# google-research/swirl-fem

Measured on AMD Instinct MI355X. Metric: GDOF/s per CG iteration, 3D p=7 Laplacian, higher is better.
Workload: dtype f64

## Files before the change

### include/sfem.h

```cpp
#ifndef SFEM_H_
#define SFEM_H_

#include <stdint.h>

#ifdef __cplusplus
extern "C" {
#endif

#define SFEM_ABI_VERSION 9

enum { SFEM_F32 = 0, SFEM_F64 = 1 };
enum {
  SFEM_OK = 0,
  SFEM_EINVAL = -1,
  SFEM_EHIP = -2,
  SFEM_EUNSUPPORTED = -3
};
#define SFEM_SENTINEL (-1)
#define SFEM_MAX_P 16

#define SFEM_IDX_MASK 0x3FFFFFFF
#define SFEM_IDX_PAD 0x3FFFFFFF
#define SFEM_IDX_DIRICHLET 0x80000000u
#define SFEM_IDX_SHARED 0x40000000u

typedef void* sfem_stream_t;

int sfem_abi_version(void);
const char* sfem_last_error(void);

int sfem_gather(const void* u, const int32_t* indices, void* out,
                int64_t count, double fill, int dtype, sfem_stream_t stream);

int sfem_gather_rows(const void* x, const int32_t* indices, void* out,
                     int64_t count, int ncomp, int dtype, sfem_stream_t stream);

int sfem_scatter_add(const void* u_local, const int32_t* indices, void* out,
                     int64_t count, int64_t num_nodes, int ncomp, int dtype,
                     sfem_stream_t stream);

int sfem_scatter_csr(const void* u_local, const int64_t* offsets,
                     const int32_t* slots, void* out, int64_t num_nodes,
                     int ncomp, int dtype, sfem_stream_t stream);

int sfem_exchange_local(const void* u, void* out, const int32_t* gidx,
                        const int32_t* unique, int64_t count,
                        int64_t num_nodes, void* sums, int64_t num_unique,
                        int ncomp, int dtype, sfem_stream_t stream);

int sfem_exchange_classes(void* u, const int32_t* members,
                          const int32_t* offsets, int64_t num_classes,
                          int ncomp, int64_t node_stride, int64_t comp_stride,
                          int dtype, sfem_stream_t stream);

int sfem_zero_strips(void* base, int64_t strip_len, int64_t strip_stride,
                     int nstrips, int dtype, sfem_stream_t stream);

int sfem_pack(const void* u, const int32_t* idx, void* buf, int64_t count,
              int ncomp, int dtype, sfem_stream_t stream);
int sfem_unpack_add(const void* buf, const int32_t* idx, void* u,
                    int64_t count, int ncomp, int dtype, sfem_stream_t stream);

int sfem_pack_strided(const void* u, const int32_t* idx, void* buf,
                      int64_t count, int ncomp, int64_t node_stride,
                      int64_t comp_stride, int dtype, sfem_stream_t stream);
int sfem_unpack_add_atomic(const void* buf, const int32_t* idx, void* u,
                           int64_t count, int ncomp, int64_t node_stride,
                           int64_t comp_stride, int dtype,
                           sfem_stream_t stream);

int sfem_geom_factors(const void* elem_coords, const void* interp1,
                      const void* grad1, int64_t num_elements, int ndim, int P,
                      int q, void* invjac, void* jacdet, void* quad_coords,
                      int dtype, sfem_stream_t stream);

int sfem_basis_eval(const void* u_local, const void* interp1,
                    const void* grad1, const void* invjac, void* val,
                    void* grad, int64_t num_elements, int ndim, int P, int q,
                    int ncomp, int collocated, int dtype, sfem_stream_t stream);

int sfem_basis_eval_t(const void* c0, const void* c1, const void* interp1,
                      const void* grad1, const void* invjac, const void* wdet,
                      void* out, int64_t num_elements, int ndim, int P, int q,
                      int ncomp, int collocated, int dtype,
                      sfem_stream_t stream);

enum { SFEM_COEF_NONE = 0, SFEM_COEF_ELEM = 1, SFEM_COEF_POINT = 2 };
enum { SFEM_GEO_POINT = 0, SFEM_GEO_AFFINE = 1, SFEM_GEO_MULTILINEAR = 3,
       SFEM_GEO_BOX = 5
                         };

int sfem_helmholtz_setup(const void* invjac, const void* jacdet,
                         const void* weights_nd , void* geo,
                         int64_t num_elements, int ndim, int Q, int dtype,
                         sfem_stream_t stream);
int sfem_helmholtz_setup_multilinear(const void* elem_coords, void* geo_elem,
                                     int64_t num_elements, int ndim, int P,
                                     int dtype, sfem_stream_t stream);

int sfem_encode_elements(const int32_t* elements, const uint8_t* dirichlet,
                         const int32_t* multiplicity,
                         const uint8_t* slot_shared, int32_t* enc,
                         int64_t count, sfem_stream_t stream);

typedef struct sfem_helmholtz_args {
  const void* u;
  void* out;
  const int32_t* enc;
  const void* geo;
  const void* geo_elem;
  const int32_t* geo_index;
  const int32_t* elem_list;
  const void* dmat;
  const void* weights;
  const void* nodes;
  int64_t num_elements;
  int64_t num_listed;
  int64_t num_nodes;
  int64_t zero_begin;
  int64_t zero_end;
  int32_t ndim;
  int32_t P;
  int32_t ncomp;
  int32_t dtype;
  int32_t geo_mode;
  int32_t colored;
  double lambda0;
  double lambda1;
  int64_t node_stride;
  int64_t comp_stride;
  double* dot_out;
  const uint16_t* shared_order;
  int32_t shared_stride;
  const int32_t* cluster_elems;
  const int32_t* cluster_offsets;
  const uint32_t* cluster_nodes;
  int64_t num_clusters;
  const int32_t* facet_table;
  const void* geo_const;
  const int32_t* chain_offsets;
  const int32_t* chain_elems;
  int64_t num_chains;
  int64_t layered_extent;
  int64_t dot_slots;
  const void* beta;
  const void* kappa;
  const void* sigma;
  int32_t coef_mode;
} sfem_helmholtz_args;

int sfem_facet_table_build(const int32_t* elements, const uint8_t* dirichlet,
                           const int32_t* multiplicity, int32_t* table,
                           uint8_t* ok, int64_t num_elements,
                           int64_t num_nodes, int P, sfem_stream_t stream);

int sfem_kernarg_selftest(int32_t* bad, sfem_stream_t stream);

int sfem_helmholtz_setup_affine(const void* geo_elem, void* geo_const,
                                int64_t num_elements, double box_tol,
                                int dtype, sfem_stream_t stream);

int sfem_helmholtz_cluster_limits(int P, int dtype, int* cluster_size,
                                  int* max_shared);
#define SFEM_DOT_SLOTS 1024

int sfem_helmholtz_apply(const sfem_helmholtz_args* args, sfem_stream_t stream);

int sfem_helmholtz_local(const sfem_helmholtz_args* args, sfem_stream_t stream);

typedef struct sfem_stokes_args {
  const void* u;
  void* out;
  const void* p_in;
  void* p_out;
  const void* scale;
  const int32_t* enc;
  const int32_t* penc;
  const void* kfac;
  const void* geo_elem;
  const int32_t* geo_index;
  const int32_t* elem_list;
  const void* dmat;
  const void* weights;
  const void* nodes;
  const void* interp;
  int64_t num_elements;
  int64_t num_listed;
  int64_t num_nodes;
  int64_t zero_begin, zero_end;
  int32_t ndim, P, dtype, geo_mode;
  int64_t node_stride, comp_stride;
  int32_t scale_per_node;
  const uint16_t* shared_order;
  int32_t shared_stride;
  double* dot_out;
  const int32_t* facet_table;
  const int32_t* chain_offsets;
  const int32_t* chain_elems;
  int64_t num_chains;
} sfem_stokes_args;

int sfem_stokes_setup(const void* invjac, const void* jacdet,
                      const void* weights_nd, void* kfac, int64_t num_elements,
                      int ndim, int Q, int dtype, sfem_stream_t stream);
int sfem_stokes_div(const sfem_stokes_args* args, sfem_stream_t stream);
int sfem_stokes_convect_local(const sfem_stokes_args* args,
                              sfem_stream_t stream);
int sfem_stokes_grad_t(const sfem_stokes_args* args, sfem_stream_t stream);
int sfem_stokes_e_first(const sfem_stokes_args* args, sfem_stream_t stream);
int sfem_stokes_e_second(const sfem_stokes_args* args, sfem_stream_t stream);

#define SFEM_CG_NSCALARS_NAMED 16
#define SFEM_CG_RR_SLOTS 64
#define SFEM_CG_NSCALARS (SFEM_CG_NSCALARS_NAMED + SFEM_CG_RR_SLOTS)
#define SFEM_CG_MEAN_SUMS (4 * SFEM_CG_RR_SLOTS)
#define SFEM_CG_STATUS_RUNNING 0.0
#define SFEM_CG_STATUS_CONVERGED 1.0
#define SFEM_CG_STATUS_MAXITER 2.0
#define SFEM_CG_STATUS_BAD_PAP 3.0
#define SFEM_CG_STATUS_BAD_GAMMA 4.0
int sfem_dot(const void* a, const void* b, int64_t count, double* result,
             int dtype, sfem_stream_t stream);
int sfem_dot_accumulate(const void* a, const void* b, int64_t count,
                        double* result, int dtype, sfem_stream_t stream);
int sfem_dot_indexed(const void* a, const void* b, const int64_t* idx,
                     const double* w, int64_t count, int ncomp,
                     int64_t node_stride, int64_t comp_stride, double scale,
                     double* result, int dtype, sfem_stream_t stream);
int sfem_subtract_weighted_mean(const void* w, const void* b, double total,
                                void* out, double* partials, int64_t count,
                                double* dot_result, int dtype,
                                sfem_stream_t stream);
int sfem_cg_scalars(double* scalars, int phase, double maxiter, double tol,
                    double atol, double* partials, sfem_stream_t stream);
int sfem_cg_update_xr(void* x, void* r, const void* p, const void* ap,
                      int64_t count, double* scalars, int fuse_rr, int dtype,
                      sfem_stream_t stream);
int sfem_cg_update_p(void* p, const void* z, int64_t count, double* scalars,
                     int dtype, sfem_stream_t stream);
int sfem_cg_update_r(void* r, const void* ap, int64_t count, double* scalars,
                     int fuse_rr, int dtype, sfem_stream_t stream);
int sfem_cg_update_xp(void* x, void* p, const void* z, int64_t count,
                      double* scalars, int dtype, sfem_stream_t stream);
#define SFEM_FOLD_GROUPS 256
int sfem_cg_scalars_n(double* scalars, int phase, double maxiter, double tol,
                      double atol, double* partials, int64_t num_partials,
                      sfem_stream_t stream);
int sfem_cg_update_r_layered_det(void* r, const void* ap_ext, int64_t count,
                                 const int64_t* layer_len,
                                 const int64_t* layer_off, int num_layers,
                                 const uint8_t* layer_masks,
                                 const int64_t* mask_off,
                                 double* scalars, double* rr_partials,
                                 int64_t rr_capacity, int64_t* num_rr,
                                 int dtype, sfem_stream_t stream);
#define SFEM_CG_LAZY_MAX 8
int sfem_cg_update_xp_lazy(void* x, void* pring, int64_t ring_stride,
                           const void* z, int64_t count, double* scalars,
                           double* lazy, int m, int dtype,
                           sfem_stream_t stream);
int sfem_cg_flush_x(void* x, const void* pring, int64_t ring_stride,
                    int64_t count, const double* scalars, double* lazy, int m,
                    int dtype, sfem_stream_t stream);
#define SFEM_MAX_LAYERS 15
#define SFEM_LAYER_CHUNK 512
int sfem_cg_update_r_layered(void* r, const void* ap_ext, int64_t count,
                             const int64_t* layer_len,
                             const int64_t* layer_off, int num_layers,
                             const uint8_t* layer_masks,
                             const int64_t* mask_off, double* scalars,
                             int fuse_rr, int dtype, sfem_stream_t stream);
int sfem_fold_layers(void* out_ext, int64_t count, const int64_t* layer_len,
                     const int64_t* layer_off, int num_layers, int dtype,
                     sfem_stream_t stream);
int sfem_fold_layers_at(void* out_ext, const int64_t* idx, int64_t num_idx,
                        int64_t count, const int64_t* layer_len,
                        const int64_t* layer_off, int num_layers, int dtype,
                        sfem_stream_t stream);
int sfem_cg_update_r_mean(void* r, const void* ap, const void* w,
                          int64_t count, double* scalars, double* sums,
                          int dtype, sfem_stream_t stream);
int sfem_cg_update_xp_mean(void* x, void* p, const void* r, int64_t count,
                           double* scalars, double* sums, double total,
                           int dtype, sfem_stream_t stream);
int sfem_fdm_solve(const void* r, void* z, const int64_t* pel, const void* S,
                   const int32_t* cases, const void* inv_eigenvalues,
                   int64_t num_elements, int ndim, int Pp, int dtype,
                   sfem_stream_t stream);
int sfem_fdm_solve_sums(const void* r, void* z, const int64_t* pel,
                        const void* S, const int32_t* cases,
                        const void* inv_eigenvalues, const void* weights,
                        void* elem_sum, void* weighted_sum,
                        int64_t num_elements, int ndim, int Pp, int dtype,
                        sfem_stream_t stream);
int sfem_add_element_constants(void* z, const void* yc, const void* shift,
                               int64_t num_elements, int n,
                               int64_t elems_per_member, int dtype,
                               sfem_stream_t stream);
int sfem_ell_chebyshev(const int32_t* cols, const void* vals, const void* dinv,
                       const void* b, void* x, void* work, int64_t n,
                       int width, int steps, double lmin, double lmax,
                       int dtype, sfem_stream_t stream);
#define SFEM_ENS_NSCALARS 16
#define SFEM_ENS_GROUPS 32
#define SFEM_ENS_MAX_MEMBERS 4096
int sfem_ens_dot(const void* a, const void* b, int64_t len, int members,
                 double* partials, int which, int dtype, sfem_stream_t stream);
int sfem_ens_init(double* scalars, const double* partials, int members,
                  double maxiter, double tol, double atol,
                  sfem_stream_t stream);
int sfem_ens_update_r(void* r, const void* ap, int64_t len, int members,
                      const double* scalars, const double* partials,
                      int dtype, sfem_stream_t stream);
int sfem_ens_close(double* scalars, const double* partials, int members,
                   double maxiter, sfem_stream_t stream);
int sfem_ens_update_xp(void* x, void* p, const void* z, int64_t len,
                       int members, const double* scalars, int dtype,
                       sfem_stream_t stream);
int sfem_ens_update_r_mean(void* r, const void* ap, const void* w, int64_t len,
                           int members, const double* scalars,
                           const double* partials, double* sums, int dtype,
                           sfem_stream_t stream);
int sfem_ens_close_mean(double* scalars, const double* partials,
                        const double* sums, double total, int members,
                        double maxiter, sfem_stream_t stream);
int sfem_ens_update_xp_mean(void* x, void* p, const void* r, int64_t len,
                            int members, const double* scalars, int dtype,
                            sfem_stream_t stream);
int sfem_ens_subtract_weighted_mean(const void* w, const void* b, double total,
                                    void* out, double* partials, int64_t len,
                                    int members, int dtype,
                                    sfem_stream_t stream);
typedef struct sfem_diag_args {
  void* mass_out;
  void* stiff_out;
  const void* geo;
  const void* geo_elem;
  const int32_t* geo_index;
  const int32_t* elem_list;
  const void* bmat;
  const void* dtil;
  const void* weights;
  const void* nodes;
  int64_t num_elements;
  int64_t num_listed;
  int ndim;
// ... 94 lines not shown
```

### swirl_fem_amd/_lib.py

```python

from __future__ import annotations

import ctypes
import os

from swirl_fem_amd import switches

_HERE = os.path.dirname(os.path.abspath(__file__))
LIB_PATH = switches.get('SFEM_LIB') or os.path.join(_HERE, 'libsfem_hip.so')
ABI_VERSION = 9

SFEM_F32, SFEM_F64 = 0, 1
SFEM_CG_NSCALARS_NAMED = 16
SFEM_CG_NSCALARS = 80
SFEM_BICGSTAB_NSCALARS = 32
BICGSTAB_STATUS = {0: 'running', 1: 'converged', 2: 'maxiter',
                   3: 'breakdown_rho', 4: 'breakdown_omega',
                   5: 'breakdown_alpha'}
CG_STATUS = {0: 'running', 1: 'converged', 2: 'maxiter', 3: 'breakdown_pAp',
             4: 'breakdown_gamma'}
SFEM_DOT_SLOTS = 1024
SFEM_CG_MEAN_SUMS = 256
SFEM_MAX_LAYERS = 15
SFEM_FOLD_GROUPS = 256
SFEM_LAYER_CHUNK = 512
SFEM_CG_LAZY_MAX = 8
SFEM_IDX_MASK = 0x3FFFFFFF
SFEM_ENS_NSCALARS = 16
SFEM_ENS_GROUPS = 32
SFEM_ENS_MAX_MEMBERS = 4096

c_i32, c_i64, c_dbl, c_ptr = (ctypes.c_int32, ctypes.c_int64, ctypes.c_double,
                              ctypes.c_void_p)


class HelmholtzArgs(ctypes.Structure):
  _fields_ = [
      ('u', c_ptr), ('out', c_ptr), ('enc', c_ptr), ('geo', c_ptr),
      ('geo_elem', c_ptr), ('geo_index', c_ptr), ('elem_list', c_ptr),
      ('dmat', c_ptr), ('weights', c_ptr), ('nodes', c_ptr),
      ('num_elements', c_i64), ('num_listed', c_i64), ('num_nodes', c_i64),
      ('zero_begin', c_i64), ('zero_end', c_i64), ('ndim', c_i32),
      ('P', c_i32), ('ncomp', c_i32), ('dtype', c_i32), ('geo_mode', c_i32),
      ('colored', c_i32), ('lambda0', c_dbl), ('lambda1', c_dbl),
      ('node_stride', c_i64), ('comp_stride', c_i64), ('dot_out', c_ptr),
      ('shared_order', c_ptr), ('shared_stride', c_i32),
      ('cluster_elems', c_ptr), ('cluster_offsets', c_ptr),
      ('cluster_nodes', c_ptr), ('num_clusters', c_i64),
      ('facet_table', c_ptr), ('geo_const', c_ptr),
      ('chain_offsets', c_ptr), ('chain_elems', c_ptr), ('num_chains', c_i64),
      ('layered_extent', c_i64), ('dot_slots', c_i64),
      ('beta', c_ptr),
      ('kappa', c_ptr), ('sigma', c_ptr), ('coef_mode', c_i32),
  ]


class StokesArgs(ctypes.Structure):
  _fields_ = [
      ('u', c_ptr), ('out', c_ptr), ('p_in', c_ptr), ('p_out', c_ptr),
      ('scale', c_ptr), ('enc', c_ptr), ('penc', c_ptr), ('kfac', c_ptr),
      ('geo_elem', c_ptr), ('geo_index', c_ptr), ('elem_list', c_ptr),
      ('dmat', c_ptr), ('weights', c_ptr), ('nodes', c_ptr), ('interp', c_ptr),
      ('num_elements', c_i64), ('num_listed', c_i64), ('num_nodes', c_i64),
      ('zero_begin', c_i64), ('zero_end', c_i64), ('ndim', c_i32),
      ('P', c_i32), ('dtype', c_i32), ('geo_mode', c_i32),
      ('node_stride', c_i64), ('comp_stride', c_i64),
      ('scale_per_node', c_i32), ('shared_order', c_ptr),
      ('shared_stride', c_i32), ('dot_out', c_ptr),
      ('facet_table', c_ptr), ('chain_offsets', c_ptr), ('chain_elems', c_ptr),
      ('num_chains', c_i64),
  ]


class DiagArgs(ctypes.Structure):
  _fields_ = [
      ('mass_out', c_ptr), ('stiff_out', c_ptr), ('geo', c_ptr),
      ('geo_elem', c_ptr), ('geo_index', c_ptr), ('elem_list', c_ptr),
      ('bmat', c_ptr), ('dtil', c_ptr), ('weights', c_ptr), ('nodes', c_ptr),
      ('num_elements', c_i64), ('num_listed', c_i64), ('ndim', c_i32),
      ('P', c_i32), ('Q', c_i32), ('dtype', c_i32), ('geo_mode', c_i32),
      ('kappa', c_ptr), ('sigma', c_ptr), ('coef_mode', c_i32),
  ]


GEO_POINT, GEO_AFFINE, GEO_MULTILINEAR, GEO_BOX = 0, 1, 3, 5
COEF_NONE, COEF_ELEM, COEF_POINT = 0, 1, 2

SIGNATURES = {
    'sfem_gather': [c_ptr, c_ptr, c_ptr, c_i64, c_dbl, c_i32, c_ptr],
    'sfem_gather_rows': [c_ptr, c_ptr, c_ptr, c_i64, c_i32, c_i32, c_ptr],
    'sfem_scatter_add': [c_ptr, c_ptr, c_ptr, c_i64, c_i64, c_i32, c_i32,
                         c_ptr],
    'sfem_scatter_csr': [c_ptr, c_ptr, c_ptr, c_ptr, c_i64, c_i32, c_i32,
                         c_ptr],
    'sfem_exchange_local': [c_ptr, c_ptr, c_ptr, c_ptr, c_i64, c_i64, c_ptr,
                            c_i64, c_i32, c_i32, c_ptr],
    'sfem_exchange_classes': [c_ptr, c_ptr, c_ptr, c_i64, c_i32, c_i64, c_i64,
                              c_i32, c_ptr],
    'sfem_zero_strips': [c_ptr, c_i64, c_i64, c_i32, c_i32, c_ptr],
    'sfem_subtract_weighted_mean': [c_ptr, c_ptr, c_dbl, c_ptr, c_ptr, c_i64,
                                    c_ptr, c_i32, c_ptr],
    'sfem_pack': [c_ptr, c_ptr, c_ptr, c_i64, c_i32, c_i32, c_ptr],
    'sfem_unpack_add': [c_ptr, c_ptr, c_ptr, c_i64, c_i32, c_i32, c_ptr],
    'sfem_pack_strided': [c_ptr, c_ptr, c_ptr, c_i64, c_i32, c_i64, c_i64,
                          c_i32, c_ptr],
    'sfem_unpack_add_atomic': [c_ptr, c_ptr, c_ptr, c_i64, c_i32, c_i64,
                               c_i64, c_i32, c_ptr],
    'sfem_geom_factors': [c_ptr, c_ptr, c_ptr, c_i64, c_i32, c_i32, c_i32,
                          c_ptr, c_ptr, c_ptr, c_i32, c_ptr],
    'sfem_basis_eval': [c_ptr, c_ptr, c_ptr, c_ptr, c_ptr, c_ptr, c_i64, c_i32,
                        c_i32, c_i32, c_i32, c_i32, c_i32, c_ptr],
    'sfem_basis_eval_t': [c_ptr, c_ptr, c_ptr, c_ptr, c_ptr, c_ptr, c_ptr,
                          c_i64, c_i32, c_i32, c_i32, c_i32, c_i32, c_i32,
                          c_ptr],
    'sfem_helmholtz_setup': [c_ptr, c_ptr, c_ptr, c_ptr, c_i64, c_i32, c_i32,
                             c_i32, c_ptr],
    'sfem_encode_elements': [c_ptr, c_ptr, c_ptr, c_ptr, c_ptr, c_i64, c_ptr],
    'sfem_helmholtz_apply': [ctypes.POINTER(HelmholtzArgs), c_ptr],
    'sfem_helmholtz_setup_multilinear': [c_ptr, c_ptr, c_i64, c_i32, c_i32,
                                         c_i32, c_ptr],
    'sfem_helmholtz_local': [ctypes.POINTER(HelmholtzArgs), c_ptr],
    'sfem_facet_table_build': [c_ptr, c_ptr, c_ptr, c_ptr, c_ptr, c_i64, c_i64,
                               c_i32, c_ptr],
    'sfem_helmholtz_setup_affine': [c_ptr, c_ptr, c_i64, c_dbl, c_i32, c_ptr],
    'sfem_helmholtz_cluster_limits': [c_i32, c_i32, ctypes.POINTER(c_i32),
                                      ctypes.POINTER(c_i32)],
    'sfem_dot': [c_ptr, c_ptr, c_i64, c_ptr, c_i32, c_ptr],
    'sfem_dot_accumulate': [c_ptr, c_ptr, c_i64, c_ptr, c_i32, c_ptr],
    'sfem_dot_indexed': [c_ptr, c_ptr, c_ptr, c_ptr, c_i64, c_i32, c_i64,
                         c_i64, c_dbl, c_ptr, c_i32, c_ptr],
    'sfem_cg_scalars': [c_ptr, c_i32, c_dbl, c_dbl, c_dbl, c_ptr, c_ptr],
    'sfem_cg_update_xr': [c_ptr, c_ptr, c_ptr, c_ptr, c_i64, c_ptr, c_i32,
                          c_i32, c_ptr],
    'sfem_cg_update_p': [c_ptr, c_ptr, c_i64, c_ptr, c_i32, c_ptr],
    'sfem_cg_update_r': [c_ptr, c_ptr, c_i64, c_ptr, c_i32, c_i32, c_ptr],
    'sfem_cg_update_xp': [c_ptr, c_ptr, c_ptr, c_i64, c_ptr, c_i32, c_ptr],
    'sfem_cg_update_r_layered': [c_ptr, c_ptr, c_i64, c_ptr, c_ptr, c_i32,
                                 c_ptr, c_ptr, c_ptr, c_i32, c_i32, c_ptr],
    'sfem_kernarg_selftest': [c_ptr, c_ptr],
    'sfem_fdm_solve': [c_ptr, c_ptr, c_ptr, c_ptr, c_ptr, c_ptr, c_i64, c_i32,
                       c_i32, c_i32, c_ptr],
    'sfem_fdm_solve_sums': [c_ptr, c_ptr, c_ptr, c_ptr, c_ptr, c_ptr, c_ptr,
                            c_ptr, c_ptr, c_i64, c_i32, c_i32, c_i32, c_ptr],
    'sfem_add_element_constants': [c_ptr, c_ptr, c_ptr, c_i64, c_i32, c_i64,
                                   c_i32, c_ptr],
    'sfem_ell_chebyshev': [c_ptr, c_ptr, c_ptr, c_ptr, c_ptr, c_ptr, c_i64,
                           c_i32, c_i32, c_dbl, c_dbl, c_i32, c_ptr],
    'sfem_ens_dot': [c_ptr, c_ptr, c_i64, c_i32, c_ptr, c_i32, c_i32, c_ptr],
    'sfem_ens_init': [c_ptr, c_ptr, c_i32, c_dbl, c_dbl, c_dbl, c_ptr],
    'sfem_ens_update_r': [c_ptr, c_ptr, c_i64, c_i32, c_ptr, c_ptr, c_i32,
                          c_ptr],
    'sfem_ens_close': [c_ptr, c_ptr, c_i32, c_dbl, c_ptr],
    'sfem_ens_update_xp': [c_ptr, c_ptr, c_ptr, c_i64, c_i32, c_ptr, c_i32,
                           c_ptr],
    'sfem_ens_update_r_mean': [c_ptr, c_ptr, c_ptr, c_i64, c_i32, c_ptr, c_ptr,
                               c_ptr, c_i32, c_ptr],
    'sfem_ens_close_mean': [c_ptr, c_ptr, c_ptr, c_dbl, c_i32, c_dbl, c_ptr],
    'sfem_ens_update_xp_mean': [c_ptr, c_ptr, c_ptr, c_i64, c_i32, c_ptr,
                                c_i32, c_ptr],
    'sfem_ens_subtract_weighted_mean': [c_ptr, c_ptr, c_dbl, c_ptr, c_ptr,
                                        c_i64, c_i32, c_i32, c_ptr],
    'sfem_fold_layers': [c_ptr, c_i64, c_ptr, c_ptr, c_i32, c_i32, c_ptr],
    'sfem_fold_layers_at': [c_ptr, c_ptr, c_i64, c_i64, c_ptr, c_ptr, c_i32,
                            c_i32, c_ptr],
    'sfem_cg_scalars_n': [c_ptr, c_i32, c_dbl, c_dbl, c_dbl, c_ptr, c_i64,
                          c_ptr],
    'sfem_cg_update_r_layered_det': [c_ptr, c_ptr, c_i64, c_ptr, c_ptr, c_i32,
                                     c_ptr, c_ptr, c_ptr, c_ptr, c_i64, c_ptr,
                                     c_i32, c_ptr],
    'sfem_cg_update_xp_lazy': [c_ptr, c_ptr, c_i64, c_ptr, c_i64, c_ptr, c_ptr,
                               c_i32, c_i32, c_ptr],
    'sfem_cg_flush_x': [c_ptr, c_ptr, c_i64, c_i64, c_ptr, c_ptr, c_i32, c_i32,
                        c_ptr],
    'sfem_cg_update_r_mean': [c_ptr, c_ptr, c_ptr, c_i64, c_ptr, c_ptr, c_i32,
                              c_ptr],
    'sfem_cg_update_xp_mean': [c_ptr, c_ptr, c_ptr, c_i64, c_ptr, c_ptr, c_dbl,
                               c_i32, c_ptr],
    'sfem_axpby': [c_dbl, c_ptr, c_dbl, c_ptr, c_i64, c_i32, c_ptr],
    'sfem_helmholtz_diag': [ctypes.POINTER(DiagArgs), c_ptr],
    'sfem_cg_update_r_jacobi': [c_ptr, c_ptr, c_ptr, c_i64, c_i32, c_ptr,
                                c_ptr, c_i32, c_ptr, c_ptr, c_ptr, c_ptr,
                                c_i64, c_ptr, c_i32, c_ptr],
    'sfem_cg_update_xp_jacobi': [c_ptr, c_ptr, c_ptr, c_ptr, c_i64, c_i32,
                                 c_ptr, c_i32, c_ptr],
    'sfem_stokes_setup': [c_ptr, c_ptr, c_ptr, c_ptr, c_i64, c_i32, c_i32,
                          c_i32, c_ptr],
    'sfem_stokes_div': [c_ptr, c_ptr],
    'sfem_stokes_grad_t': [c_ptr, c_ptr],
    'sfem_stokes_e_first': [c_ptr, c_ptr],
    'sfem_stokes_e_second': [c_ptr, c_ptr],
    'sfem_stokes_convect_local': [c_ptr, c_ptr],
    'sfem_pmg_prolong': [c_ptr, c_ptr, c_ptr, c_ptr, c_ptr, c_ptr, c_i64,
                         c_i32, c_i32, c_i32, c_i32, c_i32, c_ptr],
    'sfem_pmg_restrict': [c_ptr, c_ptr, c_ptr, c_ptr, c_ptr, c_ptr, c_i64,
                          c_i32, c_i32, c_i32, c_i32, c_ptr],
    'sfem_cheb_step': [c_ptr, c_ptr, c_ptr, c_ptr, c_ptr, c_ptr, c_dbl, c_dbl,
                       c_i64, c_i32, c_i32, c_ptr],
    'sfem_pmg_dot2': [c_ptr, c_ptr, c_ptr, c_i64, c_ptr, c_i32, c_i32, c_ptr],
    'sfem_pmg_cg_scalars': [c_ptr, c_i32, c_ptr, c_i64, c_dbl, c_dbl, c_dbl,
                            c_ptr],
    'sfem_boundary_geom': [c_ptr, c_ptr, c_i64, c_ptr, c_ptr, c_ptr, c_i32,
                           c_i32, c_i32, c_ptr, c_ptr, c_i32, c_ptr],
    'sfem_boundary_covector': [c_ptr, c_i32, c_ptr, c_i64, c_ptr, c_ptr,
                               c_i32, c_i32, c_i32, c_ptr, c_i32, c_ptr],
    'sfem_boundary_mass_apply': [c_ptr, c_ptr, c_i64, c_ptr, c_ptr, c_i32,
                                 c_i32, c_i32, c_dbl, c_ptr, c_i32, c_ptr],
    'sfem_boundary_mass_diag': [c_ptr, c_i64, c_ptr, c_ptr, c_i32, c_i32,
                                c_i32, c_dbl, c_ptr, c_i32, c_ptr],
    'sfem_boundary_add_rows': [c_ptr, c_ptr, c_ptr, c_ptr, c_i64, c_ptr, c_i32,
                               c_ptr],
    'sfem_ell_spmv': [c_ptr, c_ptr, c_ptr, c_ptr, c_i64, c_i32, c_i64, c_i64,
                      c_ptr, c_i64, c_i32, c_ptr],
    'sfem_bicgstab_scalars': [c_ptr, c_i32, c_dbl, c_dbl, c_dbl, c_ptr],
    'sfem_bicgstab_dot': [c_ptr, c_ptr, c_i64, c_ptr, c_i32, c_i32, c_i32,
                          c_ptr],
    'sfem_bicgstab_update_p': [c_ptr, c_ptr, c_ptr, c_ptr, c_ptr, c_i64, c_ptr,
                               c_i32, c_ptr],
    'sfem_bicgstab_update_s': [c_ptr, c_ptr, c_ptr, c_ptr, c_ptr, c_i64, c_ptr,
                               c_i32, c_ptr],
    'sfem_bicgstab_update_xr': [c_ptr, c_ptr, c_ptr, c_ptr, c_ptr, c_ptr,
                                c_ptr, c_i64, c_ptr, c_i32, c_ptr],
    'sfem_abi_version': [],
}

_lib = None


class SfemError(RuntimeError):
  """A C-ABI call returned a non-zero status."""


def load() -> ctypes.CDLL:
  global _lib
  if _lib is not None:
    return _lib
  if not os.path.exists(LIB_PATH):
    raise SfemError(
        f'{LIB_PATH} is missing: the HIP extension has not been built. '
        'Run `make -C swirl_fem_amd/csrc -j8` (needs hipcc, gfx950). There is '
        'no CPU fallback.')
  lib = ctypes.CDLL(LIB_PATH)
  for name, argtypes in SIGNATURES.items():
    fn = getattr(lib, name)
    fn.argtypes = argtypes
    fn.restype = ctypes.c_int
  lib.sfem_last_error.argtypes = []
  lib.sfem_last_error.restype = ctypes.c_char_p
  if lib.sfem_abi_version() != ABI_VERSION:
    raise SfemError(f'ABI version mismatch: library '
                    f'{lib.sfem_abi_version()} != binding {ABI_VERSION}')
  _lib = lib
  return lib


def check(status: int, who: str):
  if status != 0:
# ... 3 lines not shown
```

### swirl_fem_amd/_ops.py

```python

from __future__ import annotations

import ctypes
import os

import numpy as np
import torch

from swirl_fem_amd import switches
from swirl_fem_amd import _lib

_DT = {torch.float32: _lib.SFEM_F32, torch.float64: _lib.SFEM_F64}


def _dtype_code(t: torch.Tensor) -> int:
  try:
    return _DT[t.dtype]
  except KeyError:
    raise TypeError(f'unsupported dtype {t.dtype}; use float32 or float64')


def _dev(*tensors):
  dev = None
  for t in tensors:
# ... 320 lines not shown
  dev = _dev(elements, dirichlet_u8, multiplicity, slot_shared)
  enc = torch.empty_like(elements)
  with torch.cuda.device(dev):
    _lib.check(_lib.load().sfem_encode_elements(
        _ptr(elements), _ptr(dirichlet_u8), _ptr(multiplicity),
        _ptr(slot_shared), _ptr(enc), elements.numel(), _stream(dev)),
        'sfem_encode_elements')
  return enc


def helmholtz_setup_multilinear(elem_coords, ndim, P):
  elem_coords = elem_coords.contiguous()
  dev = _dev(elem_coords)
  E = elem_coords.shape[0]
  geo_elem = torch.empty((E, 24), dtype=elem_coords.dtype, device=dev)
  with torch.cuda.device(dev):
    _lib.check(_lib.load().sfem_helmholtz_setup_multilinear(
        _ptr(elem_coords), _ptr(geo_elem), E, ndim, P,
        _dtype_code(elem_coords), _stream(dev)),
        'sfem_helmholtz_setup_multilinear')
  return geo_elem


_KERNARG_CHECKED = set()


def kernarg_selftest(dev):
  if dev in _KERNARG_CHECKED:
    return
  bad = torch.zeros(1, dtype=torch.int32, device=dev)
  with torch.cuda.device(dev):
    _lib.check(_lib.load().sfem_kernarg_selftest(_ptr(bad), _stream(dev)),
               'sfem_kernarg_selftest')
  if int(bad.item()) != 0:
    raise _lib.SfemError(
        'the kernel-argument layout differs from what the facet kernels '
        f'assume (probe flags {int(bad.item())}): rebuild libsfem_hip.so with '
        'the toolchain it was written for (FacetKernarg::MAT_OFF)')
  _KERNARG_CHECKED.add(dev)


def facet_table(elements, dirichlet_u8, multiplicity, P):
  elements = _idx(elements)
  dev = _dev(elements, dirichlet_u8, multiplicity)
  kernarg_selftest(dev)
  E = elements.shape[0]
  tab = torch.empty((E, 27, 4), dtype=torch.int32, device=dev)
  ok = torch.empty((E,), dtype=torch.uint8, device=dev)
  with torch.cuda.device(dev):
    _lib.check(_lib.load().sfem_facet_table_build(
        _ptr(elements), _ptr(dirichlet_u8), _ptr(multiplicity), _ptr(tab),
        _ptr(ok), E, multiplicity.shape[0], P, _stream(dev)),
        'sfem_facet_table_build')
  return tab, ok != 0


def helmholtz_setup_affine(geo_elem, box_tol):
  geo_elem = geo_elem.contiguous()
  dev = _dev(geo_elem)
  E = geo_elem.shape[0]
  out = torch.empty((E, 8), dtype=geo_elem.dtype, device=dev)
  with torch.cuda.device(dev):
    _lib.check(_lib.load().sfem_helmholtz_setup_affine(
        _ptr(geo_elem), _ptr(out), E, float(box_tol), _dtype_code(geo_elem),
        _stream(dev)), 'sfem_helmholtz_setup_affine')
  return out


def _host(a, dtype):
  np_dt = np.float64 if dtype == torch.float64 else np.float32
  return None if a is None else np.ascontiguousarray(a, dtype=np_dt)


def _hptr(a):
  return None if a is None else a.ctypes.data


def _dptr(t):
  return None if t is None else t.data_ptr()


def _helmholtz_args(u, out, enc, part, host, ndim, P, num_elements, num_nodes,
                    lambda0, lambda1, zero_range, dot_out=None,
                    layered_extent=0, dot_slots=0):
  vec = u.dim() != (1 if enc is not None else 2)
  ncomp = u.shape[-1] if vec else 1
  node_stride = comp_stride = 0
  if vec and not u.is_contiguous():
    node_stride, comp_stride = 1, u.stride(-1)
  lst = part.get('elem_list')
  so = part.get('shared_order')
  cl = part.get('cluster') if enc is not None else None
  if cl is not None:
    enc, so = cl.enc, None
  ft = part.get('facet_table') if enc is not None else None
  ch = None
  if layered_extent:
    ft, so = part['layered_table'], None
    ch = part.get('chains') if part.get('layered_chains') else None
  elif ft is not None:
    so = None
    if ((not vec or node_stride == 1) and
        switches.get('SFEM_CHAIN') != '0' and
        (not vec or switches.get('SFEM_CHAIN_VECTOR') != '0')):
      ch = part.get('chains')
  return _lib.HelmholtzArgs(
      u=u.data_ptr(), out=out.data_ptr(), enc=_dptr(enc),
      geo=_dptr(part.get('geo')), geo_elem=_dptr(part.get('geo_elem')),
      geo_index=_dptr(part.get('geo_index')), elem_list=_dptr(lst),
      dmat=_hptr(host['dmat']), weights=_hptr(host.get('weights')),
      nodes=_hptr(host.get('nodes')), num_elements=num_elements,
      num_listed=0 if lst is None else lst.numel(), num_nodes=num_nodes,
      zero_begin=int(zero_range[0]), zero_end=int(zero_range[1]), ndim=ndim,
      P=P, ncomp=ncomp, dtype=_dtype_code(u), geo_mode=part['geo_mode'],
      colored=int(bool(part.get('colored', False))), lambda0=float(lambda0),
      lambda1=float(lambda1), node_stride=node_stride,
      comp_stride=comp_stride,
      dot_out=_dptr(dot_out),
      shared_order=_dptr(so if enc is not None else None),
      shared_stride=0 if so is None or enc is None else so.shape[1],
      cluster_elems=_dptr(cl.elems if cl is not None else None),
      cluster_offsets=_dptr(cl.offsets if cl is not None else None),
      cluster_nodes=_dptr(cl.nodes if cl is not None else None),
      num_clusters=0 if cl is None else cl.num_clusters,
      facet_table=_dptr(ft),
      geo_const=_dptr(part.get('geo_const') if ft is not None else None),
      chain_offsets=_dptr(ch[0] if ch is not None else None),
      chain_elems=_dptr(ch[1] if ch is not None else None),
      num_chains=0 if ch is None else ch[0].numel() - 1,
      layered_extent=int(layered_extent), dot_slots=int(dot_slots),
      kappa=_dptr(part.get('kappa')), sigma=_dptr(part.get('sigma')),
      coef_mode=int(part.get('coef_mode', _lib.COEF_NONE)),
      beta=_dptr(part.get('beta')))


_CLUSTER_LIMITS = {}


def helmholtz_cluster_limits(P, dtype):
  key = (P, dtype)
  if key not in _CLUSTER_LIMITS:
    size, kmax = ctypes.c_int32(0), ctypes.c_int32(0)
    code = _lib.SFEM_F64 if dtype == torch.float64 else _lib.SFEM_F32
    rc = _lib.load().sfem_helmholtz_cluster_limits(
        P, code, ctypes.byref(size), ctypes.byref(kmax))
    _CLUSTER_LIMITS[key] = None if rc else (size.value, kmax.value)
  return _CLUSTER_LIMITS[key]


def helmholtz_kernel_name(real, P, ndim, scalar, geo_mode, part, mass,
                          layered=False):
  b = lambda v: 'true' if v else 'false'
  if part.get('facet_table') is not None:
    elem = ('sfem::BoxElem<%s, %d, %s>' % (real, P, b(mass)) if geo_mode == 5
            else 'sfem::FacetElem<%s, %d, %d, %s>' % (real, P, geo_mode,
                                                     b(mass)))
    if layered:
      if part.get('chains') is not None and part.get('layered_chains'):
        return 'sfem::helmholtz_chain_kernel<%s, %d, %s, *, true>' % (
            real, P, elem)
      return 'sfem::helmholtz_facet_kernel<%s, %d, %s, true, *, true>' % (
          real, P, elem)
    if (scalar and part.get('chains') is not None and
        switches.get('SFEM_CHAIN') != '0'):
      return 'sfem::helmholtz_chain_kernel<%s, %d, %s, ' % (real, P, elem)
    return 'sfem::helmholtz_facet_kernel<%s, %d, %s, %s, ' % (
        real, P, elem, b(scalar))
  if (real == 'float' and P == 12 and ndim == 3 and scalar and
      geo_mode in (1, 3) and part.get('cluster') is None and
      not part.get('colored') and switches.get('SFEM_MFMA') == '1'):
    return 'sfem::helmholtz_mfma_p12_kernel<%d, %s>' % (geo_mode, b(mass))
  if part.get('cluster') is not None:
    return 'sfem::helmholtz_cluster_kernel<%s, %d, %s, %d, %s>' % (
        real, P, b(scalar), geo_mode, b(mass))
  if part.get('beta') is not None:
    return 'sfem::helmholtz_adv_kernel<%s, %d, %d, true, %d>' % (
        real, P, ndim, geo_mode)
  if part.get('coef_mode'):
    return ('sfem::helmholtz_kernel<%s, %d, %d, true, true, %d, false, %s, '
            '%d>' % (real, P, ndim, geo_mode, b(mass), part['coef_mode']))
  tpe = P * P if ndim == 3 else P
  can_sort = ndim == 3 and tpe <= 64
  sort = (can_sort and part.get('shared_order') is not None and
          not part.get('colored') and not (geo_mode == 3 and mass))
  b = lambda v: 'true' if v else 'false'
  return 'sfem::helmholtz_kernel<%s, %d, %d, true, %s, %d, %s, %s>' % (
      real, P, ndim, b(scalar), geo_mode, b(sort), b(mass))


def helmholtz_apply(u, out, enc, parts, host, ndim, P, lambda0, lambda1,
                    zero_range, dot_out=None):
  dev = _dev(enc)
  _check_vector_layout(u, out)
  host = {k: _host(v, u.dtype) for k, v in host.items()}
  if not parts and zero_range[1] > zero_range[0]:
    out[zero_range[0]:zero_range[1]].zero_()
  with torch.cuda.device(dev):
    for n, part in enumerate(parts):
      args = _helmholtz_args(u, out, part.get('enc', enc), part, host, ndim,
                             P, enc.shape[0], u.shape[0], lambda0, lambda1,
                             zero_range if n == 0 else (0, 0), dot_out)
      _lib.check(_lib.load().sfem_helmholtz_apply(ctypes.byref(args),
                                                  _stream(dev)),
                 'sfem_helmholtz_apply')
  return out


def layered_dot_waves(parts, P, num_elements):
  waves = (P * P + 63) // 64
  out = []
  for part in parts:
    if part.get('layered_chains'):
      groups = part['chains'][0].numel() - 1
    elif 'elem_list' in part:
      groups = part['elem_list'].numel()
    else:
      groups = num_elements
    out.append(groups * waves)
  return out


def helmholtz_apply_layered(u, ext, enc, parts, host, ndim, P, lambda0,
                            lambda1, dot_out=None, per_wave=False):
  dev = _dev(enc)
  if u.dim() != 1 or not u.is_contiguous() or not ext.is_contiguous():
    raise ValueError('layered assembly takes contiguous scalar fields')
  if ext.dtype != u.dtype:
    raise ValueError('u and the extended output differ in dtype')
  host = {k: _host(v, u.dtype) for k, v in host.items()}
  waves = (layered_dot_waves(parts, P, enc.shape[0])
           if per_wave and dot_out is not None else None)
  if waves is not None and sum(waves) > dot_out.numel():
    raise ValueError(f'{sum(waves)} waves but {dot_out.numel()} dot slots')
  at = 0
  with torch.cuda.device(dev):
    for n, part in enumerate(parts):
      dots = dot_out if waves is None else dot_out[at:at + waves[n]]
      args = _helmholtz_args(u, ext, enc, part, host, ndim, P, enc.shape[0],
                             u.shape[0], lambda0, lambda1, (0, 0), dots,
                             layered_extent=ext.numel(),
                             dot_slots=0 if waves is None else waves[n])
      if waves is not None:
        at += waves[n]
      _lib.check(_lib.load().sfem_helmholtz_apply(ctypes.byref(args),
                                                  _stream(dev)),
                 'sfem_helmholtz_apply')
  return ext


def _layer_arrays(layers):
  n = len(layers)
  arr = ctypes.c_int64 * max(n, 1)
  return (arr(*[int(l[0]) for l in layers]) if n else arr(0),
          arr(*[int(l[1]) for l in layers]) if n else arr(0), n)


def _mask_args(masks, n):
  if masks is None:
    return None, None
  data, offs = masks
  arr = ctypes.c_int64 * max(n, 1)
  return _ptr(data), arr(*[int(o) for o in offs])


def cg_update_r_layered(r, ap_ext, layers, scalars, fuse_rr, masks=None):
  dev = _dev(r, ap_ext, scalars)
  ln, off, n = _layer_arrays(layers)
  mptr, moff = _mask_args(masks, n)
  with torch.cuda.device(dev):
    _lib.check(_lib.load().sfem_cg_update_r_layered(
        _ptr(r), _ptr(ap_ext), r.numel(), ln, off, n, mptr, moff,
        _ptr(scalars), int(fuse_rr), _dtype_code(r), _stream(dev)),
        'sfem_cg_update_r_layered')


def cg_update_r_layered_det(r, ap_ext, layers, scalars, rr_partials,
                            masks=None):
  dev = _dev(r, ap_ext, scalars, rr_partials)
  ln, off, n = _layer_arrays(layers)
  mptr, moff = _mask_args(masks, n)
  count = ctypes.c_int64(0)
  with torch.cuda.device(dev):
    _lib.check(_lib.load().sfem_cg_update_r_layered_det(
        _ptr(r), _ptr(ap_ext), r.numel(), ln, off, n, mptr, moff,
        _ptr(scalars),
        _ptr(rr_partials), rr_partials.numel(), ctypes.byref(count),
        _dtype_code(r), _stream(dev)), 'sfem_cg_update_r_layered_det')
  return count.value


def cg_scalars_n(scalars, phase, maxiter, tol, atol, partials, num_partials):
  dev = _dev(scalars, partials)
  with torch.cuda.device(dev):
    _lib.check(_lib.load().sfem_cg_scalars_n(
        _ptr(scalars), phase, float(maxiter), float(tol), float(atol),
        _ptr(partials), int(num_partials), _stream(dev)), 'sfem_cg_scalars_n')


def fold_layers_at(ext, idx, count, layers):
  dev = _dev(ext, idx)
  if idx.dtype != torch.int64:
    raise ValueError('fold_layers_at: int64 node positions')
  ln, off, n = _layer_arrays(layers)
  with torch.cuda.device(dev):
    _lib.check(_lib.load().sfem_fold_layers_at(
        _ptr(ext), _ptr(idx), idx.numel(), int(count), ln, off, n,
        _dtype_code(ext), _stream(dev)), 'sfem_fold_layers_at')
  return ext


def fdm_solve(r, pel, S, cases, inv_ev, ndim, Pp):
  dev = _dev(r, pel, S, cases, inv_ev)
  z = torch.empty_like(r)
  with torch.cuda.device(dev):
    _lib.check(_lib.load().sfem_fdm_solve(
        _ptr(r), _ptr(z), _ptr(pel), _ptr(S), _ptr(cases), _ptr(inv_ev),
        cases.shape[1], int(ndim), int(Pp), _dtype_code(r), _stream(dev)),
        'sfem_fdm_solve')
  return z


def fdm_solve_sums(r, pel, S, cases, inv_ev, weights, ndim, Pp):
  dev = _dev(r, pel, S, cases, inv_ev, weights)
  E = cases.shape[1]
# ... 339 lines not shown
  for t in (u, out):
    if not t.is_cuda:
      raise RuntimeError(
          'swirl_fem_amd kernels run on MI355X device tensors only; got a '
          f'{t.device} tensor (there is no CPU fallback)')
    if not (t.is_contiguous() or is_component_major(t)):
      raise ValueError('expected a contiguous or component-major tensor')
  if u.stride() != out.stride() or u.shape != out.shape:
    raise ValueError('u and out must share shape and memory layout')


def helmholtz_local(u_local, parts, host, ndim, P, lambda0, lambda1):
  if not (u_local.is_contiguous() or is_component_major(u_local)):
    u_local = u_local.contiguous()
  dev = u_local.device
  host = {k: _host(v, u_local.dtype) for k, v in host.items()}
  out = torch.empty_like(u_local)
  _check_vector_layout(u_local, out)
  with torch.cuda.device(dev):
    for part in parts:
      args = _helmholtz_args(u_local, out, None, part, host, ndim, P,
                             u_local.shape[0], 0, lambda0, lambda1, (0, 0))
      _lib.check(_lib.load().sfem_helmholtz_local(ctypes.byref(args),
                                                  _stream(dev)),
                 'sfem_helmholtz_local')
  return out


def dot(a, b, result, slot, accumulate=False):
  dev = _dev(a, b, result)
  fn = (_lib.load().sfem_dot_accumulate if accumulate
        else _lib.load().sfem_dot)
  with torch.cuda.device(dev):
    _lib.check(fn(_ptr(a), _ptr(b), a.numel(),
                  ctypes.c_void_p(result.data_ptr() + 8 * slot),
                  _dtype_code(a), _stream(dev)), 'sfem_dot')


def dot_indexed(a, b, idx, w, result, slot, scale):
  ncomp, ns, cs = _node_view(a)
  if _node_view(b) != (ncomp, ns, cs) or a.dtype != b.dtype:
    raise ValueError('dot_indexed: operands must share layout and dtype')
  flat = lambda t: t.movedim(-1, 0) if is_component_major(t) else t
  dev = _dev(flat(a), flat(b), idx, w, result)
  with torch.cuda.device(dev):
    _lib.check(_lib.load().sfem_dot_indexed(
        _ptr(a), _ptr(b), _ptr(idx), _ptr(w), idx.numel(), ncomp, ns, cs,
        float(scale), result.data_ptr() + 8 * slot, _dtype_code(a),
        _stream(dev)), 'sfem_dot_indexed')


def cg_scalars(scalars, phase, maxiter, tol, atol, partials=None):
  dev = _dev(scalars, partials)
  with torch.cuda.device(dev):
    _lib.check(_lib.load().sfem_cg_scalars(
        _ptr(scalars), phase, float(maxiter), float(tol), float(atol),
        _ptr(partials), _stream(dev)), 'sfem_cg_scalars')


def cg_update_xr(x, r, p, ap, scalars, fuse_rr):
  dev = _dev(x, r, p, ap, scalars)
  with torch.cuda.device(dev):
    _lib.check(_lib.load().sfem_cg_update_xr(
        _ptr(x), _ptr(r), _ptr(p), _ptr(ap), x.numel(), _ptr(scalars),
        int(fuse_rr), _dtype_code(x), _stream(dev)), 'sfem_cg_update_xr')


def cg_update_p(p, z, scalars):
  dev = _dev(p, z, scalars)
  with torch.cuda.device(dev):
    _lib.check(_lib.load().sfem_cg_update_p(
        _ptr(p), _ptr(z), p.numel(), _ptr(scalars), _dtype_code(p),
        _stream(dev)), 'sfem_cg_update_p')


def cg_update_r(r, ap, scalars, fuse_rr):
  dev = _dev(r, ap, scalars)
  with torch.cuda.device(dev):
    _lib.check(_lib.load().sfem_cg_update_r(
        _ptr(r), _ptr(ap), r.numel(), _ptr(scalars), int(fuse_rr),
        _dtype_code(r), _stream(dev)), 'sfem_cg_update_r')


def cg_update_xp_lazy(x, pring, z, scalars, lazy):
  dev = _dev(x, pring, z, scalars, lazy)
  with torch.cuda.device(dev):
    _lib.check(_lib.load().sfem_cg_update_xp_lazy(
        _ptr(x), _ptr(pring), pring.stride(0), _ptr(z), x.numel(),
        _ptr(scalars), _ptr(lazy), pring.shape[0], _dtype_code(x),
        _stream(dev)), 'sfem_cg_update_xp_lazy')


def cg_flush_x(x, pring, scalars, lazy):
  dev = _dev(x, pring, scalars, lazy)
  with torch.cuda.device(dev):
    _lib.check(_lib.load().sfem_cg_flush_x(
        _ptr(x), _ptr(pring), pring.stride(0), x.numel(), _ptr(scalars),
        _ptr(lazy), pring.shape[0], _dtype_code(x), _stream(dev)),
        'sfem_cg_flush_x')


def cg_update_xp(x, p, z, scalars):
  dev = _dev(x, p, z, scalars)
  with torch.cuda.device(dev):
    _lib.check(_lib.load().sfem_cg_update_xp(
        _ptr(x), _ptr(p), _ptr(z), x.numel(), _ptr(scalars), _dtype_code(x),
        _stream(dev)), 'sfem_cg_update_xp')


def cg_update_r_mean(r, ap, w, scalars, sums):
  dev = _dev(r, ap, w, scalars, sums)
  with torch.cuda.device(dev):
    _lib.check(_lib.load().sfem_cg_update_r_mean(
        _ptr(r), _ptr(ap), _ptr(w), r.numel(), _ptr(scalars), _ptr(sums),
        _dtype_code(r), _stream(dev)), 'sfem_cg_update_r_mean')


def cg_update_xp_mean(x, p, r, scalars, sums, total):
  dev = _dev(x, p, r, scalars, sums)
  with torch.cuda.device(dev):
    _lib.check(_lib.load().sfem_cg_update_xp_mean(
        _ptr(x), _ptr(p), _ptr(r), x.numel(), _ptr(scalars), _ptr(sums),
        float(total), _dtype_code(x), _stream(dev)), 'sfem_cg_update_xp_mean')


def axpby(a, x, b, y):
  dev = _dev(x, y)
  with torch.cuda.device(dev):
    _lib.check(_lib.load().sfem_axpby(
        float(a), _ptr(x), float(b), _ptr(y), x.numel(), _dtype_code(x),
        _stream(dev)), 'sfem_axpby')
  return y


def bicgstab_scalars(scalars, phase, maxiter, tol, atol):
  dev = _dev(scalars)
  with torch.cuda.device(dev):
    _lib.check(_lib.load().sfem_bicgstab_scalars(
        _ptr(scalars), int(phase), float(maxiter), float(tol), float(atol),
        _stream(dev)), 'sfem_bicgstab_scalars')


def bicgstab_dot(a, b, scalars, slot, two=False):
  dev = _dev(a, b, scalars)
  if a.dtype != b.dtype or a.numel() != b.numel():
    raise ValueError('bicgstab_dot: operands must share size and dtype')
  with torch.cuda.device(dev):
    _lib.check(_lib.load().sfem_bicgstab_dot(
        _ptr(a), _ptr(b), a.numel(), _ptr(scalars), int(slot), int(two),
        _dtype_code(a), _stream(dev)), 'sfem_bicgstab_dot')


def _same(name, *ts):
  first = ts[0]
  for t in ts:
    if t is not None and (t.dtype != first.dtype or
                          t.numel() != first.numel()):
      raise ValueError(f'{name}: vectors must share size and dtype')


def bicgstab_update_p(p, phat, r, v, dinv, scalars):
  dev = _dev(p, phat, r, v, dinv, scalars)
  _same('bicgstab_update_p', p, phat, r, v, dinv)
  with torch.cuda.device(dev):
    _lib.check(_lib.load().sfem_bicgstab_update_p(
        _ptr(p), _ptr(phat), _ptr(r), _ptr(v), _ptr(dinv), p.numel(),
        _ptr(scalars), _dtype_code(p), _stream(dev)),
        'sfem_bicgstab_update_p')


def bicgstab_update_s(s, shat, r, v, dinv, scalars):
  dev = _dev(s, shat, r, v, dinv, scalars)
  _same('bicgstab_update_s', s, shat, r, v, dinv)
  with torch.cuda.device(dev):
    _lib.check(_lib.load().sfem_bicgstab_update_s(
        _ptr(s), _ptr(shat), _ptr(r), _ptr(v), _ptr(dinv), s.numel(),
        _ptr(scalars), _dtype_code(s), _stream(dev)),
        'sfem_bicgstab_update_s')


def bicgstab_update_xr(x, r, phat, shat, s, t, r0, scalars):
  dev = _dev(x, r, phat, shat, s, t, r0, scalars)
# ... 222 lines not shown
```

### swirl_fem_amd/core/operators.py

```python

from __future__ import annotations

import dataclasses
import os

import numpy as np
import torch

from swirl_fem_amd import switches
from swirl_fem_amd import _ops

MAX_FUSED_P = 12


def supports_fused(fespace) -> str | None:
  P = fespace.mesh.gridpoints_1d.num_points
  if not fespace.is_collocated:
    return 'quadrature points differ from the nodes'
  if fespace.mesh.ndim not in (2, 3):
    return f'ndim={fespace.mesh.ndim}'
  if not 2 <= P <= MAX_FUSED_P:
    return f'P={P} outside 2..{MAX_FUSED_P}'
  d = fespace.interpolator._differentiation_matrix_1d()
  if not np.allclose(d[::-1, ::-1], -d, rtol=0,
# ... 717 lines not shown
  def split(self, element_mask):
    if any(p.get('colored') for p in self.parts):
      raise NotImplementedError('split() of a coloured operator')
    if self.coefs is not None:
      raise NotImplementedError('split() of an operator with coefficients')
    mask = torch.as_tensor(element_mask, device=self.enc.device).to(torch.bool)
    E = self.enc.shape[0]
    if mask.shape != (E,):
      raise ValueError(f'expected an ({E},) element mask')
    clustered = any(p.get('cluster') is not None for p in self.parts)

    def restrict(part_list, keep):
      parts = []
      for part in part_list:
        part = {k: v for k, v in part.items() if k != 'cluster'}
        if 'elem_list' in part:
          lst = part['elem_list']
          lst = lst[keep[lst.to(torch.int64)]]
        else:
          lst = torch.nonzero(keep).reshape(-1).to(torch.int32)
        if lst.numel():
          new = dict(part, elem_list=lst.contiguous())
          if 'chains' in new:
            new['chains'] = facet_chains(
                self.fespace.mesh.elements, lst.to(torch.int64),
                self.fespace.mesh.gridpoints_1d.num_points, new['chain_len'])
          parts.append(new)
      return parts

    halves = []
    for keep in (mask, ~mask):
      parts = restrict(self.parts, keep)
      if clustered:
        parts = _attach_clusters(
            self.fespace, self.enc,
            self.fespace.mesh.assembly_plan().multiplicity, parts)
      facet = (None if self.facet_parts is None
               else restrict(self.facet_parts, keep))
      halves.append(dataclasses.replace(self, parts=parts, facet_parts=facet,
                                        _vector_parts=None, _layer_plan=False,
                                        _diag=None, _diag_adv=None))
    return tuple(halves)

  def apply(self, u, lambda0=0.0, lambda1=1.0, out=None, *, zero=True,
            dot_out=None):
    mesh = self.fespace.mesh
    if u.shape[0] != mesh.num_nodes:
      raise ValueError(f'expected {mesh.num_nodes} nodal values, got '
                       f'{tuple(u.shape)}')
    if self.coefs is not None:
      _check_scalar_field(u)
      lambda0, lambda1 = _scaled(self.coefs, lambda0, lambda1)
    if self.beta is not None:
      _check_scalar_field(u, 'a velocity takes')
      if dot_out is not None:
        raise NotImplementedError('dot_out of an operator with a velocity')
    u = u.to(self.fespace.dtype)
    if not (u.is_contiguous() or _ops.is_component_major(u)):
      u = u.contiguous()
    if out is None:
      out = torch.empty_like(u)
    return _ops.helmholtz_apply(
        u, out, self.enc, self._parts_for(u), self.host, mesh.ndim,
        mesh.gridpoints_1d.num_points, lambda0, lambda1,
        self.zero_range if zero else (0, 0), dot_out)

  def layer_plan(self):
    if self._layer_plan is None:
      plan = None
      if (self.facet_parts is not None and
          switches.get('SFEM_LAYERED') != '0'):
        mesh = self.fespace.mesh
        plan = build_layer_plan(self.facet_parts, mesh.num_elements,
                                mesh.num_nodes, mesh.gridpoints_1d.num_points)
      self._layer_plan = plan if plan is not None else False
    return self._layer_plan or None

  def new_extended(self):
    plan = self.layer_plan()
    return torch.zeros(plan.extent, dtype=self.fespace.dtype,
                       device=self.enc.device)

  def apply_layered(self, u, ext, lambda0=0.0, lambda1=1.0, *, dot_out=None,
                    per_wave=False):
    plan = self.layer_plan()
    if plan is None:
      raise NotImplementedError('this operator has no layer plan')
    mesh = self.fespace.mesh
    if tuple(u.shape) != (mesh.num_nodes,):
      raise ValueError(f'expected ({mesh.num_nodes},) nodal values, got '
                       f'{tuple(u.shape)}')
    if tuple(ext.shape) != (plan.extent,):
      raise ValueError(f'expected an extended output of {plan.extent} values')
    return _ops.helmholtz_apply_layered(
        u.to(self.fespace.dtype).contiguous(), ext, self.enc, plan.parts,
        self.host, mesh.ndim, mesh.gridpoints_1d.num_points, lambda0, lambda1,
        dot_out, per_wave)

  def layered_dot_slots(self):
    mesh = self.fespace.mesh
    return sum(_ops.layered_dot_waves(self.layer_plan().parts,
                                      mesh.gridpoints_1d.num_points,
                                      mesh.num_elements))

  def _parts_for(self, u):
    if self.facet_parts is None or not (
        u.dim() == 1 or u.shape[-1] == 1 or _ops.is_component_major(u)):
      return self.parts
    if u.dim() == 1 or u.shape[-1] == 1:
      return self.facet_parts
    if self._vector_parts is None:
      if not any(q['geo_mode'] == _GEO_POINT and 'facet_table' in q
                 for q in self.facet_parts):
        self._vector_parts = self.facet_parts
      elif self.fespace.dtype == torch.float64:
        self._vector_parts = (
            [q for q in self.facet_parts if q['geo_mode'] != _GEO_POINT] +
            [q for q in self.parts if q['geo_mode'] == _GEO_POINT])
      else:
        self._vector_parts = [
            {k: v for k, v in q.items() if k != 'chains'}
            if q['geo_mode'] == _GEO_POINT else q for q in self.facet_parts]
    return self._vector_parts

  def diagonal(self, lambda0=0.0, lambda1=1.0, assembled=True):
    if self._diag is None:
      self._diag = _assembled_diagonal(self.fespace, self.parts, self.host,
                                       self.keep, None)
    lambda0, lambda1 = _scaled(self.coefs, lambda0, lambda1)
    d = _combine_diagonal(self._diag, lambda0, lambda1, assembled,
                          self.fespace.mesh)
    if self.beta is not None:
      if self._diag_adv is None:
        self._diag_adv = _advection_diagonal(
            self.fespace, self.parts, self.beta, self.host['dmat'], self.keep,
            None)
      d = d + self._diag_adv
    return d

  def point_weights(self):
    mesh = self.fespace.mesh
    P = mesh.gridpoints_1d.num_points
    mass, _ = _ops.helmholtz_diag(
        self._geo_parts or self.parts, mesh.num_elements, mesh.ndim, P,
        self.host['dmat'], self.host['weights'], self.host['nodes'], None,
        want_stiff=False, dtype=self.fespace.dtype, device=self.fespace.device)
    return mass

  def apply_local(self, u_local, lambda0=0.0, lambda1=1.0):
    mesh = self.fespace.mesh
    if self.coefs is not None:
      if u_local.dim() == 3 and u_local.shape[-1] != 1:
        raise NotImplementedError('coefficients take scalar fields')
      lambda0, lambda1 = _scaled(self.coefs, lambda0, lambda1)
    if self.beta is not None and u_local.dim() == 3 and u_local.shape[-1] != 1:
      raise NotImplementedError('a velocity takes scalar fields')
    return _ops.helmholtz_local(
        u_local.to(self.fespace.dtype), self.parts, self.host, mesh.ndim,
        mesh.gridpoints_1d.num_points, lambda0, lambda1)

  def linear_operator(self, lambda0=0.0, lambda1=1.0):
    if self.beta is not None:
      return _PlainLinearOperator(self, lambda0, lambda1)
    return FusedLinearOperator(self, lambda0, lambda1)

  def bytes_per_apply(self, lambda0=0.0, ncomp=1, layered=False):
    mesh = self.fespace.mesh
    E, n = mesh.elements.shape
    s = 8 if self.fespace.dtype == torch.float64 else 4
    total = 2 * s * mesh.num_nodes * ncomp
    parts = self.facet_parts if self.facet_parts is not None else self.parts
    if layered:
      plan = self.layer_plan()
      total = s * (mesh.num_nodes + plan.written)
      parts = plan.parts
    for part in parts:
      count = part['elem_list'].numel() if 'elem_list' in part else E
      mode = part['geo_mode']
      if 'facet_table' in part:
        conn = 27 * 16 + (4 if 'chains' in part and ncomp == 1 else 0)
      else:
        conn = 4 * n + (4 if 'elem_list' in part else 0)
        if part.get('shared_order') is not None:
          conn += 2 * part['shared_order'].shape[1]
      if mode == _GEO_POINT:
        geo = (7 if lambda0 else 6) * s * n
      elif 'facet_table' in part and mode in (_GEO_AFFINE, _GEO_BOX):
        geo = 8 * s
      else:
        geo = 24 * s
      geo += _coefficient_bytes(part, s, n, lambda0)
      if part.get('beta') is not None:
        geo += s * n * mesh.ndim
      total += count * (conn + geo)
    return total

  def kernel_name(self, lambda0=0.0, lambda1=1.0, ncomp=1, layered=False):
    mesh = self.fespace.mesh
    real = 'double' if self.fespace.dtype == torch.float64 else 'float'
    P = mesh.gridpoints_1d.num_points
    names = []
    parts = (self.layer_plan().parts if layered else
             self.parts if self.facet_parts is None else self.facet_parts)
    for part in parts:
      gm = part['geo_mode']
      names.append(_ops.helmholtz_kernel_name(
          real, P, mesh.ndim, ncomp == 1, gm, part,
          _scaled(self.coefs, lambda0, lambda1)[0] != 0, layered))
    return ' + '.join(sorted(set(names)))


class FusedLinearOperator:

  def __init__(self, op, lambda0, lambda1):
    self.op, self.lambda0, self.lambda1 = op, lambda0, lambda1
    self._ext = None

  def __call__(self, u):
    return self.op.apply(u, self.lambda0, self.lambda1)

  def apply_with_dot(self, u, partials):
    return self.op.apply(u, self.lambda0, self.lambda1, dot_out=partials)

  def layer_plan(self):
    plan = self.op.layer_plan()
    if plan is not None and switches.get('SFEM_LAYERED') != 'force' and any(
        q['geo_mode'] == _GEO_POINT for q in plan.parts):
      return None
    return plan

  def apply_layered_with_dot(self, u, partials, per_wave=False):
    if self._ext is None:
      self._ext = self.op.new_extended()
    return self.op.apply_layered(u, self._ext, self.lambda0, self.lambda1,
                                 dot_out=partials, per_wave=per_wave)

  def layered_dot_slots(self):
    return self.op.layered_dot_slots()


def supports_fused_stokes(vspace, pspace) -> str | None:
  why = supports_fused(vspace)
  if why is not None:
    return why
  P = vspace.mesh.gridpoints_1d.num_points
  if P < 4:
    return f'P={P} < 4'
  if pspace.mesh.gridpoints_1d.num_points != P - 2:
    return 'pressure space is not P - 2 points per direction'
  if pspace.interpolator.evalpoints_1d != vspace.mesh.gridpoints_1d:
    return 'pressure quadrature differs from the velocity nodes'
  if pspace.mesh.num_elements != vspace.mesh.num_elements:
    return 'velocity and pressure meshes have different elements'
  E = vspace.mesh.num_elements
  sample = torch.unique(torch.linspace(
      0, max(E - 1, 0), steps=min(E, 512), device=vspace.device).round().long())
  jv, jp = _sample_jacdets(vspace, sample), _sample_jacdets(pspace, sample)
  ndim = vspace.mesh.ndim
  if jv.numel():
    h = 2.0 * float(jv.abs().amax()) ** (1.0 / ndim)
    xmax = float(vspace.mesh.node_coords.abs().amax())
    P = vspace.mesh.gridpoints_1d.num_points
    rounding = 32 * torch.finfo(jv.dtype).eps * P * P * max(xmax / h, 1.0)
  else:
    rounding = 0.0
  tight = 1e-10 if jv.dtype == torch.float64 else 1e-4
  kind = _cached_geometry_kind(vspace)[sample]
  tol = torch.where(kind != _GEO_POINT, max(tight, rounding),
                    max(tight, rounding / 4)).to(jv.dtype)
  if jv.shape != jp.shape or not bool(
      ((jv - jp).abs() <= tol[:, None] * jv.abs().amax()).all()):
    return 'velocity and pressure spaces carry different geometry'
  return None


def _cached_geometry_kind(fespace):
  cache = fespace._cache
  if 'geometry_kind' not in cache:
    cache['geometry_kind'] = classify_geometry(fespace)[0]
  return cache['geometry_kind']


def _sample_jacdets(space, elements):
  mesh = space.mesh
  i1, g1 = space._matrices()
  xe = _ops.gather_rows(mesh.node_coords,
                        mesh.elements[elements].contiguous())
  _, jacdets, _ = _ops.geom_factors(
      xe, i1, g1, mesh.ndim, mesh.gridpoints_1d.num_points,
      space.quadrature.num_points, want_quad_coords=False)
  return jacdets


def shared_slot_order(enc):
  E, n = enc.shape
  chunks, smax = [], 0
  step = max(1, (1 << 25) // n)
  for lo in range(0, E, step):
    e64 = enc[lo:lo + step].to(torch.int64)
    ids = e64 & 0x3FFFFFFF
    take = ((e64 & (1 << 30)) != 0) & (e64 >= 0) & (ids != 0x3FFFFFFF)
    key = torch.where(take, ids, torch.full_like(ids, 1 << 40))
    order = torch.argsort(key, dim=1, stable=True)
    count = take.sum(dim=1)
    smax = max(smax, int(count.max()) if count.numel() else 0)
    chunks.append((order, count))
  if smax == 0:
    return None
  out = torch.empty((E, smax), dtype=torch.int16, device=enc.device)
  col = torch.arange(smax, device=enc.device)[None, :]
  at = 0
  for order, count in chunks:
    tab = order[:, :smax].to(torch.int32)
    tab = torch.where(col < count[:, None], tab, torch.full_like(tab, 0xFFFF))
    out[at:at + len(tab)] = tab.to(torch.int16)
    at += len(tab)
  return out.contiguous()

# ... 643 lines not shown
```

### swirl_fem_amd/csrc/sfem_core.hip

```cpp
#include <stdarg.h>
#include <string.h>

#include "sfem_common.h"

namespace sfem {

static thread_local char g_error[512] = "";

void set_error(const char* fmt, ...) {
  va_list ap;
  va_start(ap, fmt);
  vsnprintf(g_error, sizeof(g_error), fmt, ap);
  va_end(ap);
}

template <typename T>
__global__ void __launch_bounds__(256)
gather_kernel(const T* __restrict__ u, const int32_t* __restrict__ idx,
              T* __restrict__ out, int64_t count, T fill) {
  const int64_t stride = (int64_t)gridDim.x * blockDim.x;
  for (int64_t i = (int64_t)blockIdx.x * blockDim.x + threadIdx.x; i < count;
       i += stride) {
    const int32_t k = idx[i];
    out[i] = k < 0 ? fill : u[k];
// ... 440 lines not shown
    const int64_t i = nvec * VN + threadIdx.x;
    p[i] = z[i] + beta * p[i];
  }
}

template <typename T, bool FUSE_RR, bool NT, bool STRIPED = false>
__global__ void __launch_bounds__(512)
cg_update_r_kernel(T* __restrict__ r, const T* __restrict__ ap, int64_t count,
                   double* __restrict__ scalars) {
  if (scalars[7] != 0.0) return;
  using V = typename Vec16<T>::type;
  constexpr int VN = Vec16<T>::N;
  const T alpha = (T)(scalars[0] / scalars[1]);
  const int64_t nvec = count / VN;
  V* rv = reinterpret_cast<V*>(r);
  const V* apv = reinterpret_cast<const V*>(ap);
  const int64_t stride = (int64_t)gridDim.x * blockDim.x;
  double acc = 0.0;
  for (int64_t i = (int64_t)blockIdx.x * blockDim.x + threadIdx.x; i < nvec;
       i += stride) {
    V rr = ld16<T, NT>(&rv[i]);
    const V aa = ld16<T, NT>(&apv[i]);
#pragma unroll
    for (int c = 0; c < VN; ++c) {
      T* re = reinterpret_cast<T*>(&rr) + c;
      *re -= alpha * vget<T>(aa, c);
      if (FUSE_RR) acc += (double)*re * (double)*re;
    }
    st16<T, NT>(rr, &rv[i]);
  }
  if (blockIdx.x == 0 && threadIdx.x < count - nvec * VN) {
    const int64_t i = nvec * VN + threadIdx.x;
    const T rn = r[i] - alpha * ap[i];
    r[i] = rn;
    if (FUSE_RR) acc += (double)rn * (double)rn;
  }
  if (FUSE_RR) {
    const double total = block_sum(acc);
    if (threadIdx.x == 0)
      unsafeAtomicAdd(STRIPED ? &scalars[SFEM_CG_NSCALARS_NAMED +
                                         (blockIdx.x & (SFEM_CG_RR_SLOTS - 1))]
                              : &scalars[2], total);
  }
}

template <typename T, bool NT>
__global__ void __launch_bounds__(512)
cg_update_xp_kernel(T* __restrict__ x, T* __restrict__ p,
                    const T* __restrict__ z, int64_t count,
                    const double* __restrict__ scalars) {
  if (scalars[7] != 0.0) return;
  using V = typename Vec16<T>::type;
  constexpr int VN = Vec16<T>::N;
  const T alpha = (T)(scalars[0] / scalars[1]);
  const T beta = (T)(cg_gamma_new(scalars) / scalars[0]);
  const int64_t nvec = count / VN;
  V* xv = reinterpret_cast<V*>(x);
  V* pv = reinterpret_cast<V*>(p);
  const V* zv = reinterpret_cast<const V*>(z);
  const int64_t stride = (int64_t)gridDim.x * blockDim.x;
  for (int64_t i = (int64_t)blockIdx.x * blockDim.x + threadIdx.x; i < nvec;
       i += stride) {
    V xx = ld16<T, NT>(&xv[i]);
    V pp = ld16<T, NT>(&pv[i]);
    const V zz = ld16<T, NT>(&zv[i]);
#pragma unroll
    for (int c = 0; c < VN; ++c) {
      T* xe = reinterpret_cast<T*>(&xx) + c;
      T* pe = reinterpret_cast<T*>(&pp) + c;
      *xe += alpha * *pe;
      *pe = vget<T>(zz, c) + beta * *pe;
    }
    st16<T, NT>(xx, &xv[i]);
    st16<T, NT>(pp, &pv[i]);
  }
  if (blockIdx.x == 0 && threadIdx.x < count - nvec * VN) {
    const int64_t i = nvec * VN + threadIdx.x;
    const T pi = p[i];
    x[i] += alpha * pi;
    p[i] = z[i] + beta * pi;
  }
}

template <typename T, bool NT>
__global__ void __launch_bounds__(512)
cg_update_xp_lazy_kernel(T* __restrict__ x, T* __restrict__ pring,
                         int64_t ring_stride, const T* __restrict__ z,
                         int64_t count, const double* __restrict__ scalars,
                         double* __restrict__ lazy, int m) {
  if (scalars[7] != 0.0) return;
  using V = typename Vec16<T>::type;
  constexpr int VN = Vec16<T>::N;
  const int64_t k = (int64_t)scalars[8];
  const int slot = (int)(k % m), next = (int)((k + 1) % m);
  const T alpha = (T)(scalars[0] / scalars[1]);
  const T beta = (T)(cg_gamma_new(scalars) / scalars[0]);
  const bool flush = next == 0;
  int64_t lo = (int64_t)lazy[0];
  if (lo < k + 1 - m) lo = k + 1 - m;
  T a_old[SFEM_CG_LAZY_MAX];
  int s_old[SFEM_CG_LAZY_MAX];
  int n_old = 0;
  if (flush) {
    for (int64_t j = lo; j < k; ++j) {
      s_old[n_old] = (int)(j % m);
      a_old[n_old++] = (T)lazy[1 + (j % m)];
    }
  }
  if (blockIdx.x == 0 && threadIdx.x == 0) lazy[1 + slot] = (double)alpha;
  const int64_t nvec = count / VN;
  V* xv = reinterpret_cast<V*>(x);
  const V* pk = reinterpret_cast<const V*>(pring + slot * ring_stride);
  V* pn = reinterpret_cast<V*>(pring + next * ring_stride);
  const V* zv = reinterpret_cast<const V*>(z);
  const int64_t stride = (int64_t)gridDim.x * blockDim.x;
  for (int64_t i = (int64_t)blockIdx.x * blockDim.x + threadIdx.x; i < nvec;
       i += stride) {
    const V pp = ld16<T, NT>(&pk[i]);
    const V zz = ld16<T, NT>(&zv[i]);
    if (flush) {
      V xx = ld16<T, NT>(&xv[i]);
      for (int q = 0; q < n_old; ++q) {
        const V po = ld16<T, NT>(
            reinterpret_cast<const V*>(pring + s_old[q] * ring_stride) + i);
#pragma unroll
        for (int c = 0; c < VN; ++c)
          reinterpret_cast<T*>(&xx)[c] += a_old[q] * vget<T>(po, c);
      }
#pragma unroll
      for (int c = 0; c < VN; ++c)
        reinterpret_cast<T*>(&xx)[c] += alpha * vget<T>(pp, c);
      st16<T, NT>(xx, &xv[i]);
    }
    V np;
#pragma unroll
    for (int c = 0; c < VN; ++c)
      reinterpret_cast<T*>(&np)[c] = vget<T>(zz, c) + beta * vget<T>(pp, c);
    st16<T, NT>(np, &pn[i]);
  }
  if (blockIdx.x == 0 && threadIdx.x < count - nvec * VN) {
    const int64_t i = nvec * VN + threadIdx.x;
    const T pi = pring[slot * ring_stride + i];
    if (flush) {
      T xx = x[i];
      for (int q = 0; q < n_old; ++q)
        xx += a_old[q] * pring[s_old[q] * ring_stride + i];
      xx += alpha * pi;
      x[i] = xx;
    }
    pring[next * ring_stride + i] = z[i] + beta * pi;
  }
}

template <typename T>
__global__ void __launch_bounds__(512)
cg_flush_x_kernel(T* __restrict__ x, const T* __restrict__ pring,
                  int64_t ring_stride, int64_t count,
                  const double* __restrict__ scalars,
                  const double* __restrict__ lazy, int m) {
  const int64_t iters = (int64_t)scalars[8];
  int64_t lo = (int64_t)lazy[0];
  if (lo < iters - iters % m) lo = iters - iters % m;
  if (lo >= iters) return;
  const int64_t stride = (int64_t)gridDim.x * blockDim.x;
  for (int64_t i = (int64_t)blockIdx.x * blockDim.x + threadIdx.x; i < count;
       i += stride) {
    T xx = x[i];
    for (int64_t j = lo; j < iters; ++j)
      xx += (T)lazy[1 + (j % m)] * pring[(j % m) * ring_stride + i];
    x[i] = xx;
  }
}

__global__ void cg_lazy_mark_kernel(const double* __restrict__ scalars,
                                    double* __restrict__ lazy) {
  if (threadIdx.x == 0 && blockIdx.x == 0) lazy[0] = scalars[8];
}

template <typename T, bool NT>
__global__ void __launch_bounds__(512)
cg_update_r_mean_kernel(T* __restrict__ r, const T* __restrict__ ap,
                        const T* __restrict__ w, int64_t count,
                        double* __restrict__ scalars,
                        double* __restrict__ sums) {
  if (scalars[7] != 0.0) return;
  using V = typename Vec16<T>::type;
  constexpr int VN = Vec16<T>::N;
  const T alpha = (T)(scalars[0] / scalars[1]);
  double* set = sums + (((int64_t)scalars[8]) & 1) * (2 * SFEM_CG_RR_SLOTS);
  const int64_t nvec = count / VN;
  V* rv = reinterpret_cast<V*>(r);
  const V* apv = reinterpret_cast<const V*>(ap);
  const V* wv = reinterpret_cast<const V*>(w);
  const int64_t stride = (int64_t)gridDim.x * blockDim.x;
  double rr_acc = 0.0, one_acc = 0.0, w_acc = 0.0;
  for (int64_t i = (int64_t)blockIdx.x * blockDim.x + threadIdx.x; i < nvec;
       i += stride) {
    V rr = ld16<T, NT>(&rv[i]);
    const V aa = ld16<T, NT>(&apv[i]);
    const V ww = ld16<T, NT>(&wv[i]);
#pragma unroll
    for (int c = 0; c < VN; ++c) {
      T* re = reinterpret_cast<T*>(&rr) + c;
      *re -= alpha * vget<T>(aa, c);
      const double v = (double)*re;
      rr_acc += v * v;
      one_acc += v;
      w_acc += v * (double)vget<T>(ww, c);
    }
    st16<T, NT>(rr, &rv[i]);
  }
  if (blockIdx.x == 0 && threadIdx.x < count - nvec * VN) {
    const int64_t i = nvec * VN + threadIdx.x;
    const T rn = r[i] - alpha * ap[i];
    r[i] = rn;
    rr_acc += (double)rn * (double)rn;
    one_acc += (double)rn;
    w_acc += (double)rn * (double)w[i];
  }
  double t[3] = {rr_acc, one_acc, w_acc};
  block_sum3(t);
  if (threadIdx.x == 0) {
    const int q = blockIdx.x & (SFEM_CG_RR_SLOTS - 1);
    unsafeAtomicAdd(&scalars[SFEM_CG_NSCALARS_NAMED + q], t[0]);
    unsafeAtomicAdd(&set[q], t[1]);
    unsafeAtomicAdd(&set[SFEM_CG_RR_SLOTS + q], t[2]);
  }
}

template <typename T, bool NT>
__global__ void __launch_bounds__(512)
cg_update_xp_mean_kernel(T* __restrict__ x, T* __restrict__ p,
                         const T* __restrict__ r, int64_t count,
                         double* __restrict__ scalars,
                         double* __restrict__ sums, double total) {
  if (scalars[7] != 0.0) return;
  using V = typename Vec16<T>::type;
  constexpr int VN = Vec16<T>::N;
  const int par = (int)(((int64_t)scalars[8]) & 1);
  const double* set = sums + par * (2 * SFEM_CG_RR_SLOTS);
  double one_r = set[threadIdx.x & 63];
  double w_r = set[SFEM_CG_RR_SLOTS + (threadIdx.x & 63)];
#pragma unroll
  for (int off = 32; off > 0; off >>= 1) {
    one_r += __shfl_xor(one_r, off, 64);
    w_r += __shfl_xor(w_r, off, 64);
  }
  const double mean = w_r / total;
  const double corr = -mean * one_r;
// ... 972 lines not shown
  SFEM_REQUIRE(x && p && z, "sfem_cg_update_xp: null pointer");
  DISPATCH_DTYPE(dtype, {
    if (streams_past_caches(count, sizeof(T)))
      hipLaunchKernelGGL((cg_update_xp_kernel<T, true>),
                         dim3(stream_grid(count, 512 * 2)), dim3(512), 0,
                         as_stream(stream), (T*)x, (T*)p, (const T*)z, count,
                         scalars);
    else
      hipLaunchKernelGGL((cg_update_xp_kernel<T, false>),
                         dim3(stream_grid(count, 512 * 2)), dim3(512), 0,
                         as_stream(stream), (T*)x, (T*)p, (const T*)z, count,
                         scalars);
  });
  SFEM_LAUNCH_CHECK();
  return SFEM_OK;
}

int sfem_cg_update_r_jacobi(void* r, const void* ap_ext, const void* dinv,
                            int64_t period, int ncomp,
                            const int64_t* layer_len,
                            const int64_t* layer_off, int num_layers,
                            const uint8_t* layer_masks,
                            const int64_t* mask_off, double* scalars,
                            double* rz_partials, int64_t rz_capacity,
                            int64_t* num_rz, int dtype, sfem_stream_t stream) {
  SFEM_REQUIRE(period >= 0 && ncomp >= 1 && scalars &&
                   (!rz_partials || (num_rz && rz_capacity >= 1)),
               "sfem_cg_update_r_jacobi: bad arguments");
  SFEM_REQUIRE(dtype == SFEM_F32 || dtype == SFEM_F64,
               "sfem_cg_update_r_jacobi: unknown dtype %d", dtype);
  const int vn = dtype == SFEM_F64 ? 2 : 4;
  SFEM_REQUIRE(ncomp == 1 || (period % vn == 0 && num_layers == 0),
               "sfem_cg_update_r_jacobi: %d components need a period that is "
               "a multiple of %d and no layers", ncomp, vn);
  if (num_rz) *num_rz = 0;
  if (period == 0) return SFEM_OK;
  SFEM_REQUIRE(r && ap_ext && dinv, "sfem_cg_update_r_jacobi: null pointer");
  LayerDesc ld;
  const int rc = make_layer_desc("sfem_cg_update_r_jacobi", layer_len,
                                 layer_off, num_layers, period, vn, &ld,
                                 layer_masks, mask_off);
  if (rc != SFEM_OK) return rc;
  int grid = stream_grid(period, 512 * 2);
  if (rz_partials && grid > rz_capacity) grid = (int)rz_capacity;
  if (num_rz) *num_rz = rz_partials ? grid : 0;
  DISPATCH_DTYPE(dtype, launch_update_r_jacobi<T>(
      streams_past_caches(period * ncomp, sizeof(T)), rz_partials != nullptr,
      grid, as_stream(stream), (T*)r, (const T*)ap_ext, (const T*)dinv,
      period, ncomp, ld, scalars, rz_partials));
  SFEM_LAUNCH_CHECK();
  return SFEM_OK;
}

int sfem_cg_update_xp_jacobi(void* x, void* p, const void* r,
                             const void* dinv, int64_t period, int ncomp,
                             double* scalars, int dtype,
                             sfem_stream_t stream) {
  SFEM_REQUIRE(period >= 0 && ncomp >= 1 && scalars,
               "sfem_cg_update_xp_jacobi: bad arguments");
  SFEM_REQUIRE(dtype == SFEM_F32 || dtype == SFEM_F64,
               "sfem_cg_update_xp_jacobi: unknown dtype %d", dtype);
  SFEM_REQUIRE(ncomp == 1 || period % (dtype == SFEM_F64 ? 2 : 4) == 0,
               "sfem_cg_update_xp_jacobi: %d components need a period that "
               "is a multiple of the vector width", ncomp);
  if (period == 0) return SFEM_OK;
  SFEM_REQUIRE(x && p && r && dinv, "sfem_cg_update_xp_jacobi: null pointer");
  DISPATCH_DTYPE(dtype, {
    const unsigned grid = stream_grid(period, 512 * 2);
    if (streams_past_caches(period * ncomp, sizeof(T)))
      hipLaunchKernelGGL((cg_update_xp_jacobi_kernel<T, true>), dim3(grid),
                         dim3(512), 0, as_stream(stream), (T*)x, (T*)p,
                         (const T*)r, (const T*)dinv, period, ncomp, scalars);
    else
      hipLaunchKernelGGL((cg_update_xp_jacobi_kernel<T, false>), dim3(grid),
                         dim3(512), 0, as_stream(stream), (T*)x, (T*)p,
                         (const T*)r, (const T*)dinv, period, ncomp, scalars);
  });
  SFEM_LAUNCH_CHECK();
  return SFEM_OK;
}

int sfem_cg_update_xp_lazy(void* x, void* pring, int64_t ring_stride,
                           const void* z, int64_t count, double* scalars,
                           double* lazy, int m, int dtype,
                           sfem_stream_t stream) {
  SFEM_REQUIRE(count >= 0 && scalars && lazy,
               "sfem_cg_update_xp_lazy: bad arguments");
  SFEM_REQUIRE(m >= 2 && m <= SFEM_CG_LAZY_MAX,
               "sfem_cg_update_xp_lazy: ring of %d directions (2..%d)", m,
               SFEM_CG_LAZY_MAX);
  if (count == 0) return SFEM_OK;
  SFEM_REQUIRE(x && pring && z && ring_stride >= count,
               "sfem_cg_update_xp_lazy: null pointer or ring stride < count");
  SFEM_REQUIRE(dtype == SFEM_F32 || dtype == SFEM_F64,
               "sfem_cg_update_xp_lazy: unknown dtype %d", dtype);
  SFEM_REQUIRE(ring_stride % (dtype == SFEM_F64 ? 2 : 4) == 0,
               "sfem_cg_update_xp_lazy: ring stride must keep 16-byte "
               "alignment");
  DISPATCH_DTYPE(dtype, {
    const int grid = stream_grid(count, 512 * 2);
    if (streams_past_caches(count, sizeof(T)))
      hipLaunchKernelGGL((cg_update_xp_lazy_kernel<T, true>), dim3(grid),
                         dim3(512), 0, as_stream(stream), (T*)x, (T*)pring,
                         ring_stride, (const T*)z, count, scalars, lazy, m);
    else
      hipLaunchKernelGGL((cg_update_xp_lazy_kernel<T, false>), dim3(grid),
                         dim3(512), 0, as_stream(stream), (T*)x, (T*)pring,
                         ring_stride, (const T*)z, count, scalars, lazy, m);
  });
  SFEM_LAUNCH_CHECK();
  return SFEM_OK;
}

int sfem_cg_flush_x(void* x, const void* pring, int64_t ring_stride,
                    int64_t count, const double* scalars, double* lazy, int m,
                    int dtype, sfem_stream_t stream) {
  SFEM_REQUIRE(count >= 0 && scalars && lazy && m >= 2 &&
                   m <= SFEM_CG_LAZY_MAX,
               "sfem_cg_flush_x: bad arguments");
  SFEM_REQUIRE(dtype == SFEM_F32 || dtype == SFEM_F64,
               "sfem_cg_flush_x: unknown dtype %d", dtype);
  if (count > 0) {
    SFEM_REQUIRE(x && pring && ring_stride >= count,
                 "sfem_cg_flush_x: null pointer or ring stride < count");
    DISPATCH_DTYPE(dtype, {
      hipLaunchKernelGGL((cg_flush_x_kernel<T>),
                         dim3(stream_grid(count, 512)), dim3(512), 0,
                         as_stream(stream), (T*)x, (const T*)pring,
                         ring_stride, count, scalars, lazy, m);
    });
  }
  hipLaunchKernelGGL(cg_lazy_mark_kernel, dim3(1), dim3(1), 0,
                     as_stream(stream), scalars, lazy);
  SFEM_LAUNCH_CHECK();
  return SFEM_OK;
}

int sfem_cg_update_r_mean(void* r, const void* ap, const void* w,
                          int64_t count, double* scalars, double* sums,
                          int dtype, sfem_stream_t stream) {
  SFEM_REQUIRE(count >= 0 && scalars && sums,
               "sfem_cg_update_r_mean: bad arguments");
  if (count == 0) return SFEM_OK;
  SFEM_REQUIRE(r && ap && w, "sfem_cg_update_r_mean: null pointer");
  DISPATCH_DTYPE(dtype, {
    const int grid = stream_grid(count, 512 * 2);
    if (streams_past_caches(count, sizeof(T)))
      hipLaunchKernelGGL((cg_update_r_mean_kernel<T, true>), dim3(grid),
                         dim3(512), 0, as_stream(stream), (T*)r, (const T*)ap,
                         (const T*)w, count, scalars, sums);
    else
      hipLaunchKernelGGL((cg_update_r_mean_kernel<T, false>), dim3(grid),
                         dim3(512), 0, as_stream(stream), (T*)r, (const T*)ap,
                         (const T*)w, count, scalars, sums);
  });
  SFEM_LAUNCH_CHECK();
  return SFEM_OK;
}

int sfem_cg_update_xp_mean(void* x, void* p, const void* r, int64_t count,
                           double* scalars, double* sums, double total,
                           int dtype, sfem_stream_t stream) {
  SFEM_REQUIRE(count >= 0 && scalars && sums && total != 0.0,
               "sfem_cg_update_xp_mean: bad arguments");
  if (count == 0) return SFEM_OK;
  SFEM_REQUIRE(x && p && r, "sfem_cg_update_xp_mean: null pointer");
  DISPATCH_DTYPE(dtype, {
    const int grid = stream_grid(count, 512 * 2);
    if (streams_past_caches(count, sizeof(T)))
      hipLaunchKernelGGL((cg_update_xp_mean_kernel<T, true>), dim3(grid),
                         dim3(512), 0, as_stream(stream), (T*)x, (T*)p,
                         (const T*)r, count, scalars, sums, total);
    else
      hipLaunchKernelGGL((cg_update_xp_mean_kernel<T, false>), dim3(grid),
                         dim3(512), 0, as_stream(stream), (T*)x, (T*)p,
                         (const T*)r, count, scalars, sums, total);
  });
  SFEM_LAUNCH_CHECK();
  return SFEM_OK;
}

int sfem_cg_scalars(double* scalars, int phase, double maxiter, double tol,
                    double atol, double* partials, sfem_stream_t stream) {
  SFEM_REQUIRE(scalars && phase >= 0 && phase <= 7 &&
                   (phase < 3 || phase >= 6 || partials),
               "sfem_cg_scalars: bad arguments");
  hipLaunchKernelGGL(cg_scalar_kernel, dim3(1), dim3(256), 0,
                     as_stream(stream), scalars, phase, maxiter, tol, atol,
                     partials, (int64_t)SFEM_DOT_SLOTS, false);
  SFEM_LAUNCH_CHECK();
  return SFEM_OK;
}

int sfem_cg_scalars_n(double* scalars, int phase, double maxiter, double tol,
                      double atol, double* partials, int64_t num_partials,
                      sfem_stream_t stream) {
  SFEM_REQUIRE(scalars && partials && num_partials >= 1 &&
                   (phase == 3 || phase == 4 || phase == 5 || phase == 8),
               "sfem_cg_scalars_n: phases 3, 4, 5, 8 over stored partial sums");
  if (num_partials > 4096) {
    const int64_t chunk = (num_partials + SFEM_FOLD_GROUPS - 1) /
                          SFEM_FOLD_GROUPS;
    hipLaunchKernelGGL(fold_partials_kernel, dim3(SFEM_FOLD_GROUPS), dim3(256),
                       0, as_stream(stream), partials, num_partials, chunk,
                       partials + num_partials);
    partials += num_partials;
    num_partials = SFEM_FOLD_GROUPS;
  }
  hipLaunchKernelGGL(cg_scalar_kernel, dim3(1), dim3(256), 0,
                     as_stream(stream), scalars, phase, maxiter, tol, atol,
                     partials, num_partials, true);
  SFEM_LAUNCH_CHECK();
// ... 17 lines not shown
```

### swirl_fem_amd/csrc/sfem_helmholtz.hip

```cpp
#include <stdlib.h>

#include "sfem_helmholtz_cluster.h"
#include "sfem_helmholtz_mfma.h"
#include "sfem_helmholtz_facet.h"
#include "sfem_helmholtz_adv.h"

namespace sfem {

template <typename T>
__global__ void __launch_bounds__(256)
helmholtz_setup_kernel(const T* __restrict__ invjac,
                       const T* __restrict__ jacdet,
                       const T* __restrict__ weights, T* __restrict__ geo,
                       int64_t num_elements, int d, int Q) {
  const int ng = d * (d + 1) / 2;
  const int64_t total = num_elements * Q;
  const int64_t stride = (int64_t)gridDim.x * blockDim.x;
  for (int64_t t = (int64_t)blockIdx.x * blockDim.x + threadIdx.x; t < total;
       t += stride) {
    const int64_t e = t / Q;
    const int q = (int)(t - e * Q);
    const T* ij = invjac + t * d * d;
    const T wd = weights[q] * jacdet[t];
    T vals[7];
// ... 127 lines not shown
  __syncthreads();
  auto cls = [P](int a) { return a == 0 ? 0 : (a == P - 1 ? 2 : 1); };
  if (lane < 27) {
    const int c[3] = {lane / 9, (lane / 3) % 3, lane % 3};
    int o[3], inner[3];
    bool exists = true;
    for (int d = 0; d < 3; ++d) {
      inner[d] = c[d] == 1;
      o[d] = c[d] == 0 ? 0 : (c[d] == 1 ? 1 : P - 1);
      if (inner[d] && P < 3) exists = false;
    }
    int32_t code = 0, sd[3] = {0, 0, 0};
    if (exists) {
      const int os = (o[0] * P + o[1]) * P + o[2];
      const int32_t id0 = ids[os];
      const int stride[3] = {P * P, P, 1};
      for (int d = 0; d < 3; ++d)
        if (inner[d] && P >= 4) sd[d] = ids[os + stride[d]] - id0;
      if (id0 < 0 || id0 >= num_nodes) {
        atomicOr(&bad, 1);
      } else {
        uint32_t v = (uint32_t)id0;
        if (dirichlet && dirichlet[id0]) v |= SFEM_IDX_DIRICHLET;
        if (multiplicity[id0] > 1) v |= SFEM_IDX_SHARED;
        code = (int32_t)v;
      }
      for (int d = 0; d < 3; ++d)
        if (sd[d] > 0x7FFFFF || sd[d] < -0x7FFFFF) atomicOr(&bad, 1);
    }
    ent[lane][0] = code; ent[lane][1] = sd[0]; ent[lane][2] = sd[1];
    ent[lane][3] = sd[2];
  }
  __syncthreads();
  for (int s = lane; s < n; s += 64) {
    const int a = s / (P * P), i = (s / P) % P, j = s % P;
    const int f = cls(a) * 9 + cls(i) * 3 + cls(j);
    const uint32_t code = (uint32_t)ent[f][0];
    const int32_t pred = (int32_t)(code & SFEM_IDX_MASK) + ent[f][1] * (a - 1) +
                         ent[f][2] * (i - 1) + ent[f][3] * (j - 1);
    const int32_t id = ids[s];
    bool good = id == pred && id >= 0 && id < num_nodes;
    if (good) {
      const bool dir = dirichlet && dirichlet[id];
      const bool sh = multiplicity[id] > 1;
      good = dir == ((code & SFEM_IDX_DIRICHLET) != 0) &&
             sh == ((code & SFEM_IDX_SHARED) != 0);
    }
    if (!good) atomicOr(&bad, 1);
  }
  __syncthreads();
  if (lane < 27) {
    int32_t* dst = tab + e * FACET_ROW + lane * 4;
    for (int q = 0; q < 4; ++q) dst[q] = ent[lane][q];
  }
  if (lane == 0) ok[e] = bad ? 0 : 1;
}

struct HelmholtzCall {
  const void* u; void* out; const int32_t* enc; const void* geo;
  const void* geo_elem; const int32_t* geo_index; const int32_t* elem_list;
  const void* dmat; const void* weights; const void* nodes;
  int64_t num_elements; int ndim, P, ncomp, geo_mode; double l0, l1; bool gs;
  double* dot_out;
  int colored;
  int64_t node_stride, comp_stride;
  const uint16_t* shared_order = nullptr;
  int shared_stride = 0;
  const int32_t* cluster_elems = nullptr;
  const int32_t* cluster_offsets = nullptr;
  const uint32_t* cluster_nodes = nullptr;
  int64_t num_clusters = 0;
  const int32_t* facet_table = nullptr;
  const void* geo_const = nullptr;
  int64_t num_nodes = 0;
  const int32_t* chain_offsets = nullptr;
  const int32_t* chain_elems = nullptr;
  int64_t num_chains = 0;
  int64_t layered_extent = 0;
  int64_t dot_slots = 0;
  const void* kappa = nullptr;
  const void* sigma = nullptr;
  int coef_mode = 0;
  const void* beta = nullptr;
};

template <typename T>
static int run_helmholtz(const HelmholtzCall& c, hipStream_t stream) {
  HelmholtzParams<T> prm{};
  prm.u = (const T*)c.u; prm.out = (T*)c.out; prm.enc = c.enc;
  prm.geo = (const T*)c.geo; prm.geo_elem = (const T*)c.geo_elem;
  prm.geo_index = c.geo_index; prm.geo_mode = c.geo_mode;
  prm.dmat_host = (const T*)c.dmat; prm.weights_host = (const T*)c.weights;
  prm.nodes_host = (const T*)c.nodes; prm.num_elements = c.num_elements;
  prm.elem_list = c.elem_list; prm.ncomp = c.ncomp;
  prm.node_stride = c.node_stride > 0 ? c.node_stride : c.ncomp;
  prm.comp_stride = c.node_stride > 0 ? c.comp_stride : 1;
  prm.comp = 0; prm.lambda0 = (T)c.l0; prm.lambda1 = (T)c.l1;
  prm.dot_out = c.dot_out;
  prm.colored = c.colored;
  prm.shared_order = c.shared_order;
  prm.shared_stride = c.shared_stride;
  if (c.beta) {
    HelmholtzAdvParams<T> ap{};
    static_cast<HelmholtzParams<T>&>(ap) = prm;
    ap.dot_out = nullptr;
    ap.shared_order = nullptr;
    ap.kappa = (const T*)c.kappa;
    ap.sigma = (const T*)c.sigma;
    ap.beta = (const T*)c.beta;
    if (c.ndim == 3) return dispatch_helmholtz_adv<T, 3>(ap, c.P, c.gs, stream);
    return dispatch_helmholtz_adv<T, 2>(ap, c.P, c.gs, stream);
  }
  if (c.coef_mode != COEF_NONE) {
    HelmholtzCoefParams<T> cp{};
    static_cast<HelmholtzParams<T>&>(cp) = prm;
    cp.kappa = (const T*)c.kappa;
    cp.sigma = (const T*)c.sigma;
    cp.coef_mode = c.coef_mode;
    if (c.ndim == 3) return dispatch_helmholtz_coef<T, 3>(cp, c.P, c.gs, stream);
    return dispatch_helmholtz_coef<T, 2>(cp, c.P, c.gs, stream);
  }
  if (c.cluster_elems) {
    ClusterParams<T> cl{c.cluster_elems, c.cluster_offsets, c.cluster_nodes,
                        c.num_clusters};
    return dispatch_helmholtz_cluster<T>(prm, cl, c.P, stream);
  }
  if (c.facet_table) {
    FacetParams<T> fp{};
    fp.u = prm.u; fp.out = prm.out; fp.tab = c.facet_table;
    fp.geo_const = (const T*)c.geo_const; fp.geo_elem = prm.geo_elem;
    fp.geo = prm.geo; fp.geo_index = prm.geo_index;
    fp.elem_list = prm.elem_list; fp.comp_stride = prm.comp_stride;
    fp.ncomp = prm.ncomp; fp.lambda0 = prm.lambda0; fp.lambda1 = prm.lambda1;
    fp.dot_out = prm.dot_out;
    fp.chain_off = c.chain_offsets;
    fp.chain_elems = c.chain_elems;
    fp.layered = c.layered_extent > 0;
    fp.dot_slots = c.dot_slots;
    if (fp.layered)
      return dispatch_helmholtz_facet<T>(
          fp, c.P, c.geo_mode,
          c.chain_offsets ? c.num_chains : c.num_elements, c.layered_extent,
          prm.dmat_host, prm.weights_host, prm.nodes_host, stream);
    if (c.chain_offsets && c.ncomp > 1) {
      for (int k = 0; k < c.ncomp; ++k) {
        FacetParams<T> fk = fp;
        fk.u = prm.u + (int64_t)k * prm.comp_stride;
        fk.out = prm.out + (int64_t)k * prm.comp_stride;
        fk.ncomp = 1;
        const int rc = dispatch_helmholtz_facet<T>(
            fk, c.P, c.geo_mode, c.num_chains, c.num_nodes, prm.dmat_host,
            prm.weights_host, prm.nodes_host, stream);
        if (rc != SFEM_OK) return rc;
      }
      return SFEM_OK;
    }
    return dispatch_helmholtz_facet<T>(fp, c.P, c.geo_mode,
                                       c.chain_offsets ? c.num_chains
                                                       : c.num_elements,
                                       c.num_nodes, prm.dmat_host,
                                       prm.weights_host, prm.nodes_host,
                                       stream);
  }
  if constexpr (sizeof(T) == 4) {
    const char* v = getenv("SFEM_MFMA");
    const bool mfma_on = v && v[0] == '1';
    if (mfma_on && helmholtz_mfma_applies(prm, c.P, c.ndim, c.gs))
      return launch_helmholtz_mfma_p12(prm, stream);
  }
  if (c.ndim == 3) return dispatch_helmholtz<T, 3>(prm, c.P, c.gs, stream);
  if (c.ndim == 2) return dispatch_helmholtz<T, 2>(prm, c.P, c.gs, stream);
  set_error("helmholtz: ndim=%d (fused kernel supports 2 and 3)", c.ndim);
  return SFEM_EUNSUPPORTED;
}

static int check_coefficients(const char* who, const sfem_helmholtz_args* a) {
  if (a->coef_mode == SFEM_COEF_NONE) return SFEM_OK;
  SFEM_REQUIRE(a->coef_mode == SFEM_COEF_ELEM || a->coef_mode == SFEM_COEF_POINT,
               "%s: unknown coef_mode %d", who, a->coef_mode);
  SFEM_REQUIRE(a->kappa || a->sigma,
               "%s: coef_mode %d needs kappa or sigma", who, a->coef_mode);
  SFEM_REQUIRE(a->ncomp == 1, "%s: coefficients take scalar fields", who);
  SFEM_REQUIRE(a->ndim == 2 || a->ndim == 3, "%s: coefficients need ndim 2 or 3",
               who);
  SFEM_REQUIRE(a->geo_mode == SFEM_GEO_AFFINE ||
                   a->geo_mode == SFEM_GEO_MULTILINEAR,
               "%s: coefficients need affine or multilinear elements (fold "
               "them into the stored factors of curved ones)", who);
  SFEM_REQUIRE(!a->cluster_elems && !a->facet_table && !a->shared_order &&
                   !a->layered_extent,
               "%s: coefficients run on index rows (no cluster, facet, "
               "layered or sorted assembly)", who);
  return SFEM_OK;
}

static int check_advection(const char* who, const sfem_helmholtz_args* a) {
  if (!a->beta) return SFEM_OK;
  const char* why = nullptr;
  if (a->ncomp != 1) why = "a vector field";
  else if (a->ndim != 2 && a->ndim != 3) why = "ndim other than 2 or 3";
  else if (a->geo_mode == SFEM_GEO_BOX) why = "SFEM_GEO_BOX";
  else if (a->cluster_elems || a->facet_table || a->shared_order ||
           a->layered_extent || a->chain_offsets)
    why = "cluster, facet, chain, layered or sorted assembly";
  else if (a->dot_out) why = "dot_out";
  else if (a->coef_mode == SFEM_COEF_ELEM)
    why = "per-element coefficients (expand them per point)";
  else if (a->coef_mode != SFEM_COEF_NONE && a->geo_mode == SFEM_GEO_POINT)
    why = "coefficient arrays on stored factors (fold them in)";
  else if (a->node_stride > 1) why = "a strided field";
  if (why) {
    set_error("%s: the advective term (beta) does not take %s", who, why);
    return SFEM_EUNSUPPORTED;
  }
  return SFEM_OK;
}

static int check_geometry(const char* who, int geo_mode, const void* geo,
                          const void* geo_elem, const void* weights,
                          const void* nodes) {
  if (geo_mode == SFEM_GEO_POINT) {
// ... 112 lines not shown
  }
  if (a->num_elements == 0) return SFEM_OK;
  SFEM_REQUIRE(a->u && (a->enc || a->facet_table) && a->dmat,
               "sfem_helmholtz_apply: null pointer");
  SFEM_REQUIRE(a->geo_mode != SFEM_GEO_BOX || a->facet_table,
               "sfem_helmholtz_apply: SFEM_GEO_BOX needs a facet table");
  int rc = check_geometry("sfem_helmholtz_apply", a->geo_mode, a->geo,
                          a->geo_elem, a->weights, a->nodes);
  if (rc) return rc;
  rc = check_advection("sfem_helmholtz_apply", a);
  if (rc) return rc;
  rc = check_coefficients("sfem_helmholtz_apply", a);
  if (rc) return rc;
  const int64_t work = a->elem_list ? a->num_listed : a->num_elements;
  SFEM_REQUIRE(work >= 0 && work <= a->num_elements,
               "sfem_helmholtz_apply: bad element list length");
  if (work == 0) return SFEM_OK;
  HelmholtzCall c{a->u, a->out, a->enc, a->geo, a->geo_elem, a->geo_index,
                  a->elem_list, a->dmat, a->weights, a->nodes, work, a->ndim,
                  a->P, a->ncomp, a->geo_mode, a->lambda0, a->lambda1, true,
                  a->dot_out, a->colored, a->node_stride, a->comp_stride,
                  a->shared_order, a->shared_stride};
  c.kappa = a->kappa;
  c.sigma = a->sigma;
  c.coef_mode = a->coef_mode;
  c.beta = a->beta;
  SFEM_REQUIRE(!a->shared_order || (a->shared_stride > 0 &&
                                    a->shared_stride <= 0xFFFF),
               "sfem_helmholtz_apply: bad shared_stride");
  if (a->cluster_elems) {
    SFEM_REQUIRE(a->ndim == 3 && a->P >= 4 && a->P <= 8,
                 "sfem_helmholtz_apply: cluster assembly is 3D, P = 4..8");
    SFEM_REQUIRE(a->cluster_offsets && a->cluster_nodes && a->num_clusters > 0,
                 "sfem_helmholtz_apply: incomplete cluster description");
    SFEM_REQUIRE(!a->colored && !a->shared_order,
                 "sfem_helmholtz_apply: clusters exclude colored / "
                 "shared_order");
    c.cluster_elems = a->cluster_elems;
    c.cluster_offsets = a->cluster_offsets;
    c.cluster_nodes = a->cluster_nodes;
    c.num_clusters = a->num_clusters;
  }
  if (a->facet_table) {
    SFEM_REQUIRE(a->ndim == 3 && facet_supported_p(a->P),
                 "sfem_helmholtz_apply: facet tables are 3D, P = 6..12");
    SFEM_REQUIRE(!a->colored && !a->cluster_elems,
                 "sfem_helmholtz_apply: facet tables exclude colored / "
                 "cluster assembly");
    SFEM_REQUIRE(a->ncomp == 1 || a->node_stride == 1,
                 "sfem_helmholtz_apply: facet tables need node_stride = 1");
    SFEM_REQUIRE(a->geo_const || (a->geo_mode != SFEM_GEO_AFFINE &&
                                  a->geo_mode != SFEM_GEO_BOX),
                 "sfem_helmholtz_apply: affine / box facet applies need "
                 "geo_const");
    c.facet_table = a->facet_table;
    c.geo_const = a->geo_const;
    c.num_nodes = a->num_nodes;
    if (a->layered_extent) {
      SFEM_REQUIRE(a->layered_extent >= a->num_nodes &&
                       a->layered_extent <= SFEM_IDX_MASK,
                   "sfem_helmholtz_apply: layered_extent must cover the "
                   "nodal values and stay below 2^30");
      SFEM_REQUIRE(a->ncomp == 1 && a->zero_end == a->zero_begin,
                   "sfem_helmholtz_apply: layered assembly takes scalar "
                   "fields and clears nothing");
      c.layered_extent = a->layered_extent;
      SFEM_REQUIRE(a->dot_slots >= 0, "sfem_helmholtz_apply: negative dot_slots");
      c.dot_slots = a->dot_slots;
    } else {
      SFEM_REQUIRE(a->dot_slots == 0,
                   "sfem_helmholtz_apply: dot_slots goes with layered "
                   "assembly");
    }
    if (a->chain_offsets) {
      SFEM_REQUIRE(a->chain_elems && a->num_chains > 0 &&
                       (a->ncomp == 1 || a->node_stride == 1),
                   "sfem_helmholtz_apply: chains need chain_elems, "
                   "num_chains > 0 and a scalar or component-major field");
      c.chain_offsets = a->chain_offsets;
      c.chain_elems = a->chain_elems;
      c.num_chains = a->num_chains;
    }
  }
  SFEM_REQUIRE(!a->layered_extent || a->facet_table,
               "sfem_helmholtz_apply: layered assembly needs a facet table");
  if (a->dtype == SFEM_F64) return run_helmholtz<double>(c, as_stream(stream));
  return run_helmholtz<float>(c, as_stream(stream));
}

int sfem_kernarg_selftest(int32_t* bad, sfem_stream_t stream) {
  SFEM_REQUIRE(bad, "sfem_kernarg_selftest: null pointer");
  hipStream_t st = as_stream(stream);
  launch_kernarg_probe<FacetParams<double>, SMat<double, 8>>(bad, st);
  launch_kernarg_probe<FacetParams<double>, DMat<double, 8>>(bad, st);
  launch_kernarg_probe<FacetParams<float>, DMat<float, 12>>(bad, st);
  launch_kernarg_probe<FacetParams<float>, SMat<float, 12>>(bad, st);
  SFEM_LAUNCH_CHECK();
  return SFEM_OK;
}

int sfem_facet_table_build(const int32_t* elements, const uint8_t* dirichlet,
                           const int32_t* multiplicity, int32_t* table,
                           uint8_t* ok, int64_t num_elements,
                           int64_t num_nodes, int P, sfem_stream_t stream) {
  SFEM_REQUIRE(num_elements >= 0 && num_nodes >= 0 && P >= 2 && P <= 12,
               "sfem_facet_table_build: bad sizes");
  if (num_elements == 0) return SFEM_OK;
  SFEM_REQUIRE(elements && multiplicity && table && ok,
               "sfem_facet_table_build: null pointer");
  SFEM_REQUIRE(num_elements <= 0x7fffffff,
               "sfem_facet_table_build: too many elements");
  hipLaunchKernelGGL(facet_table_kernel, dim3((unsigned)num_elements), dim3(64),
                     0, as_stream(stream), elements, dirichlet, multiplicity,
                     table, ok, num_elements, num_nodes, P);
  SFEM_LAUNCH_CHECK();
  return SFEM_OK;
}

int sfem_helmholtz_setup_affine(const void* geo_elem, void* geo_const,
                                int64_t num_elements, double box_tol,
                                int dtype, sfem_stream_t stream) {
  SFEM_REQUIRE(num_elements >= 0, "sfem_helmholtz_setup_affine: bad sizes");
  if (num_elements == 0) return SFEM_OK;
  SFEM_REQUIRE(geo_elem && geo_const,
               "sfem_helmholtz_setup_affine: null pointer");
  const unsigned grid = (unsigned)((num_elements + 255) / 256);
  if (dtype == SFEM_F64)
    hipLaunchKernelGGL(helmholtz_setup_affine_kernel<double>, dim3(grid),
                       dim3(256), 0, as_stream(stream),
                       (const double*)geo_elem, (double*)geo_const,
                       num_elements, box_tol);
  else if (dtype == SFEM_F32)
    hipLaunchKernelGGL(helmholtz_setup_affine_kernel<float>, dim3(grid),
                       dim3(256), 0, as_stream(stream), (const float*)geo_elem,
                       (float*)geo_const, num_elements, (float)box_tol);
  else {
    set_error("sfem_helmholtz_setup_affine: unknown dtype %d", dtype);
    return SFEM_EINVAL;
  }
  SFEM_LAUNCH_CHECK();
  return SFEM_OK;
}

int sfem_helmholtz_cluster_limits(int P, int dtype, int* cluster_size,
                                  int* max_shared) {
  SFEM_REQUIRE(cluster_size && max_shared,
               "sfem_helmholtz_cluster_limits: null pointer");
  int rc;
  if (dtype == SFEM_F64) rc = cluster_limits<double>(P, cluster_size, max_shared);
  else if (dtype == SFEM_F32) rc = cluster_limits<float>(P, cluster_size, max_shared);
  else {
    set_error("sfem_helmholtz_cluster_limits: unknown dtype %d", dtype);
    return SFEM_EINVAL;
  }
  if (rc) set_error("sfem_helmholtz_cluster_limits: P=%d outside 4..8", P);
  return rc;
}

int sfem_helmholtz_setup_multilinear(const void* elem_coords, void* geo_elem,
                                     int64_t num_elements, int ndim, int P,
                                     int dtype, sfem_stream_t stream) {
  SFEM_REQUIRE(num_elements >= 0 && (ndim == 2 || ndim == 3) && P >= 2 &&
                   P <= SFEM_MAX_P,
               "sfem_helmholtz_setup_multilinear: bad sizes");
  if (num_elements == 0) return SFEM_OK;
  SFEM_REQUIRE(elem_coords && geo_elem,
// ... 53 lines not shown
```

### swirl_fem_amd/csrc/sfem_helmholtz_facet.h

```cpp
#pragma once
#include <stdlib.h>

#include "sfem_helmholtz.h"

namespace sfem {

constexpr int GEO_BOX = 5;
constexpr int FACET_ROW = 27 * 4;

template <typename T>
struct FacetParams {
  const T* u;
  T* out;
  const int32_t* tab;
  const T* geo_const;
  const T* geo_elem;
  const T* geo;
  const int32_t* geo_index;
  const int32_t* elem_list;
  const int32_t* chain_off;
  const int32_t* chain_elems;
  int64_t comp_stride;
  int ncomp;
  T lambda0, lambda1;
  double* dot_out;
  int layered;
  int64_t dot_slots;
};

constexpr uint32_t FACET_SKIP = 0x40000000u;

template <int P>
struct FacetLayout {
  static constexpr int B = P >= 9 ? (P | 1) : P;
  static constexpr int A = P == 8 ? 67 : (P == 7 ? 52 : P * B);
  static constexpr bool SWAP = P == 8;
  static constexpr int WORDS = (P - 1) * (A + B + 1) + 1;
  static constexpr int COPY = (WORDS + 3) & ~3;
  static constexpr int TPE = P * P;
  static constexpr int WAVES = (TPE + 63) / 64;
  static constexpr int BLOCK = 64 * WAVES;
  __host__ __device__ static constexpr int word(int x, int y, int z) {
    return A * x + B * y + z;
  }
};

template <int P>
__device__ __forceinline__ void facet_sync() {
  if (FacetLayout<P>::WAVES == 1) wave_sync();
  else lds_barrier();
}

template <int P>
struct FacetSlots {
  uint16_t s[FacetLayout<P>::BLOCK][6];
};

template <int P>
constexpr FacetSlots<P> make_facet_slots() {
  using L = FacetLayout<P>;
  FacetSlots<P> t{};
  for (int l = 0; l < L::BLOCK; ++l)
    for (int q = 0; q < 6; ++q) t.s[l][q] = 0xFFFF;
  constexpr int M = P - 2, NF = M * M;
  static_assert(NF + 2 * M + 8 <= L::TPE, "rounds must fit the element's lanes");
  int edges[12][3] = {};
  int ne = 0;
  for (int d = 2; d >= 0; --d)
    for (int pp = 0; pp < 2; ++pp)
      for (int r = 0; r < 2; ++r) {
        int c[3] = {0, 0, 0};
        c[d] = -1;
        c[(d + 1) % 3] = pp ? P - 1 : 0;
        c[(d + 2) % 3] = r ? P - 1 : 0;
        for (int k = 0; k < 3; ++k) edges[ne][k] = c[k];
        ++ne;
      }
  for (int q = 0; q < 6; ++q) {
    const int d = q / 2, fixed = (q & 1) ? P - 1 : 0;
    for (int l = 0; l < NF; ++l) {
      const int x = l / M + 1, y = l % M + 1;
      int c[3] = {0, 0, 0};
      c[d] = fixed;
      c[(d + 1) % 3] = d == 1 ? y : x;
      c[(d + 2) % 3] = d == 1 ? x : y;
      t.s[l][q] = (uint16_t)L::word(c[0], c[1], c[2]);
    }
    for (int h = 0; h < 2; ++h)
      for (int z = 0; z < M; ++z) {
        int c[3] = {0, 0, 0};
        for (int k = 0; k < 3; ++k)
          c[k] = edges[2 * q + h][k] < 0 ? z + 1 : edges[2 * q + h][k];
        t.s[NF + h * M + z][q] = (uint16_t)L::word(c[0], c[1], c[2]);
      }
  }
  for (int v = 0; v < 8; ++v)
    t.s[NF + 2 * M + v][0] = (uint16_t)L::word(
        (v & 4) ? P - 1 : 0, (v & 2) ? P - 1 : 0, (v & 1) ? P - 1 : 0);
  return t;
}

template <int P>
__device__ const FacetSlots<P> g_facet_slots = make_facet_slots<P>();

template <typename T, int P>
struct SMat {
  static constexpr int PH = P / 2, PC = P - P / 2;
  T e[PC * PC];
  T o[PH * PH > 0 ? PH * PH : 1];
  T w[P];
// ... 612 lines not shown
    } else {
#pragma unroll
      for (int a = 0; a < P; ++a)
        acc[a] = MASS ? (Wm * sym_w<T, P>(sm, a)) * ua[a] : T(0);
    }
  }
};

template <typename T, int P, typename ELEM, bool SCALAR, bool OFF32,
          bool LAY = false>
__global__ void __launch_bounds__(FacetLayout<P>::BLOCK, ELEM::MINW)
helmholtz_facet_kernel(FacetParams<T> prm, typename ELEM::Mat dm) {
  using L = FacetLayout<P>;
  using Mat = typename ELEM::Mat;
  using KA = FacetKernarg<FacetParams<T>, Mat>;
  static_assert(!LAY || SCALAR, "layered assembly takes scalar fields");
  __shared__ T lds[ELEM::LDS_WORDS];
  T* s0 = lds;
  uint32_t* codes = reinterpret_cast<uint32_t*>(lds + L::COPY);

  FacetWave<P> w;
  w.init();
  const uint32_t work = blockIdx.x;
  const int64_t e = prm.elem_list ? (int64_t)prm.elem_list[work]
                                  : (int64_t)work;
  const Mat* kdm = reinterpret_cast<const Mat*>(kernarg_bytes() + KA::MAT_OFF);

  FacetLane<P, LAY> fl;
  fl.load(prm.tab, e, w.i, w.j);
  ELEM el;
  {
    typename ELEM::Raw raw;
    ELEM::fetch(raw, prm, e);
    el.finish(raw, prm, dm, kdm, w, w.template wij<T>(kdm));
  }

  const int nc = SCALAR ? 1 : prm.ncomp;
  double udot = 0.0;
  for (int k = 0; k < nc; ++k) {
    const T* ug = prm.u + (SCALAR ? 0 : k * prm.comp_stride);
    T* og = prm.out + (SCALAR ? 0 : k * prm.comp_stride);
    T ua[P], acc[P];
    if (w.ok) {
#pragma unroll
      for (int a = 0; a < P; ++a) {
        ua[a] = *facet_node<const T, OFF32>(ug, fl.code(a));
      }
    } else {
#pragma unroll
      for (int a = 0; a < P; ++a) ua[a] = T(0);
    }
    el.apply(prm, dm, w, lds, ua, acc);
    if (w.ok)
      facet_scatter_head<T, P, LAY>(fl, acc, ua, prm.dot_out != nullptr, udot);
    if constexpr (LAY && !ELEM::LAYERED_SLOTS) {
      facet_store_layered<T, P, OFF32>(fl, acc, og, w.ok);
    } else {
      uint16_t slots[6];
#pragma unroll
      for (int q = 0; q < 6; ++q) slots[q] = g_facet_slots<P>.s[w.lane][q];
      if constexpr (LAY)
        facet_store_layered_slots<T, P, OFF32>(
            fl, slots, acc, og, s0, codes, w.own_w, w.ok,
            FacetLane<P>::cls(w.i) == 1 && FacetLane<P>::cls(w.j) == 1);
      else
        facet_scatter_tail<T, P, OFF32>(fl, slots, acc, og, s0, codes, w.own_w,
                                        w.ok);
      facet_sync<P>();
    }
  }
  if (prm.dot_out) {
#pragma unroll
    for (int off = 32; off > 0; off >>= 1) udot += __shfl_down(udot, off, 64);
    if ((w.lane & 63) == 0) {
      const int64_t wave = (int64_t)blockIdx.x * L::WAVES + (w.lane >> 6);
      if (LAY && prm.dot_slots > 0)
        prm.dot_out[wave] = udot;
      else
        unsafeAtomicAdd(&prm.dot_out[wave & (SFEM_DOT_SLOTS - 1)], udot);
    }
  }
}

template <typename T, int P, typename ELEM, bool OFF32, bool LAY = false>
__global__ void __launch_bounds__(FacetLayout<P>::BLOCK, ELEM::CHAIN_MINW)
helmholtz_chain_kernel(FacetParams<T> prm, typename ELEM::Mat dm) {
  using L = FacetLayout<P>;
  using Mat = typename ELEM::Mat;
  using KA = FacetKernarg<FacetParams<T>, Mat>;
  using FL = FacetLane<P, LAY>;
  __shared__ T lds[ELEM::LDS_WORDS];
  T* s0 = lds;
  uint32_t* codes = reinterpret_cast<uint32_t*>(lds + L::COPY);

  FacetWave<P> w;
  w.init();
  const uint32_t seg = blockIdx.x;
  const int32_t k0 = prm.chain_off[seg];
  const int32_t k1 = prm.chain_off[seg + 1];
  const Mat* kdm = reinterpret_cast<const Mat*>(kernarg_bytes() + KA::MAT_OFF);
  constexpr bool OWN_ORDER = LAY && !ELEM::LAYERED_SLOTS;
  uint16_t slots[OWN_ORDER ? 1 : 6];
  if constexpr (!OWN_ORDER) {
#pragma unroll
    for (int q = 0; q < 6; ++q) slots[q] = g_facet_slots<P>.s[w.lane][q];
  }
  const bool face_inner = FL::cls(w.i) == 1 && FL::cls(w.j) == 1;
  const T* ug = prm.u;
  T* og = prm.out;

  const T wij = w.template wij<T>(kdm);
  double udot = 0.0;
  T carry = T(0);
  {
  FL fl, fn;
  typename FL::Raw traw;
  typename ELEM::Raw graw;
  fl.load(prm.tab, (int64_t)prm.chain_elems[k0], w.i, w.j);
  fn = fl;
  ELEM::fetch(graw, prm, (int64_t)prm.chain_elems[k0]);
  T ua[P];
#pragma unroll
  for (int a = 0; a < P; ++a)
    ua[a] = w.ok ? *facet_node<const T, OFF32>(ug, fl.code(a)) : T(0);
  if (k0 + 1 < k1)
    FL::issue(traw, prm.tab, (int64_t)prm.chain_elems[k0 + 1], w.i, w.j);
  for (int32_t k = k0; k < k1; ++k) {
    const bool has_pred = k > k0, has_succ = k + 1 < k1;
    ELEM el;
    el.finish(graw, prm, dm, kdm, w, wij);
    if (has_succ) {
      fn.finish(traw, w.i, w.j);
      ELEM::fetch(graw, prm, (int64_t)prm.chain_elems[k + 1]);
    }
    T acc[P];
    el.apply(prm, dm, w, lds, ua, acc);
    if (has_pred) acc[0] += carry;
    carry = acc[P - 1];
    FL fe = fl;
    if constexpr (LAY) {
      if (has_succ) fe.to[2] |= FACET_SKIP | SFEM_IDX_DIRICHLET;
    } else {
      if (has_pred && face_inner) fe.t[0] &= ~(uint32_t)SFEM_IDX_SHARED;
      if (has_succ) fe.t[2] |= SFEM_IDX_SHARED | SFEM_IDX_DIRICHLET;
    }
    const T u_last = ua[P - 1];
    if (w.ok)
      facet_scatter_head<T, P, LAY>(fe, acc, ua, prm.dot_out != nullptr, udot);
    fl = fn;
    if (has_succ) {
      ua[0] = u_last;
#pragma unroll
      for (int a = 1; a < P; ++a)
        ua[a] = w.ok ? *facet_node<const T, OFF32>(ug, fl.code(a)) : T(0);
      if (k + 2 < k1)
        FL::issue(traw, prm.tab, (int64_t)prm.chain_elems[k + 2], w.i, w.j);
    }
    if constexpr (OWN_ORDER) {
      facet_store_layered<T, P, OFF32>(fe, acc, og, w.ok);
    } else {
      if constexpr (LAY)
        facet_store_layered_slots<T, P, OFF32>(fe, slots, acc, og, s0, codes,
                                               w.own_w, w.ok, face_inner);
      else
        facet_scatter_tail<T, P, OFF32>(fe, slots, acc, og, s0, codes, w.own_w,
                                        w.ok);
      facet_sync<P>();
    }
  }
  }
  if (prm.dot_out) {
#pragma unroll
    for (int off = 32; off > 0; off >>= 1) udot += __shfl_down(udot, off, 64);
    if ((w.lane & 63) == 0) {
      const int64_t wave = (int64_t)blockIdx.x * L::WAVES + (w.lane >> 6);
      if (LAY && prm.dot_slots > 0)
        prm.dot_out[wave] = udot;
      else
        unsafeAtomicAdd(&prm.dot_out[wave & (SFEM_DOT_SLOTS - 1)], udot);
    }
  }
}

template <typename T, int P, typename ELEM>
int launch_facet_elem(const FacetParams<T>& prm, const typename ELEM::Mat& mat,
                      unsigned groups, bool off32, hipStream_t stream) {
  const dim3 grid(groups), block(FacetLayout<P>::BLOCK);
  if (prm.layered) {
    if (prm.ncomp != 1) {
      set_error("helmholtz (facet): layered assembly takes scalar fields");
      return SFEM_EINVAL;
    }
    if (prm.chain_off) {
      if constexpr (ELEM::CHAINS) {
        if (off32)
          hipLaunchKernelGGL((helmholtz_chain_kernel<T, P, ELEM, true, true>),
                             grid, block, 0, stream, prm, mat);
        else
          hipLaunchKernelGGL((helmholtz_chain_kernel<T, P, ELEM, false, true>),
                             grid, block, 0, stream, prm, mat);
      } else {
        set_error("helmholtz (facet): no chain kernel for this geometry at "
                  "P=%d", P);
        return SFEM_EUNSUPPORTED;
      }
    } else if (off32) {
      hipLaunchKernelGGL(
          (helmholtz_facet_kernel<T, P, ELEM, true, true, true>), grid, block,
          0, stream, prm, mat);
    } else {
      hipLaunchKernelGGL(
          (helmholtz_facet_kernel<T, P, ELEM, true, false, true>), grid, block,
          0, stream, prm, mat);
    }
    return SFEM_OK;
  }
  if (prm.chain_off) {
    if constexpr (ELEM::CHAINS) {
      if (off32)
        hipLaunchKernelGGL((helmholtz_chain_kernel<T, P, ELEM, true>), grid,
                           block, 0, stream, prm, mat);
      else
        hipLaunchKernelGGL((helmholtz_chain_kernel<T, P, ELEM, false>), grid,
                           block, 0, stream, prm, mat);
    } else {
      set_error("helmholtz (facet): no chain kernel for this geometry at P=%d",
                P);
      return SFEM_EUNSUPPORTED;
    }
  } else if (prm.ncomp == 1) {
    if (off32)
      hipLaunchKernelGGL((helmholtz_facet_kernel<T, P, ELEM, true, true>),
                         grid, block, 0, stream, prm, mat);
    else
      hipLaunchKernelGGL((helmholtz_facet_kernel<T, P, ELEM, true, false>),
                         grid, block, 0, stream, prm, mat);
  } else {
    if (off32)
      hipLaunchKernelGGL((helmholtz_facet_kernel<T, P, ELEM, false, true>),
                         grid, block, 0, stream, prm, mat);
    else
      hipLaunchKernelGGL((helmholtz_facet_kernel<T, P, ELEM, false, false>),
                         grid, block, 0, stream, prm, mat);
  }
  return SFEM_OK;
}

template <typename T, int P>
int launch_helmholtz_facet(const FacetParams<T>& prm, int geo_mode,
                           int64_t groups, int64_t field_reals,
                           const T* dmat, const T* weights, const T* nodes,
                           hipStream_t stream) {
  if (groups > 0x7fffffff) {
    set_error("helmholtz (facet): too many workgroups (%lld)",
              (long long)groups);
    return SFEM_EINVAL;
  }
  if (prm.chain_off && prm.ncomp != 1) {
    set_error("helmholtz (facet): chain launches take scalar fields");
    return SFEM_EINVAL;
  }
  const unsigned g = (unsigned)groups;
  if (prm.dot_out && prm.layered && prm.dot_slots > 0 &&
      groups * FacetLayout<P>::WAVES > prm.dot_slots) {
    set_error("helmholtz (facet): %lld waves but %lld dot slots",
              (long long)(groups * FacetLayout<P>::WAVES),
              (long long)prm.dot_slots);
    return SFEM_EINVAL;
  }
  const bool mass = prm.lambda0 != T(0);
  const char* force64 = getenv("SFEM_FACET_OFF64");
  const bool off32 = (uint64_t)field_reals * sizeof(T) < ((uint64_t)1 << 32) &&
                     !(force64 && force64[0] == '1');
  int rc = SFEM_OK;
  if (geo_mode == GEO_BOX) {
    const SMat<T, P> sm = make_smat<T, P>(dmat, weights);
    if (mass) rc = launch_facet_elem<T, P, BoxElem<T, P, true>>(prm, sm, g,
                                                                off32, stream);
    else rc = launch_facet_elem<T, P, BoxElem<T, P, false>>(prm, sm, g, off32,
                                                            stream);
  } else {
    const DMat<T, P> dm = make_dmat<T, P>(dmat, weights, nodes);
#define SFEM_FACET_GM(GMV)                                                    \
// ... 83 lines not shown
```

### swirl_fem_amd/linalg/cg.py

```python

from __future__ import annotations

import os

import torch

from swirl_fem_amd import switches
from swirl_fem_amd import _lib
from swirl_fem_amd import _ops
from swirl_fem_amd.core import layout


def _leaves(t):
  if isinstance(t, dict):
    return [l for k in sorted(t) for l in _leaves(t[k])]
  if isinstance(t, (list, tuple)):
    return [l for x in t for l in _leaves(x)]
  return [t]


def _map(f, *ts):
  t0 = ts[0]
  if isinstance(t0, dict):
    return {k: _map(f, *[t[k] for t in ts]) for k in t0}
# ... 1 lines not shown
    return type(t0)(_map(f, *xs) for xs in zip(*ts))
  return f(*ts)


def _as_vec(t):
  if not isinstance(t, torch.Tensor):
    raise TypeError(f'cg operates on device tensors, got {type(t)}')
  return t


MAX_KEPT_RUNNERS = 6
LAZY_X_MIN_BYTES = 1 << 28
RR_PARTIALS = 1 << 16
RESIDUAL_STOP_GROUPS = 512


def _lazy_min_bytes():
  mb = switches.get('SFEM_LAZY_X_MIN_MB')
  return LAZY_X_MIN_BYTES if mb is None else int(float(mb) * (1 << 20))


class _Scalars:
  GAMMA, PAP, GAMMA_NEW, ALPHA, BETA, BB, ATOL2, DONE, ITERS = range(9)
  STATUS = 10

  def __init__(self, device):
    self.t = torch.zeros(_lib.SFEM_CG_NSCALARS, dtype=torch.float64,
                         device=device)
    self.partials = torch.zeros(_lib.SFEM_DOT_SLOTS, dtype=torch.float64,
                                device=device)

  def interface_correction(self, slot, a, b, interface):
    idx, w = interface
    if idx.numel() == 0:
      return
    for x, y in zip(_leaves(a), _leaves(b)):
      _ops.dot_indexed(x, layout.like(y, x), idx, w, self.t, slot, -1.0)

  def dot_into(self, slot, a, b, dot_fn, reduce_fn, interface=None):
    la, lb = _leaves(a), _leaves(b)
    if dot_fn is None:
      first = True
      for x, y in zip(la, lb):
        _ops.dot(layout.flat(x), layout.flat(layout.like(y, x)), self.t, slot,
                 accumulate=not first)
        first = False
    else:
      total = sum(dot_fn(x, y) for x, y in zip(la, lb))
      self.t[slot] = torch.as_tensor(total, dtype=torch.float64,
                                     device=self.t.device)
    if interface is not None:
      self.interface_correction(slot, a, b, interface)
    if reduce_fn is not None:
      reduce_fn(self.t[slot:slot + 1])


class CGRunner:

  def __init__(self, A, b, x0=None, *, tol=1e-5, atol=0.0, maxiter=None,
               M=None, dot_fn=None, reduce_fn=None, interface=None):
    if interface is not None and (
        dot_fn is not None or
        (M is not None and not getattr(M, 'consistent', False))):
      raise ValueError('interface weights apply to the plain dot of consistent '
                       'vectors (M = None or a preconditioner that maps '
                       'consistent vectors to consistent ones, dot_fn = None)')
    b_leaves = [_as_vec(l) for l in _leaves(b)]
    if not all(l.is_cuda for l in b_leaves):
      raise RuntimeError('swirl_fem_amd.linalg.cg runs on MI355X device '
                         'tensors (there is no CPU fallback)')
    self.A, self.M, self.dot_fn, self.reduce_fn = A, M, dot_fn, reduce_fn
    self.interface = interface
    self.tol, self.atol = tol, atol
    if maxiter is None:
      maxiter = 10 * sum(l.numel() for l in b_leaves)
    self.maxiter = maxiter
    device = b_leaves[0].device
    dense = lambda t: t if (t.is_contiguous() or
                            layout.is_component_major(t)) else t.contiguous()
    b = _map(dense, b)
    self._x = (_map(torch.zeros_like, b) if x0 is None
               else _map(lambda t, bb: layout.like(t, bb).clone(), x0, b))
    self.lazy = None
    self.s = s = _Scalars(device)
    S = _Scalars
    self.identity_m = M is None
    s.dot_into(S.BB, b, b, dot_fn, reduce_fn, interface)
    self.r = _map(lambda bb, ax: bb - layout.like(ax, bb), b, A(self._x))
    z = self.r if self.identity_m else M(self.r)
    self._p = _map(lambda t, rr: layout.like(t, rr).clone(), z, self.r)
    s.dot_into(S.GAMMA, self.r, z, dot_fn, reduce_fn, interface)
    self.fused_dot = (dot_fn is None and hasattr(A, 'apply_with_dot') and
                      isinstance(self._p, torch.Tensor))
    self.parts = s.partials if self.fused_dot else None
    _ops.cg_scalars(s.t, 2, maxiter, tol, atol, self.parts)
    self.fuse_rr = self.identity_m and dot_fn is None
    self.rr_stop = None
    if (getattr(M, 'stops_on_residual', False) and dot_fn is None and
        isinstance(self.r, torch.Tensor) and self.r.dim() == 1):
      self._residual_stop_setup(A, b, z)
    if self.fuse_rr:
      self.fuse_rr = 2
    self.fold_rr = self.fuse_rr == 2 and (reduce_fn is not None or
                                          interface is not None)
    self.mean = None
    probe = getattr(M, 'mean_projection', None)
    if (probe is not None and self.rr_stop is None and dot_fn is None and reduce_fn is None and
        interface is None and isinstance(self.r, torch.Tensor) and
        switches.get('SFEM_FUSED_MEAN') != '0'):
      found = probe()
      if found is not None:
        w, total = found
        self.mean = (layout.flat(layout.like(w.to(self.r.dtype), self.r)),
                     float(total),
                     torch.zeros(_lib.SFEM_CG_MEAN_SUMS, dtype=torch.float64,
                                 device=device))
    self.jacobi = None
    probe = getattr(M, 'jacobi_diagonal', None)
    if (probe is not None and self.mean is None and self.rr_stop is None and
        dot_fn is None and
        (interface is not None or reduce_fn is None) and
        isinstance(self.r, torch.Tensor) and
        switches.get('SFEM_FUSED_JACOBI') != '0'):
      dinv = probe()
      dinv = None if dinv is None else dinv.to(self.r.dtype).contiguous()
      n = -1 if dinv is None else dinv.numel()
      vn = 16 // self.r.element_size()
      if self.r.dim() == 1 or (self.r.dim() == 2 and self.r.shape[1] == 1 and
                               self.r.is_contiguous()):
        ncomp = 1
      elif (self.r.dim() == 2 and layout.is_component_major(self.r) and
            self._p.stride() == self.r.stride() and n % vn == 0):
        ncomp = self.r.shape[1]
      else:
        ncomp = None
      if ncomp is not None and self.r.shape[0] == n:
        self.jacobi = (dinv, ncomp)
    self.jacobi_interface = None
    if self.jacobi is not None and interface is not None:
      idx, w = interface
      self.jacobi_interface = (
          idx, (w * self.jacobi[0][idx].double()).contiguous())
    self.layered = None
    if (self.fused_dot and self.mean is None and self.rr_stop is None and
        self._p.dim() == 1 and
        hasattr(A, 'apply_layered_with_dot')):
      self.layered = A.layer_plan()
    self.det = None
    if (self.layered is not None and reduce_fn is None and interface is None
        and switches.get('SFEM_DETERMINISTIC') != '0'):
      pad = _lib.SFEM_FOLD_GROUPS
      self.det = (torch.zeros(A.layered_dot_slots() + pad, dtype=torch.float64,
                              device=device),
                  torch.zeros(RR_PARTIALS + pad, dtype=torch.float64,
                              device=device))
      self._reproducible_start(b, z)
    m = int(switches.get('SFEM_LAZY_X'))
    if (m >= 2 and self.mean is None and self.jacobi is None and
        self.rr_stop is None and
        isinstance(self._p, torch.Tensor) and
        self._p.is_contiguous() and
        self._p.numel() * self._p.element_size() >= _lazy_min_bytes()):
      m = min(m, _lib.SFEM_CG_LAZY_MAX)
      n = self._p.numel()
      ring = torch.empty((m, (n + 3) // 4 * 4), dtype=self._p.dtype,
                         device=device)
      ring[0, :n] = self._p.reshape(-1)
      self._p = None
      self.lazy = (ring, n, torch.zeros(1 + _lib.SFEM_CG_LAZY_MAX,
                                        dtype=torch.float64, device=device))
      self._shape = tuple(self.r.shape)
    self.issued = 0
    self._graph = None
    self._capture_failed = False

  def _residual_stop_setup(self, A, b, z):
    dev = self.r.device
    G = RESIDUAL_STOP_GROUPS
    layered = None
    if (hasattr(A, 'apply_layered_with_dot') and hasattr(A, 'layer_plan') and
        self.reduce_fn is None and self.interface is None):
      layered = A.layer_plan()
    waves = A.layered_dot_slots() if layered is not None else 0
    self.rr_stop = dict(
        groups=G, layered=layered,
        parts=torch.zeros(2 * G, dtype=torch.float64, device=dev),
        waves=torch.zeros(waves + _lib.SFEM_FOLD_GROUPS, dtype=torch.float64,
                          device=dev), num_waves=waves)
    self.fused_dot = False
    self.parts = None
    self._residual_stop_start(b, z)

  def _residual_stop_start(self, b, z):
    st = self.rr_stop
    G, parts = st['groups'], st['parts']
    args = (self.maxiter, self.tol, self.atol)
    self._dot2(b, b, None)
    _ops.pmg_cg_scalars(self.s.t, 3, parts, G, *args)
    self._dot2(self.r, self.r, layout.like(z, self.r).contiguous())
    _ops.pmg_cg_scalars(self.s.t, 2, parts, G, *args)

  def _dot2(self, a, b, c):
    st = self.rr_stop
    G, parts = st['groups'], st['parts']
    _ops.pmg_dot2(a, b, c, parts, G)
    if self.interface is not None:
      idx, w = self.interface
      if idx.numel():
        _ops.dot_indexed(a, b, idx, w, parts, 0, -1.0)
        if c is not None:
          _ops.dot_indexed(a, c, idx, w, parts, G, -1.0)
    if self.reduce_fn is not None:
      self.reduce_fn(parts[:G if c is None else 2 * G])

  def _step_residual_stop(self):
    s, st = self.s, self.rr_stop
    G, parts = st['groups'], st['parts']
    args = (self.maxiter, self.tol, self.atol)
    if st['layered'] is not None:
      Ap = self.A.apply_layered_with_dot(self.p, st['waves'], per_wave=True)
      _ops.pmg_cg_scalars(s.t, 0, st['waves'], st['num_waves'], *args)
      _ops.cg_update_r_layered(self.r, Ap, st['layered'].layers, s.t, 0,
                               masks=st['layered'].masks)
    else:
      Ap = layout.like(self.A(self.p), self.r).contiguous()
      self._dot2(self.p, Ap, None)
      _ops.pmg_cg_scalars(s.t, 0, parts, G, *args)
      _ops.cg_update_r(self.r, Ap, s.t, 0)
    z = layout.like(self.M(self.r), self.r).contiguous()
    self._dot2(self.r, self.r, z)
    _ops.pmg_cg_scalars(s.t, 4, parts, G, *args)
    _ops.cg_update_xp(self._x, self.p, z, s.t)
    _ops.pmg_cg_scalars(s.t, 1, parts, G, *args)
    self.issued += 1

  def _reproducible_start(self, b, z):
    s, S = self.s, _Scalars
    tree = lambda u, v: (u.double() * v.double()).sum()
    s.t[S.BB] = tree(b, b)
    s.t[S.GAMMA] = tree(self.r, z)
    _ops.cg_scalars(s.t, 2, self.maxiter, self.tol, self.atol, self.parts)

  @property
  def vector_passes(self):
    if self.jacobi is not None:
      return 10
    if self.lazy is None:
      return 8
    m = self.lazy[0].shape[0]
    return 3 + (4 * m + 1) / m

  @property
  def p(self):
    if self.lazy is None:
      return self._p
    ring, n, _ = self.lazy
    return ring[self.issued % ring.shape[0], :n].view(self._shape)

  @property
  def x(self):
    if self.lazy is not None:
      self._flush()
      ring, n, state = self.lazy
      _ops.cg_flush_x(layout.flat(self._x), ring, self.s.t, state)
    return self._x

  def matches(self, b, tol, atol, maxiter) -> bool:
    mine, theirs = _leaves(self.r), _leaves(b)
    if len(mine) != len(theirs) or (tol, atol) != (self.tol, self.atol):
      return False
    if maxiter is None:
      maxiter = 10 * sum(l.numel() for l in theirs)
    if maxiter != self.maxiter:
      return False
    return all(isinstance(t, torch.Tensor) and t.shape == m.shape and
               t.dtype == m.dtype and t.device == m.device and
               (t.stride() == m.stride() or t.is_contiguous())
               for m, t in zip(mine, theirs))

  def restart(self, b, x0=None):
    s, S = self.s, _Scalars
    if x0 is None:
      _map(lambda xx: xx.zero_(), self._x)
    else:
      _map(lambda xx, t: xx.copy_(layout.like(t, xx)), self._x, x0)
    self.issued = 0
    if self.lazy is not None:
      self.lazy[2].zero_()
    s.dot_into(S.BB, b, b, self.dot_fn, self.reduce_fn, self.interface)
    _map(lambda rr, bb, ax: rr.copy_(layout.like(bb, rr) - layout.like(ax, rr)),
         self.r, b, self.A(self._x))
    z = self.r if self.identity_m else self.M(self.r)
    if z is not self.r:
      _map(lambda pp, zz: pp.copy_(layout.like(zz, pp)), self.p, z)
    else:
      _map(lambda pp, rr: pp.copy_(rr), self.p, self.r)
    s.dot_into(S.GAMMA, self.r, z, self.dot_fn, self.reduce_fn, self.interface)
    _ops.cg_scalars(s.t, 2, self.maxiter, self.tol, self.atol, self.parts)
    if self.det is not None:
      self._reproducible_start(b, z)
    if self.rr_stop is not None:
      self._residual_stop_start(b, z)
    if self.mean is not None:
      self.mean[2].zero_()
    self.issued = 0

  def step(self):
    if self._graph is not None:
      self._graph.replay()
      self.issued += 1
      return
    self._step_eager()

  def _step_eager(self):
    if self.rr_stop is not None:
      self._step_residual_stop()
      return
    s, S = self.s, _Scalars
    A, M, dot_fn, reduce_fn = self.A, self.M, self.dot_fn, self.reduce_fn
    args = (self.maxiter, self.tol, self.atol, self.parts)
    merged = self.fused_dot and reduce_fn is None
    if self.fused_dot and self.det is not None:
      Ap = A.apply_layered_with_dot(self.p, self.det[0], per_wave=True)
      _ops.cg_scalars_n(s.t, 5, self.maxiter, self.tol, self.atol,
                        self.det[0],
                        self.det[0].numel() - _lib.SFEM_FOLD_GROUPS)
    elif self.fused_dot:
      Ap = (A.apply_layered_with_dot(self.p, s.partials)
            if self.layered is not None
            else A.apply_with_dot(self.p, s.partials))
      _ops.cg_scalars(s.t, 5 if merged else 3, *args)
      if reduce_fn is not None:
        reduce_fn(s.t[S.PAP:S.PAP + 1])
    else:
      Ap = A(self.p)
    if self.fused_dot:
      pass
    elif dot_fn is None:
      for xx, yy in zip(_leaves(self.p), _leaves(Ap)):
        _ops.dot(layout.flat(xx), layout.flat(layout.like(yy, xx)), s.t,
                 S.PAP, accumulate=True)
      if self.interface is not None:
        s.interface_correction(S.PAP, self.p, Ap, self.interface)
      if reduce_fn is not None:
        reduce_fn(s.t[S.PAP:S.PAP + 1])
    else:
      s.dot_into(S.PAP, self.p, Ap, dot_fn, reduce_fn)
    if not merged:
      _ops.cg_scalars(s.t, 0, *args)
    if self.mean is not None:
      w, total, sums = self.mean
      _ops.cg_update_r_mean(layout.flat(self.r),
                            layout.flat(layout.like(Ap, self.r)), w, s.t, sums)
      _ops.cg_update_xp_mean(layout.flat(self._x), layout.flat(self.p),
                             layout.flat(self.r), s.t, sums, total)
      if not merged:
        _ops.cg_scalars(s.t, 1, *args)
      self.issued += 1
      return
    if self.jacobi is not None:
      self._jacobi_updates(Ap, merged, args)
      return
    if self.layered is not None and self.det is not None and self.fuse_rr:
      n = _ops.cg_update_r_layered_det(
          self.r, Ap, self.layered.layers, s.t,
          self.det[1][:RR_PARTIALS], masks=self.layered.masks)
      _ops.cg_scalars_n(s.t, 8, self.maxiter, self.tol, self.atol,
                        self.det[1], n)
    elif self.layered is not None:
      _ops.cg_update_r_layered(self.r, Ap, self.layered.layers, s.t,
                               self.fuse_rr, masks=self.layered.masks)
    else:
      for rr, aa in zip(_leaves(self.r), _leaves(Ap)):
        _ops.cg_update_r(layout.flat(rr), layout.flat(layout.like(aa, rr)),
                         s.t, self.fuse_rr)
    if self.fuse_rr:
      z = self.r
      if self.fold_rr:
        _ops.cg_scalars(s.t, 7, *args)
      if self.interface is not None:
        s.interface_correction(S.GAMMA_NEW, self.r, self.r, self.interface)
      if reduce_fn is not None:
        reduce_fn(s.t[S.GAMMA_NEW:S.GAMMA_NEW + 1])
    else:
      if (dot_fn is None and hasattr(M, 'apply_with_dot') and
          isinstance(self.r, torch.Tensor)):
        z = M.apply_with_dot(self.r, s.t, S.GAMMA_NEW)
        if self.interface is not None:
          s.interface_correction(S.GAMMA_NEW, self.r, z, self.interface)
        if reduce_fn is not None:
          reduce_fn(s.t[S.GAMMA_NEW:S.GAMMA_NEW + 1])
      elif dot_fn is None:
        z = self.r if self.identity_m else M(self.r)
        for xx, yy in zip(_leaves(self.r), _leaves(z)):
          _ops.dot(layout.flat(xx), layout.flat(layout.like(yy, xx)), s.t,
                   S.GAMMA_NEW, accumulate=True)
        if self.interface is not None:
          s.interface_correction(S.GAMMA_NEW, self.r, z, self.interface)
        if reduce_fn is not None:
          reduce_fn(s.t[S.GAMMA_NEW:S.GAMMA_NEW + 1])
      else:
        z = self.r if self.identity_m else M(self.r)
        s.dot_into(S.GAMMA_NEW, self.r, z, dot_fn, reduce_fn)
    if self.lazy is not None:
      ring, n, state = self.lazy
      _ops.cg_update_xp_lazy(layout.flat(self._x), ring,
                             layout.flat(layout.like(z, self.r)), s.t, state)
    else:
      for xx, pp, zz in zip(_leaves(self._x), _leaves(self.p), _leaves(z)):
        _ops.cg_update_xp(layout.flat(xx), layout.flat(pp),
                          layout.flat(layout.like(zz, pp)), s.t)
    if not merged:
      _ops.cg_scalars(s.t, 1, *args)
    self.issued += 1

  def _jacobi_updates(self, Ap, merged, args):
    s = self.s
    dinv, ncomp = self.jacobi
    if self.layered is not None:
      plan = self.layered
      if self.det is not None:
        n = _ops.cg_update_r_jacobi(self.r, Ap, dinv, s.t, 1, plan.layers,
                                    plan.masks, self.det[1][:RR_PARTIALS])
        _ops.cg_scalars_n(s.t, 8, self.maxiter, self.tol, self.atol,
                          self.det[1], n)
      else:
        _ops.cg_update_r_jacobi(self.r, Ap, dinv, s.t, 1, plan.layers,
                                plan.masks)
    else:
      _ops.cg_update_r_jacobi(layout.flat(self.r),
                              layout.flat(layout.like(Ap, self.r)), dinv, s.t,
                              ncomp)
    if self.reduce_fn is not None:
      _ops.cg_scalars(s.t, 7, *args)
      if self.jacobi_interface is not None:
        s.interface_correction(_Scalars.GAMMA_NEW, self.r, self.r,
                               self.jacobi_interface)
      self.reduce_fn(s.t[_Scalars.GAMMA_NEW:_Scalars.GAMMA_NEW + 1])
    _ops.cg_update_xp_jacobi(layout.flat(self._x), layout.flat(self.p),
                             layout.flat(self.r), dinv, s.t, ncomp)
    if not merged:
      _ops.cg_scalars(s.t, 1, *args)
    self.issued += 1

  def capture(self) -> bool:
    if self._graph is not None:
      return True
    if self.reduce_fn is not None:
      return False
    if self.lazy is not None:
      if self.issued:
        return False
      ring, n, _ = self.lazy
      self._p = ring[0, :n].view(self._shape).clone()
      self.lazy = None
    self.step()
    torch.cuda.synchronize()
    graph = torch.cuda.CUDAGraph()
    issued = self.issued
    import gc
    gc.collect()
    was_enabled = gc.isenabled()
    gc.disable()
    try:
      with torch.cuda.graph(graph):
        self._step_eager()
    except Exception:
      torch.cuda.synchronize()
      self.issued = issued
      self._capture_failed = True
      return False
    finally:
      if was_enabled:
        gc.enable()
    self.issued = issued
    self._graph = graph
    return True

  def _flush(self):
    if self.fused_dot and self.reduce_fn is None:
      _ops.cg_scalars(self.s.t, 6, self.maxiter, self.tol, self.atol, None)

  def done(self) -> bool:
    self._flush()
    return bool(self.s.t[_Scalars.DONE].item() != 0.0)

  def info(self):
    self._flush()
    scal = self.s.t.cpu()
    status = _lib.CG_STATUS.get(int(scal[_Scalars.STATUS].item()), 'unknown')
    if status == 'running' and self.issued >= self.maxiter:
      status = 'maxiter'
    return {'residual': self.s.t[_Scalars.GAMMA].clone(),
            'num_iterations': int(scal[_Scalars.ITERS].item()),
            'status': status}


def cg(A, b, x0=None, *, tol=1e-5, atol=0.0, maxiter=None, M=None,
       dot_fn=None, reduce_fn=None, interface=None, check_every=16,
       graph=False, workspace=None, key=None):
  if not _leaves(b):
    return b, {'residual': 0.0, 'num_iterations': 0, 'status': 'converged'}
  reuse = (graph and workspace is not None and key is not None and
           dot_fn is None and reduce_fn is None and interface is None)
  run = workspace.get(key) if reuse else None
  if run is not None and run.matches(b, tol, atol, maxiter):
    workspace[key] = workspace.pop(key)
    run.restart(b, x0)
  else:
    run = CGRunner(A, b, x0, tol=tol, atol=atol, maxiter=maxiter, M=M,
                   dot_fn=dot_fn, reduce_fn=reduce_fn, interface=interface)
    if reuse:
      workspace.pop(key, None)
      workspace[key] = run
      while len(workspace) > MAX_KEPT_RUNNERS:
        workspace.pop(next(iter(workspace)))
  if (graph and dot_fn is None and run.maxiter > 2 and run._graph is None and
      not run._capture_failed and not run.done()):
    run.capture()
  while run.issued < run.maxiter:
    for _ in range(min(check_every, run.maxiter - run.issued)):
      run.step()
    if run.done():
      break
  info = run.info()
  if info['status'].startswith('breakdown'):
    import warnings
    warnings.warn(f"cg stopped with status '{info['status']}' after "
                  f"{info['num_iterations']} iterations: x is the last "
                  'iterate, not a solution to the requested tolerance',
                  RuntimeWarning, stacklevel=2)
  return (_map(lambda t: t.clone(), run.x) if reuse else run.x), info


class _SymmetricSolve(torch.autograd.Function):

  @staticmethod
  def forward(ctx, b, A, kwargs, info_out):
# ... 15 lines not shown
```

### swirl_fem_amd/switches.py

```python

from __future__ import annotations

import os
import warnings

SWITCHES = {
    'SFEM_LIB': (None, '_lib.py',
                 'path of another build of libsfem_hip.so (kernel A/B runs, '
                 '`scripts/build_variant.sh`)'),
    'SFEM_HDF5_LIB': (None, 'niles/datagen/h5lite.py',
                      'path of the HDF5 C library for snapshot files when '
                      'h5py is not installed'),
    'SFEM_FACET': ('1', 'core/operators.py',
                   '0: 3D P = 6..12 operators keep their index rows instead '
                   'of the compact facet tables'),
    'SFEM_BOX': ('1', 'core/operators.py',
                 '0: Cartesian elements run the general affine kernels'),
    'SFEM_CHAIN': ('1', 'core/operators.py, _ops.py',
                   '0: one element per wave instead of chain segments'),
    'SFEM_CHAIN_LEN': (None, 'core/operators.py',
                       'elements per chain segment (default: 8 on large '
                       'meshes, shorter on small ones, '
                       '`operators.chain_segment_length`)'),
    'SFEM_CHAIN_HI': ('0', 'core/operators.py',
                      '1: chains also for P >= 9 box / affine elements '
                      '(slower: measured 1.73 vs 1.47 ms at p = 11)'),
    'SFEM_CHAIN_VECTOR': ('1', '_ops.py',
                          '0: component-major vector fields are not walked '
                          'as chains'),
    'SFEM_LAYERED': ('1', 'core/operators.py',
                     '0: CG keeps the atomic assembly; force: layered '
                     'assembly also for elements with stored factors'),
    'SFEM_DETERMINISTIC': ('1', 'linalg/cg.py',
                           '0: with layered assembly the two inner products '
                           'of a CG iteration still accumulate their partial '
                           'sums with atomics (not bitwise reproducible; one '
                           'scalar launch less per iteration)'),
    'SFEM_LAZY_X': ('4', 'linalg/cg.py',
                    'directions the CG keeps before it adds them to x '
                    '(vectors of 256 MB and more; 0 or 1: x += alpha p every '
                    'iteration)'),
    'SFEM_LAZY_X_MIN_MB': (None, 'linalg/cg.py',
                           'smallest vector (MiB) that gets the lazy x update '
                           '(default 256; the tests set 0)'),
    'SFEM_SORTED_SCATTER': ('1', 'core/operators.py',
                            '0: index-row kernels issue their atomics in slot '
                            'order instead of node order'),
    'SFEM_CLUSTER': ('0', 'core/operators.py',
                     "1: assembly='auto' means cluster assembly (slower)"),
    'SFEM_INTERP': ('1', 'the library (getenv per launch)',
                    '0: values-only sfem_basis_eval / sfem_basis_eval_t run '
                    'the generic kernels instead of the compile-time-sized '
                    'interpolation (csrc/sfem_interp.h)'),
    'SFEM_MFMA': ('0', '_ops.py and the library (getenv per launch)',
                  '1: p = 11 fp32 index-row elements run the matrix-core '
                  'kernel (slower: 1.25 vs 1.0 ms)'),
    'SFEM_FACET_OFF64': ('0', 'the library (getenv per launch)',
                         '1: facet kernels form 64-bit addresses even for '
                         'fields below 4 GiB (tests)'),
    'SFEM_STOKES_FACET': ('1', 'core/operators.py',
                          '0: Stokes div / grad_t keep their index rows'),
    'SFEM_STOKES_FACET_DIV': ('box', 'core/operators.py',
                              'all: the divergence walks chains on every '
                              'geometry, not only on box elements (tests)'),
    'SFEM_SPLIT_E': ('0', 'navier_stokes/navier_stokes.py',
                     '1: pressure operator E in two fused halves '
                     '(`sfem_stokes_e_first/second`)'),
    'SFEM_STOKES_LAYERED': ('auto', 'navier_stokes/navier_stokes.py',
                            'pressure operator E on index-row kernels: D^T '
                            'with one position per writer instead of atomics '
                            '(`StokesDivGrad.e_layered`); auto = 2D meshes, '
                            '1 = 3D index rows too, 0 = never'),
    'SFEM_FUSED_DOTS': ('1', 'navier_stokes/navier_stokes.py',
                        '0: the pressure CG computes p.Ep and r.Mr with '
                        'separate dot kernels'),
    'SFEM_FUSED_MEAN': ('1', 'linalg/cg.py',
                        '0: the mean projection of the pressure '
                        'preconditioner is applied as a separate kernel'),
    'SFEM_FUSED_JACOBI': ('1', 'linalg/cg.py',
                          '0: a Jacobi preconditioner (`linalg/jacobi.py`) is '
                          'called as a function and z = M r stored, instead '
                          'of being folded into the two CG vector updates'),
    'SFEM_GRAPHS': ('1', 'navier_stokes/navier_stokes.py',
                    '0: solver iterations are never replayed as HIP graphs'),
    'SFEM_GRAPH_REUSE': ('1', 'navier_stokes/navier_stokes.py',
                         '0: a recorded iteration is not kept across solves'),
    'SFEM_GRAPH_MAX_NUMEL': (str(1 << 25), 'navier_stokes/navier_stokes.py',
                             'largest vector (entries) whose solves are '
                             'replayed as graphs'),
    'SFEM_PRESSURE_PC': ('projection', 'examples/navier_stokes_driver.py',
                         "pressure preconditioner of the drivers: 'projection' "
                         "(the reference's nullspace projection) or 'schwarz' "
                         '(element-wise fast diagonalisation + piecewise-'
                         'constant coarse level, '
                         'navier_stokes/pressure_preconditioner.py)'),
    'SFEM_VELOCITY_PC': ('exchange', 'navier_stokes/navier_stokes.py',
                         "preconditioner of the stepper's Helmholtz solve: "
                         "'exchange' (the reference's M = QQ^T) or 'mass' "
                         '(inverse assembled lumped mass, scaled so that the '
                         "reference's stopping rule still holds) or 'jacobi' "
                         '(inverse assembled diagonal of the whole Helmholtz '
                         'operator, same scaling)'),
    'SFEM_PC_FUSED': ('1', 'navier_stokes/pressure_preconditioner.py',
                      "0: the 'schwarz' preconditioner forms the element sums, "
                      'the coarse correction and the mean removal in separate '
                      'passes'),
    'SFEM_PC_COARSE_ITERS': (None, 'navier_stokes/pressure_preconditioner.py',
                             'Chebyshev steps of the coarse solve inside the '
                             "'schwarz' preconditioner (default: from the "
                             'spectrum bounds, ~ sqrt(kappa) ln(200) / 2)'),
    'SFEM_PRESSURE_PROJECTION': ('0', 'navier_stokes/navier_stokes.py',
                                 'number of earlier pressure increments the '
                                 'steppers project the next pressure solve '
                                 'onto (successive right-hand sides; 0 = off: '
                                 "every solve starts from zero as in the "
                                 'reference)'),
    'SFEM_TEST_FULL_N': ('64', 'tests/', 'elements per direction of the '
                         'full-size property tests'),
    'SFEM_TEST_P11_N': ('64', 'tests/', 'the same for the p = 11 block'),
}

_checked = False


def check_environment() -> list:
  global _checked
  stray = sorted(k for k in os.environ
# ... 41 lines not shown
```

Before: 65.39.

## Spread lazy CG x-update over rider workgroups inside layered operator applies

The lazy x update normally accumulates pending direction terms and applies them in one bulk pass every m-th iteration. This change adds one extra ring slot and rider workgroups to the layered chain Helmholtz kernel. Each rider streams a rotating slice of x and folds in the pending ring terms while the operator apply runs, so the x traffic overlaps with compute instead of forming a periodic bandwidth-bound pass. It costs extra ring memory, extra workgroups that compete for the apply's bandwidth, and more complex flush bookkeeping.

Measured after the change: 60.28. -7.8%, worse.

```diff
diff --git a/include/sfem.h b/include/sfem.h
--- a/include/sfem.h
+++ b/include/sfem.h
@@ -7,7 +7,7 @@
 extern "C" {
 #endif
 
-#define SFEM_ABI_VERSION 9
+#define SFEM_ABI_VERSION 10
 
 enum { SFEM_F32 = 0, SFEM_F64 = 1 };
 enum {
@@ -102,6 +102,20 @@
                          const int32_t* multiplicity,
                          const uint8_t* slot_shared, int32_t* enc,
                          int64_t count, sfem_stream_t stream);
+
+typedef struct sfem_cg_rider {
+  void* x;
+  const void* ring;
+  int64_t ring_stride;
+  int64_t begin, end;
+  const double* lazy;
+  const double* scalars;
+  int64_t iteration;
+  int32_t ring_slots;
+  int32_t lag;
+  int32_t riders;
+  int32_t slice;
+} sfem_cg_rider;
 
 typedef struct sfem_helmholtz_args {
   const void* u;
@@ -144,6 +158,7 @@
   int64_t layered_extent;
   int64_t dot_slots;
   const void* beta;
+  const sfem_cg_rider* rider;
   const void* kappa;
   const void* sigma;
   int32_t coef_mode;
@@ -257,11 +272,12 @@
 #define SFEM_CG_LAZY_MAX 8
 int sfem_cg_update_xp_lazy(void* x, void* pring, int64_t ring_stride,
                            const void* z, int64_t count, double* scalars,
-                           double* lazy, int m, int dtype,
+                           double* lazy, int m, int ride, int dtype,
                            sfem_stream_t stream);
 int sfem_cg_flush_x(void* x, const void* pring, int64_t ring_stride,
                     int64_t count, const double* scalars, double* lazy, int m,
-                    int dtype, sfem_stream_t stream);
+                    int ride, int64_t part_len, int64_t issued, int dtype,
+                    sfem_stream_t stream);
 #define SFEM_MAX_LAYERS 15
 #define SFEM_LAYER_CHUNK 512
 int sfem_cg_update_r_layered(void* r, const void* ap_ext, int64_t count,
diff --git a/swirl_fem_amd/_lib.py b/swirl_fem_amd/_lib.py
--- a/swirl_fem_amd/_lib.py
+++ b/swirl_fem_amd/_lib.py
@@ -8,7 +8,7 @@
 
 _HERE = os.path.dirname(os.path.abspath(__file__))
 LIB_PATH = switches.get('SFEM_LIB') or os.path.join(_HERE, 'libsfem_hip.so')
-ABI_VERSION = 9
+ABI_VERSION = 10
 
 SFEM_F32, SFEM_F64 = 0, 1
 SFEM_CG_NSCALARS_NAMED = 16
@@ -34,6 +34,15 @@
                               ctypes.c_void_p)
 
 
+class CgRider(ctypes.Structure):
+  _fields_ = [
+      ('x', c_ptr), ('ring', c_ptr), ('ring_stride', c_i64), ('begin', c_i64),
+      ('end', c_i64), ('lazy', c_ptr), ('scalars', c_ptr),
+      ('iteration', c_i64), ('ring_slots', c_i32), ('lag', c_i32),
+      ('riders', c_i32), ('slice', c_i32),
+  ]
+
+
 class HelmholtzArgs(ctypes.Structure):
   _fields_ = [
       ('u', c_ptr), ('out', c_ptr), ('enc', c_ptr), ('geo', c_ptr),
@@ -51,6 +60,7 @@
       ('chain_offsets', c_ptr), ('chain_elems', c_ptr), ('num_chains', c_i64),
       ('layered_extent', c_i64), ('dot_slots', c_i64),
       ('beta', c_ptr),
+      ('rider', ctypes.POINTER(CgRider)),
       ('kappa', c_ptr), ('sigma', c_ptr), ('coef_mode', c_i32),
   ]
 
@@ -169,9 +179,9 @@
                                      c_ptr, c_ptr, c_ptr, c_ptr, c_i64, c_ptr,
                                      c_i32, c_ptr],
     'sfem_cg_update_xp_lazy': [c_ptr, c_ptr, c_i64, c_ptr, c_i64, c_ptr, c_ptr,
-                               c_i32, c_i32, c_ptr],
+                               c_i32, c_i32, c_i32, c_ptr],
     'sfem_cg_flush_x': [c_ptr, c_ptr, c_i64, c_i64, c_ptr, c_ptr, c_i32, c_i32,
-                        c_ptr],
+                        c_i64, c_i64, c_i32, c_ptr],
     'sfem_cg_update_r_mean': [c_ptr, c_ptr, c_ptr, c_i64, c_ptr, c_ptr, c_i32,
                               c_ptr],
     'sfem_cg_update_xp_mean': [c_ptr, c_ptr, c_ptr, c_i64, c_ptr, c_ptr, c_dbl,
diff --git a/swirl_fem_amd/_ops.py b/swirl_fem_amd/_ops.py
--- a/swirl_fem_amd/_ops.py
+++ b/swirl_fem_amd/_ops.py
@@ -426,7 +426,7 @@
 
 def _helmholtz_args(u, out, enc, part, host, ndim, P, num_elements, num_nodes,
                     lambda0, lambda1, zero_range, dot_out=None,
-                    layered_extent=0, dot_slots=0):
+                    layered_extent=0, dot_slots=0, rider=None):
   vec = u.dim() != (1 if enc is not None else 2)
   ncomp = u.shape[-1] if vec else 1
   node_stride = comp_stride = 0
@@ -475,7 +475,8 @@
       layered_extent=int(layered_extent), dot_slots=int(dot_slots),
       kappa=_dptr(part.get('kappa')), sigma=_dptr(part.get('sigma')),
       coef_mode=int(part.get('coef_mode', _lib.COEF_NONE)),
-      beta=_dptr(part.get('beta')))
+      beta=_dptr(part.get('beta')),
+      rider=None if rider is None else ctypes.pointer(rider))
 
 
 _CLUSTER_LIMITS = {}
@@ -564,9 +565,39 @@
   return out
 
 
+def cg_ride_part_len(n, m, dtype):
+  vn = 16 // torch.empty((), dtype=dtype).element_size()
+  return -(-(-(-n // vn)) // m) * vn
+
+
+def cg_rider(x, pring, scalars, lazy, iteration, riders=0, slice_len=0):
+  _dev(x, pring, scalars, lazy)
+  m = pring.shape[0] - 1
+  n = x.numel()
+  length = cg_ride_part_len(n, m, x.dtype)
+  q = iteration % m
+  return _lib.CgRider(
+      x=_ptr(x), ring=_ptr(pring), ring_stride=pring.stride(0),
+      begin=min(q * length, n), end=min((q + 1) * length, n),
+      lazy=_ptr(lazy), scalars=_ptr(scalars), iteration=int(iteration),
+      ring_slots=m + 1, lag=m, riders=int(riders), slice=int(slice_len))
+
+
+def layered_rider_part(parts):
+  for n, part in enumerate(parts):
+    if part.get('layered_chains') and part.get('chains') is not None:
+      return n
+  return None
+
+
 def helmholtz_apply_layered(u, ext, enc, parts, host, ndim, P, lambda0,
-                            lambda1, dot_out=None, per_wave=False):
+                            lambda1, dot_out=None, per_wave=False, rider=None):
   dev = _dev(enc)
+  carrier = None
+  if rider is not None:
+    carrier = layered_rider_part(parts)
+    if carrier is None:
+      raise ValueError('riders go with a layered chain launch')
   if u.dim() != 1 or not u.is_contiguous() or not ext.is_contiguous():
     raise ValueError('layered assembly takes contiguous scalar fields')
   if ext.dtype != u.dtype:
@@ -583,7 +614,8 @@
       args = _helmholtz_args(u, ext, enc, part, host, ndim, P, enc.shape[0],
                              u.shape[0], lambda0, lambda1, (0, 0), dots,
                              layered_extent=ext.numel(),
-                             dot_slots=0 if waves is None else waves[n])
+                             dot_slots=0 if waves is None else waves[n],
+                             rider=rider if n == carrier else None)
       if waves is not None:
         at += waves[n]
       _lib.check(_lib.load().sfem_helmholtz_apply(ctypes.byref(args),
@@ -1089,22 +1121,25 @@
         _dtype_code(r), _stream(dev)), 'sfem_cg_update_r')
 
 
-def cg_update_xp_lazy(x, pring, z, scalars, lazy):
+def cg_update_xp_lazy(x, pring, z, scalars, lazy, ride=False):
   dev = _dev(x, pring, z, scalars, lazy)
   with torch.cuda.device(dev):
     _lib.check(_lib.load().sfem_cg_update_xp_lazy(
         _ptr(x), _ptr(pring), pring.stride(0), _ptr(z), x.numel(),
-        _ptr(scalars), _ptr(lazy), pring.shape[0], _dtype_code(x),
-        _stream(dev)), 'sfem_cg_update_xp_lazy')
-
-
-def cg_flush_x(x, pring, scalars, lazy):
+        _ptr(scalars), _ptr(lazy), pring.shape[0] - int(bool(ride)),
+        int(bool(ride)), _dtype_code(x), _stream(dev)),
+        'sfem_cg_update_xp_lazy')
+
+
+def cg_flush_x(x, pring, scalars, lazy, ride=False, issued=0):
   dev = _dev(x, pring, scalars, lazy)
+  m = pring.shape[0] - int(bool(ride))
   with torch.cuda.device(dev):
     _lib.check(_lib.load().sfem_cg_flush_x(
         _ptr(x), _ptr(pring), pring.stride(0), x.numel(), _ptr(scalars),
-        _ptr(lazy), pring.shape[0], _dtype_code(x), _stream(dev)),
-        'sfem_cg_flush_x')
+        _ptr(lazy), m, int(bool(ride)),
+        cg_ride_part_len(x.numel(), m, x.dtype) if ride else 0, int(issued),
+        _dtype_code(x), _stream(dev)), 'sfem_cg_flush_x')
 
 
 def cg_update_xp(x, p, z, scalars):
diff --git a/swirl_fem_amd/core/operators.py b/swirl_fem_amd/core/operators.py
--- a/swirl_fem_amd/core/operators.py
+++ b/swirl_fem_amd/core/operators.py
@@ -823,7 +823,7 @@
                        device=self.enc.device)
 
   def apply_layered(self, u, ext, lambda0=0.0, lambda1=1.0, *, dot_out=None,
-                    per_wave=False):
+                    per_wave=False, rider=None):
     plan = self.layer_plan()
     if plan is None:
       raise NotImplementedError('this operator has no layer plan')
@@ -836,7 +836,12 @@
     return _ops.helmholtz_apply_layered(
         u.to(self.fespace.dtype).contiguous(), ext, self.enc, plan.parts,
         self.host, mesh.ndim, mesh.gridpoints_1d.num_points, lambda0, lambda1,
-        dot_out, per_wave)
+        dot_out, per_wave, rider)
+
+  def carries_riders(self):
+    plan = self.layer_plan()
+    return (plan is not None and
+            _ops.layered_rider_part(plan.parts) is not None)
 
   def layered_dot_slots(self):
     mesh = self.fespace.mesh
@@ -970,11 +975,15 @@
       return None
     return plan
 
-  def apply_layered_with_dot(self, u, partials, per_wave=False):
+  def apply_layered_with_dot(self, u, partials, per_wave=False, rider=None):
     if self._ext is None:
       self._ext = self.op.new_extended()
     return self.op.apply_layered(u, self._ext, self.lambda0, self.lambda1,
-                                 dot_out=partials, per_wave=per_wave)
+                                 dot_out=partials, per_wave=per_wave,
+                                 rider=rider)
+
+  def carries_riders(self):
+    return self.layer_plan() is not None and self.op.carries_riders()
 
   def layered_dot_slots(self):
     return self.op.layered_dot_slots()
diff --git a/swirl_fem_amd/csrc/sfem_core.hip b/swirl_fem_amd/csrc/sfem_core.hip
--- a/swirl_fem_amd/csrc/sfem_core.hip
+++ b/swirl_fem_amd/csrc/sfem_core.hip
@@ -546,7 +546,7 @@
   }
 }
 
-template <typename T, bool NT>
+template <typename T, bool NT, bool RIDE = false>
 __global__ void __launch_bounds__(512)
 cg_update_xp_lazy_kernel(T* __restrict__ x, T* __restrict__ pring,
                          int64_t ring_stride, const T* __restrict__ z,
@@ -559,7 +559,7 @@
   const int slot = (int)(k % m), next = (int)((k + 1) % m);
   const T alpha = (T)(scalars[0] / scalars[1]);
   const T beta = (T)(cg_gamma_new(scalars) / scalars[0]);
-  const bool flush = next == 0;
+  const bool flush = !RIDE && next == 0;
   int64_t lo = (int64_t)lazy[0];
   if (lo < k + 1 - m) lo = k + 1 - m;
   T a_old[SFEM_CG_LAZY_MAX];
@@ -629,6 +629,32 @@
   const int64_t stride = (int64_t)gridDim.x * blockDim.x;
   for (int64_t i = (int64_t)blockIdx.x * blockDim.x + threadIdx.x; i < count;
        i += stride) {
+    T xx = x[i];
+    for (int64_t j = lo; j < iters; ++j)
+      xx += (T)lazy[1 + (j % m)] * pring[(j % m) * ring_stride + i];
+    x[i] = xx;
+  }
+}
+
+template <typename T>
+__global__ void __launch_bounds__(512)
+cg_flush_x_ride_kernel(T* __restrict__ x, const T* __restrict__ pring,
+                       int64_t ring_stride, int64_t count,
+                       const double* __restrict__ scalars,
+                       const double* __restrict__ lazy, int parts,
+                       int64_t part_len, int64_t issued) {
+  const int m = parts + 1;
+  const int64_t iters = (int64_t)scalars[8];
+  const int64_t base = (int64_t)lazy[0];
+  const int64_t last = issued - 1 < iters ? issued - 1 : iters;
+  if (base >= iters) return;
+  const int64_t stride = (int64_t)gridDim.x * blockDim.x;
+  for (int64_t i = (int64_t)blockIdx.x * blockDim.x + threadIdx.x; i < count;
+       i += stride) {
+    const int64_t q = i / part_len;
+    int64_t lo = last >= q ? last - (last - q) % parts : 0;
+    if (lo < base) lo = base;
+    if (lo >= iters) continue;
     T xx = x[i];
     for (int64_t j = lo; j < iters; ++j)
       xx += (T)lazy[1 + (j % m)] * pring[(j % m) * ring_stride + i];
@@ -1767,13 +1793,14 @@
 
 int sfem_cg_update_xp_lazy(void* x, void* pring, int64_t ring_stride,
                            const void* z, int64_t count, double* scalars,
-                           double* lazy, int m, int dtype,
+                           double* lazy, int m, int ride, int dtype,
                            sfem_stream_t stream) {
   SFEM_REQUIRE(count >= 0 && scalars && lazy,
                "sfem_cg_update_xp_lazy: bad arguments");
   SFEM_REQUIRE(m >= 2 && m <= SFEM_CG_LAZY_MAX,
-               "sfem_cg_update_xp_lazy: ring of %d directions (2..%d)", m,
+               "sfem_cg_update_xp_lazy: %d directions (2..%d)", m,
                SFEM_CG_LAZY_MAX);
+  if (ride) ++m;
   if (count == 0) return SFEM_OK;
   SFEM_REQUIRE(x && pring && z && ring_stride >= count,
                "sfem_cg_update_xp_lazy: null pointer or ring stride < count");
@@ -1784,7 +1811,16 @@
                "alignment");
   DISPATCH_DTYPE(dtype, {
     const int grid = stream_grid(count, 512 * 2);
-    if (streams_past_caches(count, sizeof(T)))
+    if (ride && streams_past_caches(count, sizeof(T)))
+      hipLaunchKernelGGL((cg_update_xp_lazy_kernel<T, true, true>), dim3(grid),
+                         dim3(512), 0, as_stream(stream), (T*)x, (T*)pring,
+                         ring_stride, (const T*)z, count, scalars, lazy, m);
+    else if (ride)
+      hipLaunchKernelGGL((cg_update_xp_lazy_kernel<T, false, true>),
+                         dim3(grid), dim3(512), 0, as_stream(stream), (T*)x,
+                         (T*)pring, ring_stride, (const T*)z, count, scalars,
+                         lazy, m);
+    else if (streams_past_caches(count, sizeof(T)))
       hipLaunchKernelGGL((cg_update_xp_lazy_kernel<T, true>), dim3(grid),
                          dim3(512), 0, as_stream(stream), (T*)x, (T*)pring,
                          ring_stride, (const T*)z, count, scalars, lazy, m);
@@ -1799,20 +1835,32 @@
 
 int sfem_cg_flush_x(void* x, const void* pring, int64_t ring_stride,
                     int64_t count, const double* scalars, double* lazy, int m,
-                    int dtype, sfem_stream_t stream) {
+                    int ride, int64_t part_len, int64_t issued, int dtype,
+                    sfem_stream_t stream) {
   SFEM_REQUIRE(count >= 0 && scalars && lazy && m >= 2 &&
                    m <= SFEM_CG_LAZY_MAX,
                "sfem_cg_flush_x: bad arguments");
   SFEM_REQUIRE(dtype == SFEM_F32 || dtype == SFEM_F64,
                "sfem_cg_flush_x: unknown dtype %d", dtype);
+  SFEM_REQUIRE(!ride || (part_len > 0 && issued >= 0 &&
+                         part_len * m >= count),
+               "sfem_cg_flush_x: ride mode needs the part length (%d parts "
+               "must cover x) and the iterations issued", m);
   if (count > 0) {
     SFEM_REQUIRE(x && pring && ring_stride >= count,
                  "sfem_cg_flush_x: null pointer or ring stride < count");
     DISPATCH_DTYPE(dtype, {
-      hipLaunchKernelGGL((cg_flush_x_kernel<T>),
-                         dim3(stream_grid(count, 512)), dim3(512), 0,
-                         as_stream(stream), (T*)x, (const T*)pring,
-                         ring_stride, count, scalars, lazy, m);
+      if (ride)
+        hipLaunchKernelGGL((cg_flush_x_ride_kernel<T>),
+                           dim3(stream_grid(count, 512)), dim3(512), 0,
+                           as_stream(stream), (T*)x, (const T*)pring,
+                           ring_stride, count, scalars, lazy, m, part_len,
+                           issued);
+      else
+        hipLaunchKernelGGL((cg_flush_x_kernel<T>),
+                           dim3(stream_grid(count, 512)), dim3(512), 0,
+                           as_stream(stream), (T*)x, (const T*)pring,
+                           ring_stride, count, scalars, lazy, m);
     });
   }
   hipLaunchKernelGGL(cg_lazy_mark_kernel, dim3(1), dim3(1), 0,
diff --git a/swirl_fem_amd/csrc/sfem_helmholtz.hip b/swirl_fem_amd/csrc/sfem_helmholtz.hip
--- a/swirl_fem_amd/csrc/sfem_helmholtz.hip
+++ b/swirl_fem_amd/csrc/sfem_helmholtz.hip
@@ -233,7 +233,34 @@
   const void* sigma = nullptr;
   int coef_mode = 0;
   const void* beta = nullptr;
+  const sfem_cg_rider* rider = nullptr;
 };
+
+constexpr int64_t RIDER_SEGMENTS = 8;
+constexpr int64_t RIDER_SLICE_BYTES = 16384;
+
+template <typename T>
+static FacetRider<T> make_facet_rider(const sfem_cg_rider& rd,
+                                      int64_t segments) {
+  FacetRider<T> fr{};
+  fr.x = (T*)rd.x;
+  fr.ring = (const T*)rd.ring;
+  fr.ring_stride = rd.ring_stride;
+  fr.begin = rd.begin;
+  fr.end = rd.end;
+  fr.slice = rd.slice > 0 ? rd.slice : RIDER_SLICE_BYTES / (int64_t)sizeof(T);
+  fr.lazy = rd.lazy;
+  fr.scalars = rd.scalars;
+  fr.iteration = rd.iteration;
+  fr.ring_slots = rd.ring_slots;
+  fr.lag = rd.lag;
+  int64_t riders = rd.riders > 0
+                       ? rd.riders
+                       : (segments + RIDER_SEGMENTS - 1) / RIDER_SEGMENTS;
+  fr.riders = (uint32_t)riders;
+  fr.period = (uint32_t)((segments + riders) / riders);
+  return fr;
+}
 
 template <typename T>
 static int run_helmholtz(const HelmholtzCall& c, hipStream_t stream) {
@@ -288,6 +315,7 @@
     fp.chain_elems = c.chain_elems;
     fp.layered = c.layered_extent > 0;
     fp.dot_slots = c.dot_slots;
+    if (c.rider) fp.rider = make_facet_rider<T>(*c.rider, c.num_chains);
     if (fp.layered)
       return dispatch_helmholtz_facet<T>(
           fp, c.P, c.geo_mode,
@@ -566,6 +594,29 @@
       c.num_chains = a->num_chains;
     }
   }
+  if (a->rider) {
+    const sfem_cg_rider* rd = a->rider;
+    if (!(a->facet_table && a->layered_extent && a->chain_offsets)) {
+      set_error("sfem_helmholtz_apply: riders go with layered chain launches");
+      return SFEM_EUNSUPPORTED;
+    }
+    const int64_t vn = a->dtype == SFEM_F64 ? 2 : 4;
+    SFEM_REQUIRE(rd->x && rd->ring && rd->lazy && rd->scalars,
+                 "sfem_helmholtz_apply: rider: null pointer");
+    SFEM_REQUIRE(rd->begin >= 0 && rd->begin <= rd->end &&
+                     rd->end <= rd->ring_stride && rd->begin % vn == 0 &&
+                     rd->ring_stride % vn == 0,
+                 "sfem_helmholtz_apply: rider: bad range or ring stride");
+    SFEM_REQUIRE(rd->lag >= 1 && rd->lag <= SFEM_CG_LAZY_MAX &&
+                     rd->ring_slots > rd->lag &&
+                     rd->ring_slots <= SFEM_CG_LAZY_MAX + 1 &&
+                     rd->iteration >= 0,
+                 "sfem_helmholtz_apply: rider: bad ring or iteration");
+    SFEM_REQUIRE(rd->riders >= 0 && rd->slice >= 0 && rd->slice % vn == 0 &&
+                     (int64_t)rd->riders + a->num_chains <= 0x7fffffff,
+                 "sfem_helmholtz_apply: rider: bad rider count or slice");
+    c.rider = rd;
+  }
   SFEM_REQUIRE(!a->layered_extent || a->facet_table,
                "sfem_helmholtz_apply: layered assembly needs a facet table");
   if (a->dtype == SFEM_F64) return run_helmholtz<double>(c, as_stream(stream));
diff --git a/swirl_fem_amd/csrc/sfem_helmholtz_facet.h b/swirl_fem_amd/csrc/sfem_helmholtz_facet.h
--- a/swirl_fem_amd/csrc/sfem_helmholtz_facet.h
+++ b/swirl_fem_amd/csrc/sfem_helmholtz_facet.h
@@ -1,4 +1,5 @@
 #pragma once
+#include <stddef.h>
 #include <stdlib.h>
 
 #include "sfem_helmholtz.h"
@@ -7,6 +8,20 @@
 
 constexpr int GEO_BOX = 5;
 constexpr int FACET_ROW = 27 * 4;
+
+template <typename T>
+struct FacetRider {
+  T* x;
+  const T* ring;
+  int64_t ring_stride;
+  int64_t begin, end;
+  int64_t slice;
+  const double* lazy;
+  const double* scalars;
+  int64_t iteration;
+  int32_t ring_slots, lag;
+  uint32_t riders, period;
+};
 
 template <typename T>
 struct FacetParams {
@@ -26,6 +41,7 @@
   double* dot_out;
   int layered;
   int64_t dot_slots;
+  FacetRider<T> rider;
 };
 
 constexpr uint32_t FACET_SKIP = 0x40000000u;
@@ -804,6 +820,111 @@
   }
 }
 
+template <typename T>
+struct RiderVec;
+template <>
+struct RiderVec<double> {
+  typedef double type __attribute__((ext_vector_type(2)));
+  static constexpr int N = 2;
+};
+template <>
+struct RiderVec<float> {
+  typedef float type __attribute__((ext_vector_type(4)));
+  static constexpr int N = 4;
+};
+
+template <typename T, int NTERMS, int BLOCK>
+__device__ __forceinline__ void facet_rider_terms(const FacetRider<T>& rd,
+                                                  uint32_t r, int64_t j0) {
+  using V = typename RiderVec<T>::type;
+  constexpr int VN = RiderVec<T>::N;
+  constexpr int U = 4;
+  T a[NTERMS];
+  const T* pj[NTERMS];
+#pragma unroll
+  for (int q = 0; q < NTERMS; ++q) {
+    const int64_t s = (j0 + q) % rd.ring_slots;
+    a[q] = (T)rd.lazy[1 + s];
+    pj[q] = rd.ring + s * rd.ring_stride;
+  }
+  const int64_t v1 = rd.end / VN, sv = rd.slice / VN;
+  for (int64_t s0 = rd.begin / VN + (int64_t)r * sv; s0 < v1;
+       s0 += (int64_t)rd.riders * sv) {
+    const uint32_t len = (uint32_t)(s0 + sv < v1 ? sv : v1 - s0);
+    V* xs = reinterpret_cast<V*>(rd.x) + s0;
+    const V* ps[NTERMS];
+#pragma unroll
+    for (int q = 0; q < NTERMS; ++q)
+      ps[q] = reinterpret_cast<const V*>(pj[q]) + s0;
+    uint32_t t = threadIdx.x;
+    for (; t + (U - 1) * BLOCK < len; t += U * BLOCK) {
+      V xx[U], pp[NTERMS][U];
+#pragma unroll
+      for (int u = 0; u < U; ++u) {
+        xx[u] = __builtin_nontemporal_load(xs + (t + u * BLOCK));
+#pragma unroll
+        for (int q = 0; q < NTERMS; ++q)
+          pp[q][u] = __builtin_nontemporal_load(ps[q] + (t + u * BLOCK));
+      }
+#pragma unroll
+      for (int u = 0; u < U; ++u) {
+#pragma unroll
+        for (int q = 0; q < NTERMS; ++q)
+#pragma unroll
+          for (int c = 0; c < VN; ++c) xx[u][c] += a[q] * pp[q][u][c];
+        __builtin_nontemporal_store(xx[u], xs + (t + u * BLOCK));
+      }
+    }
+    for (; t < len; t += BLOCK) {
+      V xx = __builtin_nontemporal_load(xs + t);
+      V pp[NTERMS];
+#pragma unroll
+      for (int q = 0; q < NTERMS; ++q)
+        pp[q] = __builtin_nontemporal_load(ps[q] + t);
+#pragma unroll
+      for (int q = 0; q < NTERMS; ++q)
+#pragma unroll
+        for (int c = 0; c < VN; ++c) xx[c] += a[q] * pp[q][c];
+      __builtin_nontemporal_store(xx, xs + t);
+    }
+  }
+  if (r == 0 && (int64_t)threadIdx.x < rd.end - v1 * VN) {
+    const int64_t i = v1 * VN + threadIdx.x;
+    T xx = rd.x[i];
+#pragma unroll
+    for (int q = 0; q < NTERMS; ++q) xx += a[q] * pj[q][i];
+    rd.x[i] = xx;
+  }
+}
+
+template <typename T, int BLOCK>
+__device__ __attribute__((noinline)) void facet_rider(const char* kernarg) {
+#if defined(__HIP_DEVICE_COMPILE__)
+  typedef const __attribute__((address_space(4))) FacetRider<T>* KernargRider;
+  const uint64_t addr = (uint64_t)(uintptr_t)kernarg +
+                        offsetof(FacetParams<T>, rider);
+  const uint64_t uniform =
+      (uint64_t)(uint32_t)__builtin_amdgcn_readfirstlane((uint32_t)addr) |
+      ((uint64_t)(uint32_t)__builtin_amdgcn_readfirstlane(
+           (uint32_t)(addr >> 32)) << 32);
+  const FacetRider<T> rd = *(KernargRider)uniform;
+  if (rd.scalars[7] != 0.0) return;
+  const uint32_t r = blockIdx.x / rd.period;
+  const int64_t first = rd.iteration > rd.lag ? rd.iteration - rd.lag : 0;
+  int64_t behind = (int64_t)rd.lazy[0] - first;
+  behind = behind < 0 ? 0 : (behind > rd.lag ? rd.lag : behind);
+  int64_t j0 = first + __builtin_amdgcn_readfirstlane((int32_t)behind);
+  while (j0 < rd.iteration) {
+    const int64_t n = rd.iteration - j0;
+    if (n >= 4) facet_rider_terms<T, 4, BLOCK>(rd, r, j0);
+    else if (n == 3) facet_rider_terms<T, 3, BLOCK>(rd, r, j0);
+    else if (n == 2) facet_rider_terms<T, 2, BLOCK>(rd, r, j0);
+    else facet_rider_terms<T, 1, BLOCK>(rd, r, j0);
+    j0 += n >= 4 ? 4 : n;
+  }
+#endif
+}
+
 template <typename T, int P, typename ELEM, bool OFF32, bool LAY = false>
 __global__ void __launch_bounds__(FacetLayout<P>::BLOCK, ELEM::CHAIN_MINW)
 helmholtz_chain_kernel(FacetParams<T> prm, typename ELEM::Mat dm) {
@@ -815,9 +936,20 @@
   T* s0 = lds;
   uint32_t* codes = reinterpret_cast<uint32_t*>(lds + L::COPY);
 
+  uint32_t seg = blockIdx.x;
+  if constexpr (LAY) {
+    if (prm.rider.x != nullptr) {
+      const uint32_t before = seg / prm.rider.period;
+      if (before < prm.rider.riders &&
+          seg - before * prm.rider.period == prm.rider.period - 1) {
+        facet_rider<T, L::BLOCK>(kernarg_bytes());
+        return;
+      }
+      seg -= before < prm.rider.riders ? before : prm.rider.riders;
+    }
+  }
   FacetWave<P> w;
   w.init();
-  const uint32_t seg = blockIdx.x;
   const int32_t k0 = prm.chain_off[seg];
   const int32_t k1 = prm.chain_off[seg + 1];
   const Mat* kdm = reinterpret_cast<const Mat*>(kernarg_bytes() + KA::MAT_OFF);
@@ -895,7 +1027,7 @@
 #pragma unroll
     for (int off = 32; off > 0; off >>= 1) udot += __shfl_down(udot, off, 64);
     if ((w.lane & 63) == 0) {
-      const int64_t wave = (int64_t)blockIdx.x * L::WAVES + (w.lane >> 6);
+      const int64_t wave = (int64_t)seg * L::WAVES + (w.lane >> 6);
       if (LAY && prm.dot_slots > 0)
         prm.dot_out[wave] = udot;
       else
@@ -915,12 +1047,13 @@
     }
     if (prm.chain_off) {
       if constexpr (ELEM::CHAINS) {
+        const dim3 cgrid(groups + (prm.rider.x ? prm.rider.riders : 0u));
         if (off32)
           hipLaunchKernelGGL((helmholtz_chain_kernel<T, P, ELEM, true, true>),
-                             grid, block, 0, stream, prm, mat);
+                             cgrid, block, 0, stream, prm, mat);
         else
           hipLaunchKernelGGL((helmholtz_chain_kernel<T, P, ELEM, false, true>),
-                             grid, block, 0, stream, prm, mat);
+                             cgrid, block, 0, stream, prm, mat);
       } else {
         set_error("helmholtz (facet): no chain kernel for this geometry at "
                   "P=%d", P);
diff --git a/swirl_fem_amd/linalg/cg.py b/swirl_fem_amd/linalg/cg.py
--- a/swirl_fem_amd/linalg/cg.py
+++ b/swirl_fem_amd/linalg/cg.py
@@ -107,6 +107,7 @@
     self._x = (_map(torch.zeros_like, b) if x0 is None
                else _map(lambda t, bb: layout.like(t, bb).clone(), x0, b))
     self.lazy = None
+    self.ride = None
     self.s = s = _Scalars(device)
     S = _Scalars
     self.identity_m = M is None
@@ -188,12 +189,20 @@
         self._p.numel() * self._p.element_size() >= _lazy_min_bytes()):
       m = min(m, _lib.SFEM_CG_LAZY_MAX)
       n = self._p.numel()
-      ring = torch.empty((m, (n + 3) // 4 * 4), dtype=self._p.dtype,
-                         device=device)
+      ride = (self.det is not None and reduce_fn is None and
+              interface is None and
+              switches.get('SFEM_LAZY_X_RIDE') != '0' and
+              getattr(A, 'carries_riders', lambda: False)())
+      ring = torch.empty((m + int(ride), (n + 3) // 4 * 4),
+                         dtype=self._p.dtype, device=device)
       ring[0, :n] = self._p.reshape(-1)
       self._p = None
-      self.lazy = (ring, n, torch.zeros(1 + _lib.SFEM_CG_LAZY_MAX,
-                                        dtype=torch.float64, device=device))
+      self.lazy = (ring[:m], n, torch.zeros(2 + _lib.SFEM_CG_LAZY_MAX,
+                                            dtype=torch.float64, device=device))
+      if ride:
+        self.ride = dict(
+            ring=ring, riders=int(switches.get('SFEM_LAZY_X_RIDERS') or 0),
+            slice_len=int(switches.get('SFEM_LAZY_X_SLICE') or 0))
       self._shape = tuple(self.r.shape)
     self.issued = 0
     self._graph = None
@@ -280,6 +289,8 @@
     if self.lazy is None:
       return self._p
     ring, n, _ = self.lazy
+    if self.ride is not None:
+      ring = self.ride['ring']
     return ring[self.issued % ring.shape[0], :n].view(self._shape)
 
   @property
@@ -287,7 +298,11 @@
     if self.lazy is not None:
       self._flush()
       ring, n, state = self.lazy
-      _ops.cg_flush_x(layout.flat(self._x), ring, self.s.t, state)
+      if self.ride is not None:
+        _ops.cg_flush_x(layout.flat(self._x), self.ride['ring'], self.s.t,
+                        state, ride=True, issued=self.issued)
+      else:
+        _ops.cg_flush_x(layout.flat(self._x), ring, self.s.t, state)
     return self._x
 
   def matches(self, b, tol, atol, maxiter) -> bool:
@@ -345,7 +360,16 @@
     A, M, dot_fn, reduce_fn = self.A, self.M, self.dot_fn, self.reduce_fn
     args = (self.maxiter, self.tol, self.atol, self.parts)
     merged = self.fused_dot and reduce_fn is None
-    if self.fused_dot and self.det is not None:
+    if self.fused_dot and self.det is not None and self.ride is not None:
+      rider = _ops.cg_rider(layout.flat(self._x), self.ride['ring'], s.t,
+                            self.lazy[2], self.issued, self.ride['riders'],
+                            self.ride['slice_len'])
+      Ap = A.apply_layered_with_dot(self.p, self.det[0], per_wave=True,
+                                    rider=rider)
+      _ops.cg_scalars_n(s.t, 5, self.maxiter, self.tol, self.atol,
+                        self.det[0],
+                        self.det[0].numel() - _lib.SFEM_FOLD_GROUPS)
+    elif self.fused_dot and self.det is not None:
       Ap = A.apply_layered_with_dot(self.p, self.det[0], per_wave=True)
       _ops.cg_scalars_n(s.t, 5, self.maxiter, self.tol, self.atol,
                         self.det[0],
@@ -429,8 +453,11 @@
         s.dot_into(S.GAMMA_NEW, self.r, z, dot_fn, reduce_fn)
     if self.lazy is not None:
       ring, n, state = self.lazy
+      if self.ride is not None:
+        ring = self.ride['ring']
       _ops.cg_update_xp_lazy(layout.flat(self._x), ring,
-                             layout.flat(layout.like(z, self.r)), s.t, state)
+                             layout.flat(layout.like(z, self.r)), s.t, state,
+                             ride=self.ride is not None)
     else:
       for xx, pp, zz in zip(_leaves(self._x), _leaves(self.p), _leaves(z)):
         _ops.cg_update_xp(layout.flat(xx), layout.flat(pp),
@@ -479,6 +506,7 @@
       ring, n, _ = self.lazy
       self._p = ring[0, :n].view(self._shape).clone()
       self.lazy = None
+      self.ride = None
     self.step()
     torch.cuda.synchronize()
     graph = torch.cuda.CUDAGraph()
diff --git a/swirl_fem_amd/switches.py b/swirl_fem_amd/switches.py
--- a/swirl_fem_amd/switches.py
+++ b/swirl_fem_amd/switches.py
@@ -43,6 +43,17 @@
     'SFEM_LAZY_X_MIN_MB': (None, 'linalg/cg.py',
                            'smallest vector (MiB) that gets the lazy x update '
                            '(default 256; the tests set 0)'),
+    'SFEM_LAZY_X_RIDE': ('1', 'linalg/cg.py',
+                         '0: the lazy x update adds its pending terms in one '
+                         'lump every SFEM_LAZY_X-th iteration instead of '
+                         'spreading them over rider workgroups of the layered '
+                         'operator applies'),
+    'SFEM_LAZY_X_RIDERS': (None, 'linalg/cg.py',
+                           'rider workgroups per layered apply (default: the '
+                           "library's, one per eight chain segments)"),
+    'SFEM_LAZY_X_SLICE': (None, 'linalg/cg.py',
+                          'elements a rider streams before it moves on '
+                          "(default: the library's, 16 KiB)"),
     'SFEM_SORTED_SCATTER': ('1', 'core/operators.py',
                             '0: index-row kernels issue their atomics in slot '
                             'order instead of node order'),
```
